# PieSil/CUDA-spectral-ray-tracer

Measured on AMD Instinct MI355X. Metric: Mray/s, higher is better.
Workload: dtype f32; 1 GPU; random-spheres tri scene (4802 tris, 9603 BVH nodes), 1920x1080, 1024 spp, depth 16; scene_id=100, tiles=8x8 px per wave, rank = tile % n_gpus, gather=none (1 GPU), launch_mode=one process, one GPU

## Files before the change

cuda-spectral-ray-tracer_amd/binding.py:

```python
import ctypes as C
import os

_HERE = os.path.dirname(os.path.abspath(__file__))
LIB_PATH = os.environ.get("SRT_LIB_PATH") or os.path.join(_HERE, "libsrt_hip.so")

N_CIE = 95
TILE_PLANES = 9
TILE_LANES = 64

SCENE_CORNELL, SCENE_PRISM, SCENE_TRIS, SCENE_RANDOM_SPHERES, SCENE_MESH100K = 0, 1, 2, 100, 101
BVH_REFERENCE, BVH_SAH = 0, 1
MAT_LAMBERTIAN, MAT_METALLIC, MAT_DIELECTRIC, MAT_EMISSIVE, MAT_NO_MAT = 0, 1, 2, 4, 6


class TriIn(C.Structure):
    _fields_ = [("v0", C.c_float * 3), ("v1", C.c_float * 3), ("v2", C.c_float * 3),
                ("mat_index", C.c_uint32), ("aa_plane", C.c_uint32)]


class Material(C.Structure):
    _fields_ = [("col", C.c_float * 3), ("reflection_fuzz", C.c_float), ("material_type", C.c_uint32),
                ("spectral_distribution", C.c_float * N_CIE), ("emission_power", C.c_float),
                ("sellmeier_B", C.c_float * 3), ("sellmeier_C", C.c_float * 3)]


class CameraData(C.Structure):
    _fields_ = [("width", C.c_uint32), ("height", C.c_uint32),
                ("pixel_delta_u", C.c_float * 3), ("pixel_delta_v", C.c_float * 3), ("pixel00_loc", C.c_float * 3),
                ("defocus_angle", C.c_float),
                ("camera_center", C.c_float * 3), ("defocus_disk_u", C.c_float * 3), ("defocus_disk_v", C.c_float * 3)]


class Stats(C.Structure):
    _fields_ = [("rays", C.c_uint64), ("paths", C.c_uint64), ("node_visits", C.c_uint64), ("tri_tests", C.c_uint64),
                ("box_tests", C.c_uint64), ("util", C.c_uint64 * 9), ("reserved", C.c_uint64 * 2), ("shade", C.c_uint64 * 4),
                ("waves", C.c_uint64 * 4), ("hits", C.c_uint64)]


class Calibration(C.Structure):
    _fields_ = [("wave_cycles_mean", C.c_double), ("wave_cycles_max", C.c_double), ("wall_ms", C.c_double),
                ("instr_per_wave", C.c_uint64), ("n_waves", C.c_uint32), ("n_cu", C.c_uint32), ("waves_per_simd", C.c_uint32),
                ("reserved", C.c_uint32), ("wave_cycles_min", C.c_double)]


class Adaptive(C.Structure):
    _fields_ = [("rel_tol", C.c_float), ("abs_tol", C.c_float), ("min_spp", C.c_uint32), ("reserved", C.c_uint32)]


class Denoise(C.Structure):
    _fields_ = [("levels", C.c_uint32), ("sigma_color", C.c_float), ("sigma_normal", C.c_float), ("sigma_albedo", C.c_float),
                ("sigma_depth", C.c_float), ("reserved", C.c_uint32 * 3)]


class DenoiseVG(C.Structure):
    _fields_ = [("levels", C.c_uint32), ("sigma_variance", C.c_float), ("sigma_normal", C.c_float), ("sigma_albedo", C.c_float),
                ("sigma_depth", C.c_float), ("variance_floor", C.c_float), ("reserved", C.c_uint32 * 2)]


class TreeTuning(C.Structure):
    _fields_ = [("pixels_per_lane", C.c_double), ("throughput_bound", C.c_uint32), ("reinsertion", C.c_uint32),
                ("probe_width", C.c_uint32), ("probe_height", C.c_uint32), ("probe_spp", C.c_uint32), ("nodes_swapped", C.c_uint32),
                ("order_status", C.c_int32)]


class TileScheduleInfo(C.Structure):
    _fields_ = [("tiles_local", C.c_uint32), ("n_rows", C.c_uint32), ("cost_max", C.c_uint32), ("n_waves_plan", C.c_uint32),
                ("split_load_pct", C.c_uint32), ("order_max_pct", C.c_uint32), ("streams", C.c_uint32), ("reserved", C.c_uint32)]


assert C.sizeof(Denoise) == 32 and C.sizeof(DenoiseVG) == 32
assert C.sizeof(Adaptive) == 16 and C.sizeof(TreeTuning) == 40 and C.sizeof(TileScheduleInfo) == 32
assert C.sizeof(Material) == 428 and C.sizeof(CameraData) == 84 and C.sizeof(TriIn) == 44

_vp, _i, _u32, _u64, _f, _sz = C.c_void_p, C.c_int, C.c_uint32, C.c_uint64, C.c_float, C.c_size_t
_fp = C.POINTER(C.c_float)
PROTOTYPES = {
    "srt_version": (C.c_char_p, []),
    "srt_camera_init": (_i, [_i, _i, _f, _fp, _fp, _fp, _f, _f, C.POINTER(CameraData)]),
    "srt_scene_create": (_vp, []),
    "srt_scene_builtin": (_vp, [_i, _u64]),
    "srt_scene_destroy": (None, [_vp]),
    "srt_scene_default_camera": (_i, [_vp, _i, _i, C.POINTER(CameraData)]),
    "srt_scene_set_triangles": (_i, [_vp, C.POINTER(TriIn), _sz]),
    "srt_scene_set_materials": (_i, [_vp, C.POINTER(Material), _sz]),
    "srt_scene_set_background": (_i, [_vp, _fp]),
    "srt_scene_tri_count": (_sz, [_vp]),
    "srt_scene_material_count": (_sz, [_vp]),
    "srt_scene_get_triangles": (_i, [_vp, C.POINTER(TriIn)]),
    "srt_scene_get_materials": (_i, [_vp, C.POINTER(Material)]),
    "srt_scene_get_background": (_i, [_vp, _fp]),
    "srt_scene_get_tri_records": (_i, [_vp, _fp]),
    "srt_material_bake": (_i, [C.POINTER(Material)]),
    "srt_set_reference_quirks": (_i, [_i]),
    "srt_bake_sigmoid_spectrum": (_i, [_fp, _f, _i, _fp]),
    "srt_fit_sigmoid_coeffs": (_i, [_fp, _fp]),
    "srt_color_tables": (_i, [_fp, _fp]),
    "srt_background_spectrum": (_i, [_fp, _fp]),
    "srt_rotation_matrix": (_i, [_f, _i, _fp]),
    "srt_scene_build_bvh": (_i, [_vp, _i, _u64]),
    "srt_scene_order_children": (_i, [_vp, _fp]),
    "srt_scene_optimise_bvh": (_i, [_vp, C.c_int]),
    "srt_scene_is_paired": (_i, [_vp]),
    "srt_scene_node_count": (_sz, [_vp]),
    "srt_scene_bvh_depth": (_i, [_vp]),
    "srt_scene_get_bvh": (_i, [_vp, C.POINTER(C.c_int32), C.POINTER(C.c_int32), C.POINTER(C.c_int32), _fp]),
    "srt_create": (_i, [_i, C.POINTER(_vp)]),
    "srt_destroy": (None, [_vp]),
    "srt_last_error": (C.c_char_p, [_vp]),
    "srt_upload_scene": (_i, [_vp, _vp]),
    "srt_set_camera": (_i, [_vp, C.POINTER(CameraData)]),
    "srt_launch_plan": (_i, [_vp, C.POINTER(_i), C.POINTER(_i), C.POINTER(_i), C.POINTER(_i)]),
    "srt_launch_paired": (_i, [_vp, C.POINTER(_i)]),
    "srt_set_test_knobs": (_i, [_vp, _i, _i, _u32]),
    "srt_get_test_knobs": (_i, [_vp, C.POINTER(_i), C.POINTER(_i), C.POINTER(_u32), C.POINTER(_i)]),
    "srt_launch_lds_bytes": (_i, [_vp, C.POINTER(_sz)]),
    "srt_init_device_params": (_i, [_vp, _u32, _u32, _u32, _u32, _u32, _u32, _u32, _u32, _u64]),
    "srt_set_partition": (_i, [_vp, _u32, _u32]),
    "srt_render_chunk": (_i, [_vp, _u32, _u32, _u32, _u32, _vp]),
    "srt_synchronize": (_i, [_vp]),
    "srt_accum_reset": (_i, [_vp]),
    "srt_render_chunk_accum": (_i, [_vp, _u32, _u32, _u32, _u32, _u32, _vp]),
    "srt_accum_samples": (_i, [_vp, C.POINTER(_u32)]),
    "srt_accum_reset_adaptive": (_i, [_vp, C.POINTER(Adaptive)]),
    "srt_accum_active": (_i, [_vp, C.POINTER(_u64)]),
    "srt_read_accum_stats": (_i, [_vp, C.POINTER(_u32), _fp, _fp, _u32, _u32]),
    "srt_accum_reset_spectral": (_i, [_vp]),
    "srt_read_spectral": (_i, [_vp, _u32, _u32, _fp, _u32, _u32]),
    "srt_develop_spectral": (_i, [_vp, _fp, _u32, _f, _fp, _u32, _u32]),
    "srt_develop_spectral_srgb": (_i, [_vp, _fp, _f, _fp, _fp, _fp, _u32, _u32]),
    "srt_develop_kat": (_i, [_vp, _fp, _u32, _fp, _u32, _f, _fp]),
    "srt_develop_last_ms": (_i, [_vp, _fp, _fp]),
    "srt_accum_reset_features": (_i, [_vp]),
    "srt_read_features": (_i, [_vp, _fp, _u32, _u32]),
    "srt_accum_reset_adaptive_features": (_i, [_vp, C.POINTER(Adaptive)]),
    "srt_accum_reset_spectral_features": (_i, [_vp]),
    "srt_denoise_developed": (_i, [_vp, C.POINTER(Denoise), _fp, _u32, _f, _fp, _fp, _u32, _u32]),
    "srt_denoise_developed_kat": (_i, [_vp, C.POINTER(Denoise), _fp, _fp, _fp, _u32, _u32, _u32, _u32, _fp, _fp]),
    "srt_denoise_features": (_i, [_vp, C.POINTER(Denoise), _fp, _fp, _fp, _u32, _u32]),
    "srt_denoise_kat": (_i, [_vp, C.POINTER(Denoise), _fp, _fp, _u32, _u32, _u32, _fp]),
    "srt_denoise_last_ms": (_i, [_vp, _fp, _fp, _fp, C.POINTER(_u32)]),
    "srt_denoise_features_vg": (_i, [_vp, C.POINTER(DenoiseVG), _fp, _fp, _fp, _fp, _u32, _u32]),
    "srt_denoise_vg_kat": (_i, [_vp, C.POINTER(DenoiseVG), _fp, _fp, _u32, _u32, _u32, _fp, _fp]),
    "srt_denoise_estimate_last_ms": (_i, [_vp, _fp]),
    "srt_denoise_features_mv": (_i, [_vp, C.POINTER(DenoiseVG), _fp, _fp, _fp, _fp, _u32, _u32]),
    "srt_denoise_mv_kat": (_i, [_vp, C.POINTER(DenoiseVG), _fp, _fp, C.POINTER(_u32), _fp, _u32, _u32, _fp, _fp]),
    "srt_accum_reset_streams": (_i, [_vp, _u32]),
    "srt_accum_streams": (_i, [_vp, C.POINTER(_u32)]),
    "srt_set_gather_planes": (_i, [_vp, _u32]),
    "srt_tile_buffer": (_i, [_vp, C.POINTER(_vp), C.POINTER(_sz), C.POINTER(_u32), C.POINTER(_u32)]),
    "srt_copy_tile_buffer": (_i, [_vp, _vp, _vp]),
    "srt_scatter_tiles": (_i, [_vp, _vp, _vp]),
    "srt_dev_fb": (_i, [_vp, C.POINTER(_vp), C.POINTER(_vp), C.POINTER(_vp), C.POINTER(_sz)]),
    "srt_read_fb": (_i, [_vp, _fp, _fp, _fp]),
    "srt_read_fb_rowmajor": (_i, [_vp, _fp, _fp, _fp, _u32, _u32]),
    "srt_read_fb_aux": (_i, [_vp, _i, _fp, _fp, _fp]),
    "srt_get_tile_costs": (_i, [_vp, C.POINTER(C.c_uint32), _sz]),
    "srt_order_children_by_profile": (_i, [_vp, _vp, C.c_uint32, C.c_uint32, C.c_uint32, C.c_uint32, C.c_uint32, C.POINTER(C.c_uint32)]),
    "srt_pixels_per_lane": (_i, [_vp, _u32, _u32, _u32, C.POINTER(C.c_double)]),
    "srt_tune_tree_for_throughput": (_i, [_vp, _vp, _u32, _u32, _u32, _u32, _i, C.POINTER(TreeTuning)]),
    "srt_get_stats": (_i, [_vp, C.POINTER(Stats)]),
    "srt_set_count_traversal": (_i, [_vp, _i]),
    "srt_get_wave_debug": (_i, [_vp, C.POINTER(C.c_uint32), _sz]),
    "srt_last_kernel_ms": (_i, [_vp, C.POINTER(_f)]),
    "srt_trace_rays": (_i, [_vp, _fp, _sz, _fp]),
    "srt_device_op_sweep": (_i, [_vp, _i, _fp, _fp, _sz, _fp]),
    "srt_order_tiles_kat": (_i, [_vp, C.POINTER(_u32), _u32, _u32, _u32, _u32, C.POINTER(_u32), _sz, C.POINTER(_u32), C.POINTER(_u32)]),
    "srt_read_tile_schedule": (_i, [_vp, _i, C.POINTER(_u32), _sz, C.POINTER(TileScheduleInfo)]),
    "srt_calibrate": (_i, [_vp, _i, _u32, _u32, C.POINTER(Calibration)]),
    "srt_ctx_device": (_i, [_vp]),
    "srt_ctx_cu_count": (_i, [_vp]),
    "srt_comm_init_all": (_i, [C.POINTER(_i), _i, C.POINTER(_vp)]),
    "srt_comm_unique_id": (_i, [C.POINTER(C.c_ubyte)]),
    "srt_comm_init_rank": (_i, [_vp, C.POINTER(C.c_ubyte), _u32, _u32, C.POINTER(_vp)]),
    "srt_comm_available": (_i, []),
    "srt_comm_set_gather_planes": (_i, [_vp, _u32]),
    "srt_comm_last_gather_ms": (_i, [_vp, C.POINTER(_f)]),
    "srt_comm_destroy": (None, [_vp]),
    "srt_comm_last_error": (C.c_char_p, [_vp]),
    "srt_comm_world": (_u32, [_vp]),
    "srt_comm_local_count": (_u32, [_vp]),
    "srt_comm_ctx": (_vp, [_vp, _u32]),
    "srt_comm_root_ctx": (_vp, [_vp]),
    "srt_comm_upload_scene": (_i, [_vp, _vp]),
    "srt_comm_set_camera": (_i, [_vp, C.POINTER(CameraData)]),
    "srt_comm_init_device_params": (_i, [_vp, _u32, _u32, _u32, _u32, _u32, _u32, _u32, _u32, _u64]),
    "srt_render_frame_multi": (_i, [_vp, _u32, _u32, _u32, _u32]),
    "srt_comm_accum_reset": (_i, [_vp]),
    "srt_render_frame_multi_accum": (_i, [_vp, _u32, _u32, _u32, _u32, _u32]),
    "srt_comm_accum_reset_adaptive": (_i, [_vp, C.POINTER(Adaptive)]),
    "srt_comm_accum_active": (_i, [_vp, C.POINTER(_u64)]),
    "srt_comm_accum_reset_spectral": (_i, [_vp]),
    "srt_comm_accum_reset_features": (_i, [_vp]),
    "srt_comm_accum_reset_adaptive_features": (_i, [_vp, C.POINTER(Adaptive)]),
    "srt_comm_accum_reset_spectral_features": (_i, [_vp]),
    "srt_comm_accum_reset_streams": (_i, [_vp, _u32]),
    "srt_comm_synchronize": (_i, [_vp]),
    "srt_comm_stats": (_i, [_vp, C.POINTER(_u64), C.POINTER(_u64), C.POINTER(_f)]),
}


class SrtError(RuntimeError):
    def __init__(self, code, msg):
        super().__init__("srt error %d: %s" % (code, msg))
        self.code = code


_lib = None


def lib():
    global _lib
    if _lib is None:
        if not os.path.exists(LIB_PATH):
            raise ImportError("%s not found: run `python -c 'import __graft_entry__ as g; g.build()'` "
                              "(there is no CPU fallback for the render path)" % LIB_PATH)
        L = C.CDLL(LIB_PATH)
        for name, (res, args) in PROTOTYPES.items():
            fn = getattr(L, name)
            fn.restype = res
            fn.argtypes = args
        _lib = L
    return _lib


COMM_ID_BYTES = 128


def check_comm(code, comm=None):
    if code is not None and code < 0:
        msg = lib().srt_comm_last_error(comm)
        raise SrtError(code, msg.decode() if msg else "")
    return code


def check(code, ctx=None):
    if code is not None and code < 0:
        msg = lib().srt_last_error(ctx)
        raise SrtError(code, msg.decode() if msg else "")
    return code


def fptr(arr):
    return arr.ctypes.data_as(_fp)
```

cuda-spectral-ray-tracer_amd/csrc/srt_capi.cpp:

```cpp
#include <dlfcn.h>
#include <hip/hip_runtime.h>
#include <stdint.h>
#include <stdlib.h>
#include <string.h>

#include <algorithm>
#include <cmath>
#include <cstddef>
#include <string>
#include <vector>

#include "srt_host.h"
#include "srt_internal.h"

using namespace srt;

#ifndef SRT_FRINGE_STRIDE_L2
#define SRT_FRINGE_STRIDE_L2 96
#endif
static constexpr uint32_t kFringeStrideL2 = SRT_FRINGE_STRIDE_L2;
static constexpr uint32_t kScoreShadeL2 = 320u, kScoreFringeL2 = 800u;

struct DeviceBuffer {
    void *ptr = nullptr;
    size_t bytes = 0;
    DeviceBuffer() = default;
    DeviceBuffer(DeviceBuffer &&o) noexcept { swap(o); }
    DeviceBuffer &operator=(DeviceBuffer &&o) noexcept { swap(o); return *this; }
    ~DeviceBuffer() { release(); }
    void swap(DeviceBuffer &o) { std::swap(ptr, o.ptr); std::swap(bytes, o.bytes); }
    void release() { if (ptr) (void)hipFree(ptr); ptr = nullptr; bytes = 0; }
    hipError_t reserve(size_t n) {
        if (n <= bytes) return hipSuccess;
        release();
        const hipError_t e = hipMalloc(&ptr, n);
        if (e == hipSuccess) bytes = n; else ptr = nullptr;
        return e;
    }
    template <typename T> T *as() const { return static_cast<T *>(ptr); }
    explicit operator bool() const { return ptr != nullptr; }
};

struct srt_ctx {
    int device = 0;
    std::string err;
    DeviceBuffer d_nodes, d_nodes_sw, d_fringe, d_tris, d_mat_sd, d_mat_par, d_shade, d_cmf;
    DeviceBuffer d_mat_col;
    int root_ref = 0, stack_depth = 1, n_inner = 0, n_records = 0;
    bool paired = false;
    uint32_t fringe_stride = 96;
    uint32_t n_tris = 0;
    uint32_t n_materials = 0;
    bool scene_ready = false, camera_ready = false, params_ready = false;
    srt_camera_data cam;
    uint32_t tx = 0, ty = 0, bx = 0, by = 0, chunk_w = 0, chunk_h = 0, spp = 0, bounce = 0;
    uint64_t seed = SRT_DEFAULT_SEED;
    uint32_t n_lanes = 0;
    uint32_t rank = 0, world = 1;
    uint32_t gather_planes = 3;
    uint32_t fb_groups_valid = 3;
    uint32_t last_w = 0, last_h = 0, last_offx = 0, last_offy = 0;
    uint32_t tiles_x = 0, tiles_y = 0, n_tiles = 0, tiles_local = 0, tiles_padded = 0;
    DeviceBuffer d_rng;
    DeviceBuffer d_fb;
    DeviceBuffer d_tiles;
    DeviceBuffer d_counters;
    int n_cu = 256;
    uint32_t waves_per_cu = 0;
    uint32_t score_shade = 0, score_fringe = 0;
    uint32_t debug_lane_limit = 0;
    PlanKnobs knobs;
    bool knobs_from_env = false;
    uint32_t split_load_pct = 200;
    uint32_t probe_spp = 2;
    int order_max_pct = -1;
    DeviceBuffer d_tile_cost, d_tile_order;
    srt_tile_schedule_info sched_note = {};
    bool sched_probe_queue = false, sched_compacted_queue = false;
    bool count_traversal = false;
    hipEvent_t ev0 = nullptr, ev1 = nullptr;
    bool timed = false;
    DeviceBuffer d_rowmajor;
    uint32_t rowmajor_w = 0, rowmajor_h = 0;
    OrderProfile order_profile = {};
    DeviceBuffer d_wave_debug;
    uint32_t stats_spp = 0;
    bool stats_adaptive = false;
    struct Accumulation {
        enum class State { Invalid, Empty, Bound } state = State::Invalid;
        enum class Kind { Plain, Adaptive, Spectral, Streams, Features, AdaptiveFeatures, SpectralFeatures } kind = Kind::Plain;
        uint32_t total = 0;
        uint32_t n_streams = 1;
        uint32_t w = 0, h = 0, offx = 0, offy = 0;
        void invalidate() { state = State::Invalid; }
        void begin(Kind k, uint32_t streams_per_pixel = 1) { kind = k; n_streams = streams_per_pixel; state = State::Empty; }
        bool valid() const { return state != State::Invalid; }
        bool bound() const { return state == State::Bound; }
        bool adaptive() const { return kind == Kind::Adaptive || kind == Kind::AdaptiveFeatures; }
        bool spectral() const { return kind == Kind::Spectral || kind == Kind::SpectralFeatures; }
        bool streamed() const { return kind == Kind::Streams; }
        bool featured() const { return kind == Kind::Features || kind == Kind::AdaptiveFeatures || kind == Kind::SpectralFeatures; }
    } accum;
    DeviceBuffer d_accum;
    DeviceBuffer d_adapt;
    DeviceBuffer d_adapt_queue;
    DeviceBuffer d_film;
    DeviceBuffer d_film_staging;
    DeviceBuffer d_features;
    DeviceBuffer d_features_staging;
    DeviceBuffer d_denoise;
    DeviceBuffer d_denoise_in;
    DeviceBuffer d_denoise_dev;
    hipEvent_t denoise_ev[12] = {};
    uint32_t denoise_timed_levels = 0;
    uint32_t denoise_level_ev = 1;
    bool denoise_timed = false;
    DeviceBuffer d_develop;
    DeviceBuffer d_develop_in;
    hipEvent_t develop_ev[3] = {};
    bool develop_timed = false, develop_epilogue = false;
    DeviceBuffer d_streams;
    uint32_t streams_seeded = 0;
};

namespace {

struct Roctx {
    int (*push)(const char *) = nullptr;
    int (*pop)() = nullptr;
    Roctx() {
        for (const char *n : {"libroctx64.so.4", "libroctx64.so", "/opt/rocm/lib/libroctx64.so.4"}) {
            if (void *h = dlopen(n, RTLD_NOW | RTLD_LOCAL)) {
                push = (int (*)(const char *))dlsym(h, "roctxRangePushA");
                pop = (int (*)())dlsym(h, "roctxRangePop");
                if (push && pop) return;
                push = nullptr; pop = nullptr;
            }
        }
    }
};
struct RoctxRange {
    static Roctx &api() { static Roctx r; return r; }
    explicit RoctxRange(const char *name) { if (api().push) api().push(name); }
    ~RoctxRange() { if (api().pop) api().pop(); }
};

int fail(srt_ctx *ctx, int code, const std::string &msg) {
    if (ctx) ctx->err = msg;
    set_global_error(msg);
    return code;
}
int hip_fail(srt_ctx *ctx, hipError_t e, const char *what) {
    return fail(ctx, SRT_ERR_HIP, std::string(what) + ": " + hipGetErrorString(e));
}
#define HIP_TRY_AS(ctx, what, expr) do { if (hipError_t _e = (expr)) return hip_fail(ctx, _e, what); } while (0)
#define HIP_TRY(ctx, expr) HIP_TRY_AS(ctx, #expr, expr)

int upload(srt_ctx *ctx, DeviceBuffer &dst, const std::vector<float> &src) {
    HIP_TRY(ctx, dst.reserve(src.size() * sizeof(float)));
    HIP_TRY(ctx, hipMemcpy(dst.ptr, src.data(), src.size() * sizeof(float), hipMemcpyHostToDevice));
    return SRT_OK;
}


struct TileSchedule {
    uint32_t *rows = nullptr, *sorted = nullptr, *info = nullptr, *cost = nullptr;
    static size_t order_bytes(size_t tiles) { return (tiles * 65 + 4) * sizeof(uint32_t); }
    static size_t cost_bytes(size_t tiles) { return 2 * tiles * sizeof(uint32_t); }
    explicit TileSchedule(const srt_ctx *c) : cost(c->d_tile_cost.as<uint32_t>()) {
        if (!c->d_tile_order) return;
        const size_t tiles = (c->d_tile_order.bytes / sizeof(uint32_t) - 4) / 65;
        rows = c->d_tile_order.as<uint32_t>(); sorted = rows + tiles * 64; info = sorted + tiles;
    }
};

struct AdaptQueue {
    uint32_t *info, *rows, *flags;
    unsigned long long *counts;
    static size_t bytes(size_t n_rows) { return (8 + 2 * n_rows) * sizeof(uint32_t); }
    explicit AdaptQueue(const DeviceBuffer &d_adapt_queue)
        : info(d_adapt_queue.as<uint32_t>()), rows(info + 8), flags(rows + (d_adapt_queue.bytes / sizeof(uint32_t) - 8) / 2),
          counts(reinterpret_cast<unsigned long long *>(info + 4)) {}
};
int read_adapt_counts(srt_ctx *c, uint64_t *rendered, uint64_t *active) {
    unsigned long long counts = 0;
    HIP_TRY(c, hipMemcpy(&counts, AdaptQueue(c->d_adapt_queue).counts, sizeof(counts), hipMemcpyDeviceToHost));
    if (rendered) *rendered = counts & 0xffffffffull;
    if (active) *active = counts >> 32;
    return SRT_OK;
}

struct AccumLayout {
    static constexpr size_t kAccumHeaderBytes = 256;
    AccumHeader *header;
    float *sums, *y;
    static size_t sums_bytes(size_t lanes) { return 3 * lanes * sizeof(float); }
    static size_t bytes(size_t lanes) { return kAccumHeaderBytes + sums_bytes(lanes); }
    explicit AccumLayout(const srt_ctx *c)
        : header(c->d_accum.as<AccumHeader>()), sums(reinterpret_cast<float *>(c->d_accum.as<char>() + kAccumHeaderBytes)), y(sums + c->n_lanes) {}
};
void set_accum_header(RenderParams &p, AccumHeader *h) { p.wave_debug = reinterpret_cast<uint32_t *>(h); }

struct AdaptPlanes {
    float *sum2;
    uint32_t *state;
    static size_t bytes(size_t lanes) { return 2 * lanes * sizeof(float); }
    explicit AdaptPlanes(const srt_ctx *c) : sum2(c->d_adapt.as<float>()), state(c->d_adapt.as<uint32_t>() + c->n_lanes) {}
};

struct StreamPlanes {
    uint32_t *rng;
    float *sums;
    static size_t sums_bytes(size_t lanes, size_t k) { return 3 * k * lanes * sizeof(float); }
    static size_t bytes(size_t lanes, size_t k) { return kStreamSumPlane * k * lanes * sizeof(uint32_t) + sums_bytes(lanes, k); }
    StreamPlanes(const DeviceBuffer &d_streams, size_t lanes, size_t k) : rng(d_streams.as<uint32_t>()), sums(d_streams.as<float>() + kStreamSumPlane * k * lanes) {}
};

uint32_t clipped_w(const srt_ctx *c) { return std::min<uint32_t>(c->last_w, c->tx * c->bx); }
uint32_t clipped_h(const srt_ctx *c) { return std::min<uint32_t>(c->last_h, c->ty * c->by); }
struct ChunkRect { uint32_t w, h; size_t first; };
ChunkRect chunk_rect(const srt_ctx *c, uint32_t image_width, uint32_t image_height) {
    if (c->last_offx >= image_width || c->last_offy >= image_height) return {0, 0, 0};
    return {std::min<uint32_t>(clipped_w(c), image_width - c->last_offx), std::min<uint32_t>(clipped_h(c), image_height - c->last_offy),
            (size_t)c->last_offy * image_width + c->last_offx};
}

size_t wave_debug_bytes(size_t n_waves) { return sizeof(OrderProfile) + n_waves * 4 * sizeof(uint32_t); }
uint32_t wave_debug_waves(const srt_ctx *c) { return c->d_wave_debug ? (uint32_t)((c->d_wave_debug.bytes - sizeof(OrderProfile)) / (4 * sizeof(uint32_t))) : 0u; }

float *fb_plane(const srt_ctx *c, int k) { return c->d_fb.as<float>() + (size_t)k * c->n_lanes; }

LaunchPlan plan_of(const srt_ctx *c) { LaunchPlan lp; render_launch_plan(c->stack_depth, c->n_records, c->n_inner, c->knobs, lp); return lp; }

void fill_params(const srt_ctx *c, RenderParams &p) {
    memset(&p, 0, sizeof(p));
    p.nodes = c->d_nodes.as<const float4>(); p.nodes_sw = c->d_nodes_sw.as<const float>(); p.fringe = c->d_fringe.as<const float4>(); p.tris = c->d_tris.as<const float4>();
    p.mat_sd = c->d_mat_sd.as<const float2>(); p.mat_par = c->d_mat_par.as<const float4>();
    p.shade = c->d_shade.as<const float4>(); p.cmf = c->d_cmf.as<const float4>();
    p.root_ref = c->root_ref; p.stack_depth = c->stack_depth; p.n_materials = c->n_materials;
    p.n_inner = c->n_inner; p.n_cached = 0;
    p.n_tris = c->n_tris; p.n_records = c->n_records; p.fringe_stride = c->fringe_stride;
    p.paired = c->paired ? 1u : 0u;
    for (int k = 0; k < 3; k++) {
        p.du[k] = c->cam.pixel_delta_u[k]; p.dv[k] = c->cam.pixel_delta_v[k]; p.p00[k] = c->cam.pixel00_loc[k];
        p.center[k] = c->cam.camera_center[k]; p.disk_u[k] = c->cam.defocus_disk_u[k]; p.disk_v[k] = c->cam.defocus_disk_v[k];
    }
    p.defocus_angle = c->cam.defocus_angle;
    p.tx = c->tx; p.ty = c->ty; p.bx = c->bx; p.by = c->by;
    p.spp = c->spp; p.bounce_limit = c->bounce;
    p.rank = c->rank; p.world = c->world;
    p.rng = c->d_rng.as<uint32_t>(); p.n_lanes = c->n_lanes;
    p.tile_out = c->d_tiles.as<float>(); p.counters = c->d_counters.as<unsigned long long>();
    p.tile_group_stride = c->tiles_padded * (uint32_t)(kGroupPlanes * kTileLanes);
    p.write_parity = c->gather_planes == (uint32_t)kTilePlanes ? 1u : 0u;
}


struct Pass {
    uint32_t spp_add;
    hipStream_t st;
    RenderMode mode;
    bool later;
    LaunchPlan plan;
    bool ordered;
    uint32_t adapt_bound;
    uint32_t streams;
};

bool adaptive_mode(RenderMode m) { return m == Adaptive || m == AdaptiveFeatures; }
uint32_t split_rows_bound(const srt_ctx *c) { return (uint32_t)std::min<uint64_t>((uint64_t)c->tiles_local * 64, 0x7fffffffull); }
constexpr uint64_t kQueueSlots = 1ull << 32;
bool queue_may_split(const srt_ctx *c, uint32_t streams) { return c->split_load_pct && (streams == 1 || (uint64_t)split_rows_bound(c) * streams * 64 < kQueueSlots); }

void tile_geometry(srt_ctx *c) {
    const uint32_t cover_w = c->tx * c->bx, cover_h = c->ty * c->by;
    c->tiles_x = (cover_w + 7) / 8; c->tiles_y = (cover_h + 7) / 8;
    c->n_tiles = c->tiles_x * c->tiles_y;
    c->tiles_padded = (c->n_tiles + c->world - 1) / c->world;
    c->tiles_local = c->n_tiles > c->rank ? (c->n_tiles - c->rank + c->world - 1) / c->world : 0;
}

int prepare_tiles(srt_ctx *c, const Pass &ps) {
    tile_geometry(c);
    const size_t tile_floats = (size_t)std::max<uint32_t>(c->tiles_padded, 1) * kTileLanes;
    HIP_TRY(c, c->d_tiles.reserve(tile_floats * kTilePlanes * sizeof(float)));
    if (!(adaptive_mode(ps.mode) && ps.later)) HIP_TRY(c, hipMemsetAsync(c->d_tiles.ptr, 0, tile_floats * c->gather_planes * sizeof(float), ps.st));
    HIP_TRY(c, hipMemsetAsync(c->d_counters.ptr, 0, (kCounters + 1) * sizeof(unsigned long long), ps.st));
    return SRT_OK;
}

void chunk_params(const srt_ctx *c, const Pass &ps, uint32_t width, uint32_t height, uint32_t offx, uint32_t offy, RenderParams &p) {
    fill_params(c, p);
    if (ps.spp_add) p.spp = ps.spp_add / ps.streams;
    p.width = width; p.height = height; p.offx = offx; p.offy = offy;
    p.tiles_x = c->tiles_x; p.tiles_y = c->tiles_y; p.n_tiles = c->n_tiles;
    p.tiles_local = c->tiles_local;
    p.pixel_counter = reinterpret_cast<uint32_t *>(c->d_counters.as<unsigned long long>() + kCounters);
    p.waves_per_cu_override = c->waves_per_cu;
    const bool all_cached = ps.plan.all_cached;
    p.score_shade = c->score_shade ? c->score_shade : (all_cached ? 70u : kScoreShadeL2);
    const bool paired = render_paired_variant(c->paired, render_narrow_refs(c->n_records, c->knobs), all_cached);
    p.score_fringe = c->score_fringe ? c->score_fringe : (all_cached ? (paired ? 400u : 280u) : kScoreFringeL2);
    p.tile_order = nullptr; p.tile_cost = nullptr; p.queue_rows = nullptr; p.queue_rows_bound = c->tiles_local;
    p.debug_lane_limit = c->debug_lane_limit;
}

int run_cost_probe(srt_ctx *c, const Pass &ps, const RenderParams &p) {
    HIP_TRY(c, c->d_tile_cost.reserve(TileSchedule::cost_bytes(c->tiles_local)));
    HIP_TRY(c, c->d_tile_order.reserve(TileSchedule::order_bytes(c->tiles_local)));
    const TileSchedule sched(c);
    HIP_TRY(c, hipMemsetAsync(sched.cost, 0, TileSchedule::cost_bytes(c->tiles_local), ps.st));
    RenderParams pp = p;
    pp.spp = c->probe_spp; pp.tile_cost = sched.cost;
    RoctxRange range_probe("srt cost probe + pixel queue");
    HIP_TRY(c, launch_render(pp, c->knobs, (uint32_t)c->n_cu, Probe, ps.st));
    const uint32_t n_waves_plan = std::max<uint32_t>((uint32_t)c->n_cu * (uint32_t)ps.plan.waves_per_cu / ps.streams, 1u);
    const uint32_t order_pct = c->order_max_pct >= 0 ? (uint32_t)c->order_max_pct : ((!ps.plan.all_cached && (uint64_t)c->tiles_local < 6ull * n_waves_plan) ? 100u : 0u);
    const uint32_t split_pct = queue_may_split(c, ps.streams) ? c->split_load_pct : 0u;
    HIP_TRY(c, launch_order_tiles(sched.cost, sched.sorted, sched.rows, c->tiles_local, n_waves_plan, split_pct, sched.info, order_pct, ps.st));
    c->sched_note = {};
    c->sched_note.tiles_local = c->tiles_local; c->sched_note.n_waves_plan = n_waves_plan; c->sched_note.split_load_pct = split_pct;
    c->sched_note.order_max_pct = order_pct; c->sched_note.streams = ps.streams;
    HIP_TRY(c, hipMemsetAsync(c->d_counters.as<unsigned long long>() + kCounters, 0, sizeof(unsigned long long), ps.st));
    return SRT_OK;
}

enum class QueueSource { Identity, FreshProbe, ReusedProbe, Compacted };

QueueSource queue_source(const srt_ctx *c, const Pass &ps) {
    if (adaptive_mode(ps.mode) && ps.later && c->tiles_local <= kQueueTileMask) return QueueSource::Compacted;
    if (!ps.ordered) return QueueSource::Identity;
    return ps.later ? QueueSource::ReusedProbe : QueueSource::FreshProbe;
}

int choose_queue(srt_ctx *c, Pass &ps, RenderParams &p) {
    const bool schedulable = c->probe_spp > 0 && c->tiles_local > 1 && c->tiles_local <= kQueueTileMask;
    ps.ordered = schedulable && (ps.spp_add || c->spp > 4 * c->probe_spp);
    ps.adapt_bound = ps.ordered && c->split_load_pct ? split_rows_bound(c) : c->tiles_local;
    if (adaptive_mode(ps.mode)) HIP_TRY(c, c->d_adapt_queue.reserve(AdaptQueue::bytes(std::max<uint32_t>(ps.adapt_bound, 1u))));
    const QueueSource src = queue_source(c, ps);
    c->sched_probe_queue = false; c->sched_compacted_queue = false;
    if (src == QueueSource::Compacted) {
        const AdaptQueue q(c->d_adapt_queue);
        p.tile_order = q.rows;
        p.queue_rows = q.info;
        p.prio_cost = ps.ordered ? c->d_tile_cost.as<uint32_t>() : nullptr;
        p.queue_rows_bound = ps.adapt_bound;
    } else if (src != QueueSource::Identity) {
        if (src == QueueSource::FreshProbe)
            if (const int rc = run_cost_probe(c, ps, p)) return rc;
        const TileSchedule sched(c);
        p.tile_order = sched.rows;
        p.queue_rows = sched.info;
        p.prio_cost = sched.cost;
        if (queue_may_split(c, ps.streams)) p.queue_rows_bound = split_rows_bound(c);
    }
    c->sched_probe_queue = ps.ordered && src != QueueSource::Identity;
    p.queue_rows_bound *= ps.streams;
    return SRT_OK;
}

int bind_wave_debug(srt_ctx *c, const Pass &ps, RenderParams &p) {
    if (!c->count_traversal) return SRT_OK;
    const uint32_t most_waves = render_launch_grid(ps.plan, (uint32_t)c->n_cu, p.waves_per_cu_override, UINT32_MAX).waves;
    HIP_TRY(c, c->d_wave_debug.reserve(wave_debug_bytes(most_waves)));
    HIP_TRY(c, hipMemsetAsync(c->d_wave_debug.ptr, 0, c->d_wave_debug.bytes, ps.st));
    p.wave_debug = c->d_wave_debug.as<uint32_t>();
    if (c->order_profile.magic == kOrderProfileMagic)
        HIP_TRY(c, hipMemcpyAsync(c->d_wave_debug.ptr, &c->order_profile, sizeof(OrderProfile), hipMemcpyHostToDevice, ps.st));
    return SRT_OK;
}

int launch_pass(srt_ctx *c, const Pass &ps, RenderParams &p) {
    if (c->count_traversal && render_launch_grid(ps.plan, (uint32_t)c->n_cu, p.waves_per_cu_override, p.queue_rows_bound).waves > wave_debug_waves(c))
        return fail(c, SRT_ERR_HIP, "srt_render_chunk: the launch started more waves than the debug buffer holds (launch plan and launcher disagree)");
    HIP_TRY(c, hipEventRecord(c->ev0, ps.st));
    if (ps.spp_add) set_accum_header(p, AccumLayout(c).header);
    HIP_TRY(c, launch_render(p, c->knobs, (uint32_t)c->n_cu, ps.mode, ps.st));
    HIP_TRY(c, hipEventRecord(c->ev1, ps.st));
    return SRT_OK;
}

int compact_adaptive_queue(srt_ctx *c, const Pass &ps, const RenderParams &p) {
    const TileSchedule sched(c);
    const AdaptQueue dst(c->d_adapt_queue);
    AdaptQueueParams q = {};
    q.src_rows = ps.ordered ? sched.rows : nullptr; q.src_info = ps.ordered ? sched.info : nullptr; q.n_identity = c->tiles_local;
    q.dst_info = dst.info; q.dst_rows = dst.rows; q.flags = dst.flags; q.counts = dst.counts;
    q.state = AdaptPlanes(c).state;
    q.spp_total = c->accum.total + ps.spp_add;
    q.width = p.width; q.height = p.height; q.tx = c->tx; q.ty = c->ty; q.bx = c->bx; q.by = c->by;
    q.tiles_x = c->tiles_x; q.n_tiles = c->n_tiles; q.rank = c->rank; q.world = c->world;
    q.lane_limit = c->debug_lane_limit ? c->debug_lane_limit : 64u;
    HIP_TRY(c, hipMemsetAsync(q.counts, 0, sizeof(unsigned long long), ps.st));
    HIP_TRY(c, launch_adapt_queue(q, ps.adapt_bound, ps.st));
    c->sched_compacted_queue = true;
    return SRT_OK;
}

int combine_streams(srt_ctx *c, const Pass &ps, const RenderParams &p) {
    StreamCombineParams q = {};
    q.stream_sums = StreamPlanes(c->d_streams, c->n_lanes, ps.streams).sums; q.sums = AccumLayout(c).sums; q.tile_out = p.tile_out;
    q.streams = ps.streams; q.spp_total = c->accum.total + ps.spp_add; q.n_lanes = c->n_lanes;
    q.tile_group_stride = p.tile_group_stride; q.write_parity = p.write_parity; q.tiles_local = c->tiles_local;
    q.width = p.width; q.height = p.height; q.tx = c->tx; q.ty = c->ty; q.bx = c->bx; q.by = c->by;
    q.tiles_x = c->tiles_x; q.n_tiles = c->n_tiles; q.rank = c->rank; q.world = c->world;
    q.lane_limit = c->debug_lane_limit ? c->debug_lane_limit : 64u;
    HIP_TRY(c, launch_stream_combine(q, ps.st));
    return SRT_OK;
}

int render_chunk_impl(srt_ctx *c, uint32_t width, uint32_t height, uint32_t offx, uint32_t offy, uint32_t spp_add, hipStream_t st) {
    Pass ps = {};
    ps.spp_add = spp_add; ps.st = st;
    ps.mode = !spp_add ? (c->count_traversal ? Counting : Plain) : c->accum.adaptive() ? (c->accum.featured() ? AdaptiveFeatures : Adaptive) : c->accum.spectral() ? (c->accum.featured() ? SpectralFeatures : Spectral) : c->accum.streamed() ? Streams : c->accum.featured() ? Features : Accum;
    ps.later = spp_add && c->accum.bound(); ps.plan = plan_of(c);
    ps.streams = ps.mode == Streams ? c->accum.n_streams : 1u;
    c->last_w = width; c->last_h = height; c->last_offx = offx; c->last_offy = offy;
    RenderParams p;
    if (const int rc = prepare_tiles(c, ps)) return rc;
    chunk_params(c, ps, width, height, offx, offy, p);
    if (const int rc = choose_queue(c, ps, p)) return rc;
    if (const int rc = bind_wave_debug(c, ps, p)) return rc;
    RoctxRange range_render("srt render_kernel");
    if (const int rc = launch_pass(c, ps, p)) return rc;
    if (adaptive_mode(ps.mode))
        if (const int rc = compact_adaptive_queue(c, ps, p)) return rc;
    if (ps.mode == Streams)
        if (const int rc = combine_streams(c, ps, p)) return rc;
    c->timed = true;
    c->stats_spp = spp_add;
    c->stats_adaptive = adaptive_mode(ps.mode);
    return SRT_OK;
}

int read_planes(srt_ctx *c, int first_plane, float *p0, float *p1, float *p2) {
    if (!c || !c->d_fb) return fail(c, SRT_ERR_INVALID, "read: device parameters not initialised");
    if (const int rc = srt_synchronize(c)) return rc;
    float *dst[3] = {p0, p1, p2};
    for (int k = 0; k < 3; k++)
        if (dst[k]) HIP_TRY(c, hipMemcpy(dst[k], fb_plane(c, first_plane + k), (size_t)c->n_lanes * sizeof(float), hipMemcpyDeviceToHost));
    return SRT_OK;
}

int read_rowmajor(srt_ctx *c, const float *const src[3], float *const host[3], uint32_t image_width, uint32_t image_height) {
    HIP_TRY(c, hipSetDevice(c->device));
    const size_t n = (size_t)image_width * image_height;
    if (c->rowmajor_w != image_width || c->rowmajor_h != image_height || !c->d_rowmajor) {
        HIP_TRY(c, c->d_rowmajor.reserve(3 * n * sizeof(float)));
        HIP_TRY(c, hipMemset(c->d_rowmajor.ptr, 0, 3 * n * sizeof(float)));
        c->rowmajor_w = image_width; c->rowmajor_h = image_height;
    }
    float *dst[3] = {c->d_rowmajor.as<float>(), c->d_rowmajor.as<float>() + n, c->d_rowmajor.as<float>() + 2 * n};
    HIP_TRY(c, launch_unswizzle(src, dst, c->tx, c->ty, c->bx, c->by, c->last_w, c->last_h, c->last_offx, c->last_offy, image_width, image_height, nullptr));
    const ChunkRect rect = chunk_rect(c, image_width, image_height);
    const size_t pitch = (size_t)image_width * sizeof(float);
    for (int k = 0; k < 3 && rect.w && rect.h; k++)
        if (host[k]) HIP_TRY(c, hipMemcpy2D(host[k] + rect.first, pitch, dst[k] + rect.first, pitch, (size_t)rect.w * sizeof(float), rect.h, hipMemcpyDeviceToHost));
    HIP_TRY(c, hipDeviceSynchronize());
    return SRT_OK;
}

}

extern "C" {

int srt_create(int device, srt_ctx **out) {
    if (!out) return fail(nullptr, SRT_ERR_INVALID, "srt_create: null out");
    *out = nullptr;
    int n = 0;
    hipError_t e = hipGetDeviceCount(&n);
    if (e != hipSuccess || n <= 0)
        return fail(nullptr, SRT_ERR_NO_DEVICE, std::string("srt_create: no HIP device (") + (e != hipSuccess ? hipGetErrorString(e) : "count 0") +
                                                    "); this library has no CPU fallback");
    if (device < 0 || device >= n) return fail(nullptr, SRT_ERR_NO_DEVICE, "srt_create: device index out of range");
    e = hipSetDevice(device);
    if (e != hipSuccess) return hip_fail(nullptr, e, "hipSetDevice");
    srt_ctx *c = new srt_ctx();
    c->device = device;
    if (const char *ev = getenv("SRT_WAVES_PER_CU")) c->waves_per_cu = (uint32_t)std::max(0, atoi(ev));
    if (const char *ev = getenv("SRT_PROBE_SPP")) c->probe_spp = (uint32_t)std::max(0, atoi(ev));
    if (const char *ev = getenv("SRT_SCORE_SHADE")) c->score_shade = (uint32_t)std::max(1, atoi(ev));
    if (const char *ev = getenv("SRT_SCORE_FRINGE")) c->score_fringe = (uint32_t)std::max(1, atoi(ev));
    if (const char *tk = getenv("SRT_TEST_KNOBS")) if (atoi(tk) == 1) {
        if (const char *ev = getenv("SRT_DEBUG_LANE_LIMIT")) { c->debug_lane_limit = (uint32_t)std::max(0, atoi(ev)); c->knobs_from_env = true; }
        if (const char *ev = getenv("SRT_WIDE_REFS")) { c->knobs.wide_refs = atoi(ev) != 0; c->knobs_from_env = true; }
        if (const char *ev = getenv("SRT_LDS_CACHE_MAX")) { c->knobs.lds_cache_max = std::max(0, atoi(ev)); c->knobs_from_env = true; }
    }
    if (const char *ev = getenv("SRT_SPLIT_LOAD")) c->split_load_pct = (uint32_t)std::max(0, atoi(ev));
    if (const char *ev = getenv("SRT_ORDER_MAX_PCT")) c->order_max_pct = std::min(400, std::max(-1, atoi(ev)));
    {
        hipDeviceProp_t prop;
        if (hipGetDeviceProperties(&prop, device) == hipSuccess && prop.multiProcessorCount > 0) c->n_cu = prop.multiProcessorCount;
    }
    std::vector<float> rows(96 * 4);
    cmf_rows(rows.data());
    int rc = upload(c, c->d_cmf, rows);
    if (rc != SRT_OK) { delete c; return rc; }
    if ((e = c->d_counters.reserve((kCounters + 1) * sizeof(unsigned long long))) != hipSuccess ||
        (e = hipMemset(c->d_counters.ptr, 0, (kCounters + 1) * sizeof(unsigned long long))) != hipSuccess ||
        (e = hipEventCreate(&c->ev0)) != hipSuccess || (e = hipEventCreate(&c->ev1)) != hipSuccess) {
        int r = hip_fail(nullptr, e, "srt_create");
        srt_destroy(c);
        return r;
    }
    *out = c;
    return SRT_OK;
}

void srt_destroy(srt_ctx *c) {
    if (!c) return;
    (void)hipSetDevice(c->device);
    (void)hipDeviceSynchronize();
    if (c->ev0) (void)hipEventDestroy(c->ev0);
    if (c->ev1) (void)hipEventDestroy(c->ev1);
    for (hipEvent_t e : c->denoise_ev) if (e) (void)hipEventDestroy(e);
    for (hipEvent_t e : c->develop_ev) if (e) (void)hipEventDestroy(e);
    delete c;
}

int srt_ctx_device(const srt_ctx *ctx) { return ctx ? ctx->device : -1; }
int srt_ctx_cu_count(const srt_ctx *ctx) { return ctx ? ctx->n_cu : -1; }

const char *srt_last_error(const srt_ctx *ctx) { return ctx ? ctx->err.c_str() : global_error(); }

int srt_upload_scene(srt_ctx *c, const srt_scene *s) {
    if (!c || !s) return fail(c, SRT_ERR_INVALID, "srt_upload_scene: null argument");
    c->accum.invalidate();
    c->sched_probe_queue = false; c->sched_compacted_queue = false;
    HIP_TRY(c, hipSetDevice(c->device));
    FlatScene f;
    int rc = flatten_scene(*s, f);
    if (rc != SRT_OK) return fail(c, rc, global_error());
    if (render_lds_bytes(f.stack_depth, 1, 0, f.n_records, c->knobs) > 64 * 1024) return fail(c, SRT_ERR_BVH, "srt_upload_scene: BVH too deep for the LDS traversal stack");
    if ((rc = upload(c, c->d_nodes, f.nodes)) != SRT_OK) return rc;
    {
        LaunchPlan plan;
        render_launch_plan(f.stack_depth, f.n_records, f.n_inner, c->knobs, plan);
        uint32_t stride = plan.all_cached ? 96u : kFringeStrideL2;
        if (const char *ev = getenv("SRT_FRINGE_STRIDE")) stride = (atoi(ev) == 128 && !plan.all_cached) ? 128u : 96u;
        if ((uint64_t)(f.n_records - f.n_inner + 1) * stride >= (1ull << 31)) stride = 96u;
        std::vector<float> padded;
        if (stride != 96u) {
            const size_t n_fr = f.fringe.size() / 24;
            padded.assign(n_fr * 32, 0.f);
            for (size_t k = 0; k < n_fr; k++) memcpy(&padded[32 * k], &f.fringe[24 * k], 24 * sizeof(float));
        }
        if ((rc = upload(c, c->d_fringe, stride == 96u ? f.fringe : padded)) != SRT_OK) return rc;
        c->fringe_stride = stride;
        c->d_nodes_sw.release();
        if (!plan.all_cached && (rc = upload(c, c->d_nodes_sw, f.nodes_sw)) != SRT_OK) return rc;
    }
    if ((rc = upload(c, c->d_tris, f.tris)) != SRT_OK) return rc;
    if ((rc = upload(c, c->d_mat_sd, f.mat_sd)) != SRT_OK) return rc;
    if ((rc = upload(c, c->d_mat_par, f.mat_par)) != SRT_OK) return rc;
    if ((rc = upload(c, c->d_shade, f.shade)) != SRT_OK) return rc;
    {
        std::vector<float> col(4 * s->mats.size(), 0.f);
        for (size_t m = 0; m < s->mats.size(); m++)
            for (int k = 0; k < 3; k++) col[4 * m + k] = s->mats[m].col[k];
        if ((rc = upload(c, c->d_mat_col, col)) != SRT_OK) return rc;
    }
    c->root_ref = f.root_ref; c->stack_depth = f.stack_depth; c->n_materials = (uint32_t)s->mats.size();
    c->n_inner = f.n_inner; c->n_records = f.n_records; c->n_tris = (uint32_t)s->raw.size();
    c->paired = tree_is_paired(*s);
    c->scene_ready = true;
    return SRT_OK;
}

int srt_set_camera(srt_ctx *c, const srt_camera_data *cam) {
    if (!c || !cam) return fail(c, SRT_ERR_INVALID, "srt_set_camera: null argument");
    c->accum.invalidate();
    c->cam = *cam;
    c->camera_ready = true;
    return SRT_OK;
}

int srt_launch_plan(const srt_ctx *c, int *waves_per_cu, int *n_cached, int *all_cached, int *narrow_refs) {
    if (!c || !c->scene_ready) return fail(nullptr, SRT_ERR_INVALID, "srt_launch_plan: no scene uploaded");
    const LaunchPlan plan = plan_of(c);
    if (waves_per_cu) *waves_per_cu = plan.waves_per_cu;
    if (n_cached) *n_cached = plan.n_cached;
    if (all_cached) *all_cached = plan.all_cached ? 1 : 0;
    if (narrow_refs) *narrow_refs = render_narrow_refs(c->n_records, c->knobs) ? 1 : 0;
    return SRT_OK;
}

int srt_launch_paired(const srt_ctx *c, int *paired) {
    if (!c || !c->scene_ready || !paired) return fail(nullptr, SRT_ERR_INVALID, "srt_launch_paired: no scene uploaded / null argument");
    const LaunchPlan plan = plan_of(c);
    *paired = render_paired_variant(c->paired, render_narrow_refs(c->n_records, c->knobs), plan.all_cached) ? 1 : 0;
    return SRT_OK;
}

int srt_launch_lds_bytes(const srt_ctx *c, size_t *bytes) {
    if (!c || !c->scene_ready || !bytes) return fail(nullptr, SRT_ERR_INVALID, "srt_launch_lds_bytes: no scene uploaded / null argument");
    const LaunchPlan plan = plan_of(c);
    *bytes = render_lds_bytes(c->stack_depth, plan.waves_per_block, plan.n_cached, c->n_records, c->knobs);
    return SRT_OK;
}

int srt_set_test_knobs(srt_ctx *c, int wide_refs, int lds_cache_max, uint32_t lane_limit) {
    if (!c || lds_cache_max < -1 || lane_limit > 64) return fail(c, SRT_ERR_INVALID, "srt_set_test_knobs: bad argument");
    c->knobs.wide_refs = wide_refs != 0; c->knobs.lds_cache_max = lds_cache_max; c->debug_lane_limit = lane_limit;
    c->scene_ready = false;
    return SRT_OK;
}
int srt_get_test_knobs(const srt_ctx *c, int *wide_refs, int *lds_cache_max, uint32_t *lane_limit, int *from_env) {
    if (!c) return fail(nullptr, SRT_ERR_INVALID, "srt_get_test_knobs: null ctx");
    if (wide_refs) *wide_refs = c->knobs.wide_refs ? 1 : 0;
    if (lds_cache_max) *lds_cache_max = c->knobs.lds_cache_max;
    if (lane_limit) *lane_limit = c->debug_lane_limit;
    if (from_env) *from_env = c->knobs_from_env ? 1 : 0;
    return SRT_OK;
}

int srt_internal_init_device_params(srt_ctx *c, uint32_t tx, uint32_t ty, uint32_t bx, uint32_t by, uint32_t chunk_w, uint32_t chunk_h,
                                    uint32_t spp, uint32_t bounce_limit, uint64_t seed, int wait) {
    if (!c) return fail(c, SRT_ERR_INVALID, "srt_init_device_params: null ctx");
    if (tx == 0 || ty == 0 || bx == 0 || by == 0 || chunk_w == 0 || chunk_h == 0)
        return fail(c, SRT_ERR_INVALID, "srt_init_device_params: zero dimension");
    c->accum.invalidate();
    c->sched_probe_queue = false; c->sched_compacted_queue = false;
    const uint64_t lanes = (uint64_t)tx * ty * bx * by;
    if (lanes > 0x7fffffffull) return fail(c, SRT_ERR_INVALID, "srt_init_device_params: grid too large");
    HIP_TRY(c, hipSetDevice(c->device));
    c->tx = tx; c->ty = ty; c->bx = bx; c->by = by; c->chunk_w = chunk_w; c->chunk_h = chunk_h;
    c->spp = (uint16_t)spp; c->bounce = (uint16_t)bounce_limit;
    c->seed = seed; c->n_lanes = (uint32_t)lanes;
    c->streams_seeded = 0;
    HIP_TRY(c, c->d_rng.reserve(6 * lanes * sizeof(uint32_t)));
    HIP_TRY(c, c->d_fb.reserve(kTilePlanes * lanes * sizeof(float)));
    HIP_TRY(c, hipMemset(c->d_fb.ptr, 0, kTilePlanes * lanes * sizeof(float)));
    HIP_TRY(c, launch_init_rng(c->d_rng.as<uint32_t>(), c->n_lanes, seed, nullptr));
    if (wait) HIP_TRY(c, hipDeviceSynchronize());
    c->fb_groups_valid = (uint32_t)kTileGroups;
    c->params_ready = true;
    return SRT_OK;
}

int srt_init_device_params(srt_ctx *c, uint32_t tx, uint32_t ty, uint32_t bx, uint32_t by, uint32_t chunk_w, uint32_t chunk_h,
                           uint32_t spp, uint32_t bounce_limit, uint64_t seed) {
    return srt_internal_init_device_params(c, tx, ty, bx, by, chunk_w, chunk_h, spp, bounce_limit, seed, 1);
}

int srt_set_partition(srt_ctx *c, uint32_t rank, uint32_t world) {
    if (!c || world == 0 || rank >= world) return fail(c, SRT_ERR_INVALID, "srt_set_partition: need rank < world");
    c->accum.invalidate();
    c->sched_probe_queue = false; c->sched_compacted_queue = false;
    c->rank = rank; c->world = world;
    return SRT_OK;
}

// ... 944 lines not shown
        }
        c->count_traversal = true; c->rank = 0; c->world = 1;
        int r = srt_init_device_params(c, tx, ty, bx, by, width, height, spp, bounce_limit, SRT_DEFAULT_SEED);
        if (r == SRT_OK) r = srt_render_chunk(c, width, height, 0, 0, nullptr);
        if (r == SRT_OK) r = srt_synchronize(c);
        c->count_traversal = counting; c->rank = rank; c->world = world;
        c->order_profile = OrderProfile{};
        c->params_ready = false;
        if (r != SRT_OK) return r;
        unsigned long long h[kCounters];
        HIP_TRY_AS(c, "srt_order_children_by_profile: counters", hipMemcpy(h, c->d_counters.ptr, sizeof(h), hipMemcpyDeviceToHost));
        work = h[1] + 2ull * h[2];
        return SRT_OK;
    };
    unsigned long long work_before = 0, work_after = 0;
    if ((rc = probe_frame(true, work_before)) != SRT_OK) return rc;
    std::vector<uint32_t> cnt(2 * n_nodes, 0u);
    HIP_TRY_AS(c, "srt_order_children_by_profile: read back", hipMemcpy(cnt.data(), d_cnt.ptr, cnt.size() * sizeof(uint32_t), hipMemcpyDeviceToHost));
    {
        unsigned long long samples = 0;
        for (uint32_t v : cnt) samples += v;
        if (samples == 0) return fail(c, SRT_ERR_INVALID, "srt_order_children_by_profile: the probe frame recorded no samples (no closest hit with the sibling's box beyond it)");
    }
    const uint32_t *won = cnt.data();
    std::vector<uint32_t> swapped_nodes;
    for (size_t k = 0; k < n_nodes; k++) {
        BvhNode &nd = s->nodes[k];
        if (nd.prim >= 0) continue;
        const uint32_t l = won[2 * k], r = won[2 * k + 1];
        if (l + r >= std::max<uint32_t>(min_samples, 1u) && r > l) { std::swap(nd.left, nd.right); swapped_nodes.push_back((uint32_t)k); }
    }
    if (!swapped_nodes.empty()) {
        rc = srt_upload_scene(c, s);
        if (rc == SRT_OK) rc = probe_frame(false, work_after);
        if (rc == SRT_OK && work_after >= work_before) {
            for (uint32_t k : swapped_nodes) std::swap(s->nodes[k].left, s->nodes[k].right);
            swapped_nodes.clear();
            rc = srt_upload_scene(c, s);
        }
    }
    if (rc == SRT_OK && n_swapped) *n_swapped = (uint32_t)swapped_nodes.size();
    return rc;
}

int srt_pixels_per_lane(const srt_ctx *c, uint32_t width, uint32_t height, uint32_t world, double *out) {
    if (!c || !c->scene_ready || !out) return fail(nullptr, SRT_ERR_INVALID, "srt_pixels_per_lane: no scene uploaded / null argument");
    const double lanes = (double)c->n_cu * plan_of(c).waves_per_cu * 64.0;
    *out = (double)width * height / (double)std::max<uint32_t>(world, 1u) / (lanes > 0 ? lanes : 1.0);
    return SRT_OK;
}

static constexpr double kTunePixelsPerLane = 6.0;
static constexpr size_t kTuneReinsertionMaxTris = 8192;
static constexpr int kTuneReinsertionPasses = 3;
static constexpr uint32_t kTuneProbeDivisor = 4, kTuneProbeMinSide = 32, kTuneProbeSpp = 8;
static constexpr uint32_t kTuneDecidingRays = 16;

int srt_tune_tree_for_throughput(srt_ctx *c, srt_scene *s, uint32_t width, uint32_t height, uint32_t world, uint32_t bounce_limit,
                                 int only_if_throughput_bound, srt_tree_tuning *out) {
    if (out) memset(out, 0, sizeof(*out));
    if (!c || !s || !out || !s->bvh_valid || width == 0 || height == 0)
        return fail(c, SRT_ERR_INVALID, "srt_tune_tree_for_throughput: null argument / BVH not built / empty frame");
    int rc = srt_upload_scene(c, s);
    if (rc == SRT_OK) rc = srt_pixels_per_lane(c, width, height, world, &out->pixels_per_lane);
    if (rc != SRT_OK) return rc;
    out->throughput_bound = out->pixels_per_lane >= kTunePixelsPerLane ? 1u : 0u;
    if (only_if_throughput_bound && !out->throughput_bound) return SRT_OK;
    if (s->raw.size() <= kTuneReinsertionMaxTris) {
        auto resident = [&](const FlatScene &f) { LaunchPlan lp; render_launch_plan(f.stack_depth, f.n_records, f.n_inner, c->knobs, lp); return lp.all_cached; };
        const bool kept = optimise_bvh_unless(*s, kTuneReinsertionPasses, [&](const FlatScene &before, const FlatScene &after) { return !(resident(before) && !resident(after)); });
        out->reinsertion = kept ? 1u : 2u;
    }
    const uint32_t pw = std::max(width / kTuneProbeDivisor, kTuneProbeMinSide), ph = std::max(height / kTuneProbeDivisor, kTuneProbeMinSide);
    srt_camera_data probe_cam{};
    rc = srt_scene_default_camera(s, (int)pw, (int)ph, &probe_cam);
    if (rc == SRT_OK) rc = srt_set_camera(c, &probe_cam);
    if (rc == SRT_OK) {
        out->probe_width = pw; out->probe_height = ph; out->probe_spp = kTuneProbeSpp;
        rc = srt_order_children_by_profile(c, s, pw, ph, kTuneProbeSpp, bounce_limit, kTuneDecidingRays, &out->nodes_swapped);
    } else fail(c, rc, global_error());
    out->order_status = rc;
    return SRT_OK;
}

int srt_set_count_traversal(srt_ctx *c, int on) {
    if (!c) return fail(c, SRT_ERR_INVALID, "srt_set_count_traversal: null ctx");
    c->count_traversal = on != 0;
    return SRT_OK;
}

int srt_last_kernel_ms(srt_ctx *c, float *ms) {
    if (!c || !ms || !c->timed) return fail(c, SRT_ERR_INVALID, "srt_last_kernel_ms: nothing rendered yet");
    HIP_TRY(c, hipSetDevice(c->device));
    HIP_TRY(c, hipEventSynchronize(c->ev1));
    HIP_TRY(c, hipEventElapsedTime(ms, c->ev0, c->ev1));
    return SRT_OK;
}

int srt_trace_rays(srt_ctx *c, const float *rays, size_t n, float *out) {
    if (!c || !c->scene_ready || (!rays && n) || (!out && n)) return fail(c, SRT_ERR_INVALID, "srt_trace_rays: scene not uploaded / bad argument");
    if (n == 0) return SRT_OK;
    HIP_TRY(c, hipSetDevice(c->device));
    DeviceBuffer d_in, d_out;
    HIP_TRY_AS(c, "srt_trace_rays", d_in.reserve(6 * n * sizeof(float)));
    HIP_TRY_AS(c, "srt_trace_rays", d_out.reserve(4 * n * sizeof(float)));
    HIP_TRY_AS(c, "srt_trace_rays", hipMemcpy(d_in.ptr, rays, 6 * n * sizeof(float), hipMemcpyHostToDevice));
    RenderParams p;
    fill_params(c, p);
    HIP_TRY_AS(c, "srt_trace_rays", launch_trace(p, d_in.as<float>(), n, d_out.as<float>(), nullptr));
    HIP_TRY_AS(c, "srt_trace_rays", hipDeviceSynchronize());
    HIP_TRY_AS(c, "srt_trace_rays", hipMemcpy(out, d_out.ptr, 4 * n * sizeof(float), hipMemcpyDeviceToHost));
    return SRT_OK;
}

int srt_device_op_sweep(srt_ctx *c, int which, const float *a, const float *b, size_t n, float *out) {
    if (!c || !a || !b || !out) return fail(c, SRT_ERR_INVALID, "srt_device_op_sweep: null argument");
    if (n == 0) return SRT_OK;
    HIP_TRY(c, hipSetDevice(c->device));
    DeviceBuffer buf;
    HIP_TRY_AS(c, "srt_device_op_sweep", buf.reserve(3 * n * sizeof(float)));
    float *d = buf.as<float>();
    HIP_TRY_AS(c, "srt_device_op_sweep", hipMemcpy(d, a, n * sizeof(float), hipMemcpyHostToDevice));
    HIP_TRY_AS(c, "srt_device_op_sweep", hipMemcpy(d + n, b, n * sizeof(float), hipMemcpyHostToDevice));
    HIP_TRY_AS(c, "srt_device_op_sweep", launch_op_sweep(which, d, d + n, n, d + 2 * n, nullptr));
    HIP_TRY_AS(c, "srt_device_op_sweep", hipDeviceSynchronize());
    HIP_TRY_AS(c, "srt_device_op_sweep", hipMemcpy(out, d + 2 * n, n * sizeof(float), hipMemcpyDeviceToHost));
    return SRT_OK;
}

int srt_order_tiles_kat(srt_ctx *c, const uint32_t *cost, uint32_t n, uint32_t n_waves, uint32_t split_load_pct, uint32_t order_max_pct,
                        uint32_t *rows_out, size_t rows_cap, uint32_t *sorted_out, uint32_t *info_out) {
    if (!c || !cost || !rows_out || !sorted_out || !info_out) return fail(c, SRT_ERR_INVALID, "srt_order_tiles_kat: null argument");
    if (n == 0 || n > (1u << 20)) return fail(c, SRT_ERR_INVALID, "srt_order_tiles_kat: n must be in 1 .. 2^20");
    if (rows_cap < (size_t)n * 64 + 64) return fail(c, SRT_ERR_INVALID, "srt_order_tiles_kat: rows_cap must be at least 64 * n + 64 (the largest queue and 64 guard words)");
    HIP_TRY(c, hipSetDevice(c->device));
    DeviceBuffer d_cost, d_rows, d_sorted, d_info;
    HIP_TRY_AS(c, "srt_order_tiles_kat", d_cost.reserve(TileSchedule::cost_bytes(n)));
    HIP_TRY_AS(c, "srt_order_tiles_kat", d_rows.reserve(rows_cap * sizeof(uint32_t)));
    HIP_TRY_AS(c, "srt_order_tiles_kat", d_sorted.reserve(n * sizeof(uint32_t)));
    HIP_TRY_AS(c, "srt_order_tiles_kat", d_info.reserve(4 * sizeof(uint32_t)));
    HIP_TRY_AS(c, "srt_order_tiles_kat", hipMemcpy(d_cost.ptr, cost, TileSchedule::cost_bytes(n), hipMemcpyHostToDevice));
    HIP_TRY_AS(c, "srt_order_tiles_kat", hipMemset(d_rows.ptr, 0xff, rows_cap * sizeof(uint32_t)));
    HIP_TRY_AS(c, "srt_order_tiles_kat", hipMemset(d_sorted.ptr, 0xff, n * sizeof(uint32_t)));
    HIP_TRY_AS(c, "srt_order_tiles_kat", hipMemset(d_info.ptr, 0xff, 4 * sizeof(uint32_t)));
    HIP_TRY_AS(c, "srt_order_tiles_kat", launch_order_tiles(d_cost.as<uint32_t>(), d_sorted.as<uint32_t>(), d_rows.as<uint32_t>(), n, n_waves, split_load_pct,
                                                            d_info.as<uint32_t>(), order_max_pct, nullptr));
    HIP_TRY_AS(c, "srt_order_tiles_kat", hipDeviceSynchronize());
    HIP_TRY_AS(c, "srt_order_tiles_kat", hipMemcpy(rows_out, d_rows.ptr, rows_cap * sizeof(uint32_t), hipMemcpyDeviceToHost));
    HIP_TRY_AS(c, "srt_order_tiles_kat", hipMemcpy(sorted_out, d_sorted.ptr, n * sizeof(uint32_t), hipMemcpyDeviceToHost));
    HIP_TRY_AS(c, "srt_order_tiles_kat", hipMemcpy(info_out, d_info.ptr, 4 * sizeof(uint32_t), hipMemcpyDeviceToHost));
    return SRT_OK;
}

int srt_read_tile_schedule(srt_ctx *c, int which, uint32_t *rows_out, size_t rows_cap, srt_tile_schedule_info *info) {
    if (!c || !info || (!rows_out && rows_cap) || (which != 0 && which != 1)) return fail(c, SRT_ERR_INVALID, "srt_read_tile_schedule: bad argument");
    if (which == 0 ? !c->sched_probe_queue : !c->sched_compacted_queue)
        return fail(c, SRT_ERR_INVALID, which == 0 ? "srt_read_tile_schedule: the last launch ran no cost probe's queue (no probe, or too few samples or tiles for one)"
                                                   : "srt_read_tile_schedule: the last launch was no adaptive pass: no compacted queue");
    if (const int rc = srt_synchronize(c)) return rc;
    const uint32_t *d_rows = which == 0 ? TileSchedule(c).rows : AdaptQueue(c->d_adapt_queue).rows;
    const uint32_t *d_info = which == 0 ? TileSchedule(c).info : AdaptQueue(c->d_adapt_queue).info;
    uint32_t head[2] = {0u, 0u};
    HIP_TRY(c, hipMemcpy(head, d_info, sizeof(head), hipMemcpyDeviceToHost));
    srt_tile_schedule_info out = c->sched_probe_queue ? c->sched_note : srt_tile_schedule_info{};
    if (!c->sched_probe_queue) { out.tiles_local = c->tiles_local; out.streams = 1u; }
    out.n_rows = head[0]; out.cost_max = head[1];
    if (rows_cap < out.n_rows) return fail(c, SRT_ERR_INVALID, "srt_read_tile_schedule: rows_cap is smaller than the queue");
    if (out.n_rows) HIP_TRY(c, hipMemcpy(rows_out, d_rows, (size_t)out.n_rows * sizeof(uint32_t), hipMemcpyDeviceToHost));
    *info = out;
    return SRT_OK;
}

int srt_calibrate(srt_ctx *c, int kind, uint32_t waves_per_simd, uint32_t iters, srt_calibration *out) {
    if (!c || !out || kind < 0 || kind >= calib_kinds() || waves_per_simd < 1 || waves_per_simd > 4 || iters == 0)
        return fail(c, SRT_ERR_INVALID, "srt_calibrate: bad argument");
    HIP_TRY(c, hipSetDevice(c->device));
    const uint32_t threads = waves_per_simd * 256u, n_blocks = (uint32_t)c->n_cu, n_waves = n_blocks * threads / 64u;
    DeviceBuffer d_cyc, d_sink, d_table;
    HIP_TRY_AS(c, "srt_calibrate", d_cyc.reserve(n_waves * sizeof(unsigned long long)));
    HIP_TRY_AS(c, "srt_calibrate", d_sink.reserve(1024 * sizeof(float)));
    const uint32_t n_table = 1u << 18;
    if (kind >= 11) {
        HIP_TRY_AS(c, "srt_calibrate", d_table.reserve((size_t)n_table * 64));
        HIP_TRY_AS(c, "srt_calibrate", hipMemset(d_table.ptr, 0, (size_t)n_table * 64));
    }
    struct Event { hipEvent_t ev = nullptr; ~Event() { if (ev) (void)hipEventDestroy(ev); } } e0, e1;
    HIP_TRY_AS(c, "srt_calibrate", hipEventCreate(&e0.ev));
    HIP_TRY_AS(c, "srt_calibrate", hipEventCreate(&e1.ev));
    HIP_TRY_AS(c, "srt_calibrate", launch_calib(kind, n_blocks, threads, iters / 8u + 1u, d_sink.as<float>(), d_cyc.as<unsigned long long>(), d_table.as<float4>(), n_table, nullptr));
    HIP_TRY_AS(c, "srt_calibrate", hipEventRecord(e0.ev, nullptr));
    HIP_TRY_AS(c, "srt_calibrate", launch_calib(kind, n_blocks, threads, iters, d_sink.as<float>(), d_cyc.as<unsigned long long>(), d_table.as<float4>(), n_table, nullptr));
    HIP_TRY_AS(c, "srt_calibrate", hipEventRecord(e1.ev, nullptr));
    HIP_TRY_AS(c, "srt_calibrate", hipEventSynchronize(e1.ev));
    float ms = 0.f;
    HIP_TRY_AS(c, "srt_calibrate", hipEventElapsedTime(&ms, e0.ev, e1.ev));
    std::vector<unsigned long long> h(n_waves);
    HIP_TRY_AS(c, "srt_calibrate", hipMemcpy(h.data(), d_cyc.ptr, n_waves * sizeof(unsigned long long), hipMemcpyDeviceToHost));
    double sum = 0, mx = 0, mn = 1e300;
    for (unsigned long long v : h) { sum += (double)v; mx = std::max(mx, (double)v); mn = std::min(mn, (double)v); }
    memset(out, 0, sizeof(*out));
    out->wave_cycles_mean = sum / n_waves; out->wave_cycles_max = mx; out->wave_cycles_min = mn; out->wall_ms = ms;
    out->instr_per_wave = (uint64_t)iters * 32u;
    out->n_waves = n_waves; out->n_cu = n_blocks; out->waves_per_simd = waves_per_simd;
    return SRT_OK;
}

}
```

cuda-spectral-ray-tracer_amd/csrc/srt_internal.h:

```cpp
#pragma once
#include <hip/hip_runtime.h>
#include <stdint.h>
#include <stddef.h>

struct srt_ctx;
extern "C" int srt_internal_init_device_params(srt_ctx *c, uint32_t tx, uint32_t ty, uint32_t bx, uint32_t by, uint32_t chunk_w, uint32_t chunk_h,
                                               uint32_t spp, uint32_t bounce_limit, uint64_t seed, int wait);

extern "C" uint32_t srt_internal_gather_planes(const srt_ctx *c);

namespace srt {

constexpr int kTilePlanes = 9;
constexpr int kTileGroups = 3;
constexpr int kGroupPlanes = 3;
constexpr int kTileLanes = 64;
constexpr int kCounters = 32;

constexpr uint32_t kQueueTileBits = 22, kQueueTileMask = (1u << kQueueTileBits) - 1u;
constexpr uint32_t kQueuePartShift = kQueueTileBits, kQueuePartMask = 63u;
constexpr uint32_t kQueueLevelShift = 28, kQueueLevelMask = 7u;

struct RenderParams {
    const float4 *nodes;
    const float *nodes_sw;
    const float4 *fringe;
    const float4 *tris;
    const float2 *mat_sd;
    const float4 *shade;
    const float4 *mat_par;
    const float4 *cmf;
    int root_ref;
    int stack_depth;
    int n_inner;
    int n_cached;
    int n_records;
    uint32_t fringe_stride;
    uint32_t n_materials;
    uint32_t n_tris;
    uint32_t paired;
    float du[3], dv[3], p00[3];
    float defocus_angle;
    float center[3], disk_u[3], disk_v[3];
    uint32_t width, height, offx, offy;
    uint32_t tx, ty, bx, by;
    uint32_t spp, bounce_limit;
    uint32_t tiles_x, tiles_y, n_tiles;
    uint32_t rank, world;
    uint32_t tiles_local;
    uint32_t *pixel_counter;
    const uint32_t *tile_order;
    uint32_t *tile_cost;
    const uint32_t *queue_rows;
    const uint32_t *prio_cost;
    uint32_t queue_rows_bound;
    uint32_t waves_per_cu_override;
    uint32_t score_shade, score_fringe;
    uint32_t debug_lane_limit;
    uint32_t *rng;
    uint32_t n_lanes;
    float *tile_out;
    uint32_t tile_group_stride;
    uint32_t write_parity;
    unsigned long long *counters;
    uint32_t *wave_debug;
};

struct OrderProfile {
    unsigned long long magic;
    const int32_t *leaf;
    const int32_t *up;
    const float *sibbox;
    uint32_t *cnt;
    unsigned long long n_nodes;
};
constexpr unsigned long long kOrderProfileMagic = 0x5352544f52444552ull;

struct AccumHeader {
    float *sums;
    uint32_t spp_total;
    uint32_t pad;
    float *sum2;
    uint32_t *state;
    float rel_tol, abs_tol;
    uint32_t min_spp, pad2;
    float *film;
    uint32_t *stream_planes;
    uint32_t streams, pad3;
    float *features;
    const float *mat_col;
};
constexpr uint32_t kFeatureStride = 8;
constexpr uint32_t kStreamSumPlane = 6;
constexpr uint32_t kMaxStreams = 16;
constexpr uint32_t kFilmSamples = 95;
constexpr uint32_t kFilmStride = 96;
constexpr uint32_t kAdaptConverged = 0x80000000u;


struct ScatterParams {
    const float *gathered;
    uint32_t groups;
    float *fb[9];
    uint32_t width, height;
    uint32_t tx, ty, bx, by;
    uint32_t tiles_x, n_tiles, world, tiles_padded;
};

hipError_t launch_init_rng(uint32_t *rng, uint32_t n_lanes, uint64_t seed, hipStream_t st);
struct PlanKnobs { bool wide_refs = false; int lds_cache_max = -1; };
enum RenderMode { Plain = 0, Counting = 1, Probe = 2, Accum = 3, Adaptive = 4, Spectral = 5, Streams = 6, Features = 7, AdaptiveFeatures = 8, SpectralFeatures = 9 };
hipError_t launch_render(const RenderParams &p, const PlanKnobs &knobs, uint32_t n_cu, RenderMode mode, hipStream_t st);
hipError_t launch_accum_header(AccumHeader *dst, float *sums, uint32_t spp_total, hipStream_t st);
struct AdaptQueueParams {
    const uint32_t *src_rows, *src_info;
    uint32_t n_identity;
    uint32_t *dst_rows, *dst_info, *flags;
    unsigned long long *counts;
    const uint32_t *state;
    uint32_t spp_total;
    uint32_t width, height, tx, ty, bx, by, tiles_x, n_tiles, rank, world, lane_limit;
};
hipError_t launch_adapt_queue(const AdaptQueueParams &p, uint32_t n_rows_bound, hipStream_t st);
hipError_t launch_film_unswizzle(const float *film, float *dst, uint32_t first, uint32_t count, uint32_t w, uint32_t h, uint32_t tx,
                                 uint32_t ty, uint32_t bx, hipStream_t st);
hipError_t launch_features_unswizzle(const float *rows, float *dst, uint32_t w, uint32_t h, uint32_t tx, uint32_t ty, uint32_t bx, hipStream_t st);
struct StreamCombineParams {
    const float *stream_sums;
    float *sums;
    float *tile_out;
    uint32_t streams, spp_total, n_lanes;
    uint32_t tile_group_stride, write_parity;
    uint32_t tiles_local;
    uint32_t width, height, tx, ty, bx, by, tiles_x, n_tiles, rank, world, lane_limit;
};
hipError_t launch_stream_combine(const StreamCombineParams &p, hipStream_t st);
struct DenoisePrepassParams {
    const float *sums;
    size_t sum_pixel_stride, sum_comp_stride;
    const float4 *rows;
    uint32_t tx, ty, bx;
    uint32_t w, h, samples;
    float4 *guides, *colour;
    const uint32_t *counts;
};
hipError_t launch_denoise_prepass(const DenoisePrepassParams &p, hipStream_t st);
struct DenoiseLevelParams {
    const float4 *guides, *src;
    float4 *dst;
    uint32_t w, h, step;
    uint32_t tiles_x;
    float kn, ka, kz, kc;
};
hipError_t launch_denoise_level(const DenoiseLevelParams &p, hipStream_t st);
hipError_t launch_denoise_epilogue(const float *colour, float *out_xyz, float *out_lin, float *out_q, size_t n, hipStream_t st);
struct DenoiseVarianceParams {
    const float4 *guides;
    float *colour, *out_var;
    uint32_t w, h;
    uint32_t tiles_x;
    float kn, ka, kz;
};
hipError_t launch_denoise_variance(const DenoiseVarianceParams &p, hipStream_t st);
struct DenoiseMeasuredParams {
    const float *sum_y, *sum_y2;
    const uint32_t *counts;
    size_t sum_pixel_stride;
    uint32_t tx, ty, bx;
    uint32_t w, h;
    float *colour, *out_var;
};
hipError_t launch_denoise_measured(const DenoiseMeasuredParams &p, hipStream_t st);
struct DenoiseLevelVgParams {
    const float4 *guides, *src;
    float4 *dst;
    uint32_t w, h, step;
    uint32_t tiles_x;
    float kn, ka, kz, ks, floor;
};
hipError_t launch_denoise_level_vg(const DenoiseLevelVgParams &p, hipStream_t st);
hipError_t launch_denoise_var_out(const float *colour, float *out_var, size_t n, hipStream_t st);
uint32_t denoise_payload_groups(uint32_t channels);
struct DenoisePayloadPrepassParams {
    const float *developed;
    float4 *payload;
    size_t pixels;
    uint32_t channels, groups, samples;
};
hipError_t launch_denoise_payload_prepass(const DenoisePayloadPrepassParams &p, hipStream_t st);
struct DenoiseLevelDevParams {
    const float4 *guides, *src;
    float4 *dst;
    const float4 *psrc;
    float4 *pdst;
    uint32_t w, h, step;
    uint32_t tiles_x;
    uint32_t groups;
    float kn, ka, kz, kc;
};
hipError_t launch_denoise_level_dev(const DenoiseLevelDevParams &p, hipStream_t st);
hipError_t launch_denoise_dev_out(const float4 *payload, float *out_dev, uint32_t channels, uint32_t groups, size_t n, hipStream_t st);
constexpr uint32_t kMaxDevelopChannels = 16;
struct DevelopParams {
    const float *film, *response;
    float *out;
    float scale;
    uint32_t channels;
    uint32_t n_lanes, tx, ty, bx;
    uint32_t w, h;
};
uint32_t develop_padded_channels(uint32_t channels);
hipError_t launch_develop(const DevelopParams &p, hipStream_t st);
hipError_t launch_develop_srgb(const float *xyz, float *out_lin, float *out_q, uint32_t samples, size_t n, hipStream_t st);
hipError_t launch_order_tiles(const uint32_t *cost, uint32_t *sorted, uint32_t *rows, uint32_t n, uint32_t n_waves,
                              uint32_t split_load_pct, uint32_t *queue_info, uint32_t order_max_pct, hipStream_t st);
hipError_t launch_scatter(const ScatterParams &p, hipStream_t st);
hipError_t launch_unswizzle(const float *const src[3], float *const dst[3], uint32_t tx, uint32_t ty, uint32_t bx, uint32_t by,
                            uint32_t n_cols, uint32_t n_rows, uint32_t offx, uint32_t offy, uint32_t image_width,
                            uint32_t image_height, hipStream_t st);
// ... 16 lines not shown
```

cuda-spectral-ray-tracer_amd/csrc/srt_kernel_common.h:

```cpp
#pragma once
#include "srt_device.h"
#include "srt_internal.h"

namespace srt {

constexpr int kLdsUniF4 = 16;
constexpr int kLdsCmfF4 = 96;
constexpr int kLdsTablesF4 = kLdsUniF4 + kLdsCmfF4;

struct LdsUniforms {
    float du[3], dv[3], p00[3], center[3], disk_u[3], disk_v[3], defocus_angle;
    uint32_t width, height, offx, offy, tx, ty, bx, by, tiles_x, n_tiles, rank, world, spp, n_lanes;
    uint32_t n_rows;
    uint32_t lane_limit;
    uint32_t rng[2], tile_out[2], tile_order[2], tile_cost[2], pixel_counter[2];
    uint32_t tile_group_stride;
    uint32_t first_row_taken;
    uint32_t n_assigned_slots;
    uint32_t prio_cost[2], prio_full;
    uint32_t accum_sums[2], spp_total;
    uint32_t accum_sum2[2], accum_state[2], min_spp;
    float rel_tol, abs_tol;
    uint32_t accum_film[2];
    uint32_t streams;
};
static_assert(sizeof(LdsUniforms) <= kLdsUniF4 * 16, "uniform block too large");
typedef __attribute__((address_space(3))) LdsUniforms lds_uniforms;
__device__ __forceinline__ void split_ptr(const void *p, __attribute__((address_space(3))) uint32_t *dst) {
    const unsigned long long v = (unsigned long long)p;
    dst[0] = (uint32_t)v; dst[1] = (uint32_t)(v >> 32);
}
template <typename T>
__device__ __forceinline__ T *join_ptr(uint32_t lo, uint32_t hi) { return reinterpret_cast<T *>(((unsigned long long)hi << 32) | lo); }

constexpr size_t kLdsBudget = 160 * 1024;

#ifndef SRT_PRIO_MODE
#define SRT_PRIO_MODE 1
#endif
#ifndef SRT_ASSIGN_FIRST_ROW
#define SRT_ASSIGN_FIRST_ROW 1
#endif
#ifndef SRT_PRIO_L2
#define SRT_PRIO_L2 0
#endif
#ifndef SRT_PRIO_T1
#define SRT_PRIO_T1 256
#define SRT_PRIO_T2 64
#define SRT_PRIO_T3 16
#endif

__device__ __forceinline__ uint32_t wave_sum(uint32_t v) {
#pragma unroll
    for (int off = 32; off > 0; off >>= 1) v += __shfl_xor(v, off, 64);
    return v;
}

__device__ __forceinline__ uint32_t block_linear_idx(uint32_t i, uint32_t j, uint32_t tx, uint32_t ty, uint32_t bx) {
    uint32_t gbx = i / tx, gby = j / ty;
    uint32_t lx = i - gbx * tx, ly = j - gby * ty;
    return ly * tx + lx + tx * ty * (gby * bx + gbx);
}

struct QueueRow { uint32_t tile_local, part, s; };
__host__ __device__ __forceinline__ uint32_t queue_row_pack(uint32_t tile_local, uint32_t part, uint32_t s) {
    return tile_local | (part << kQueuePartShift) | (s << kQueueLevelShift);
}
__host__ __device__ __forceinline__ QueueRow queue_row_unpack(uint32_t row) {
    return {row & kQueueTileMask, (row >> kQueuePartShift) & kQueuePartMask, (row >> kQueueLevelShift) & kQueueLevelMask};
}
__device__ __forceinline__ bool queue_slot_in_share(uint32_t lt, uint32_t part, uint32_t s) { return (lt >> (6u - s)) == part; }

struct PixelIJ { uint32_t i, j; };
__device__ __forceinline__ uint32_t queue_global_tile(uint32_t tile_local, uint32_t rank, uint32_t world) { return rank + world * tile_local; }
__device__ __forceinline__ PixelIJ tile_slot_pixel(uint32_t tile, uint32_t lt, uint32_t tiles_x) {
    const uint32_t tile_x = tile % tiles_x, tile_y = tile / tiles_x;
    return {tile_x * 8u + (lt & 7u), tile_y * 8u + (lt >> 3)};
}
__device__ __forceinline__ bool queue_slot_in_chunk(uint32_t tile, uint32_t lt, PixelIJ px, uint32_t n_tiles, uint32_t lane_limit, uint32_t width,
                                                    uint32_t height, uint32_t tx, uint32_t ty, uint32_t bx, uint32_t by) {
    return (tile < n_tiles) && (lt < lane_limit) && (px.i < width) && (px.j < height) && (px.i / tx < bx) && (px.j / ty < by);
}

}
```

cuda-spectral-ray-tracer_amd/csrc/srt_kernels.hip:

```cpp
#include <algorithm>
#include <stdlib.h>

#include "srt_color_consts.h"
#include "srt_kernel_common.h"

namespace srt {

#ifndef SRT_INNER_BURST
#define SRT_INNER_BURST 8
#endif
#ifndef SRT_BURST_DROP
#define SRT_BURST_DROP 3
#endif
#ifndef SRT_ASM_BURST
#define SRT_ASM_BURST 2
#endif
#ifndef SRT_INNER_BURST_L2
#define SRT_INNER_BURST_L2 4
#endif
#ifndef SRT_ASM_BURST_L2
#define SRT_ASM_BURST_L2 1
#endif
#ifndef SRT_BURST_DROP_L2
#define SRT_BURST_DROP_L2 2
#endif
constexpr int kInnerBurstL2 = SRT_INNER_BURST_L2;
constexpr uint32_t kBurstDropL2 = SRT_BURST_DROP_L2;
constexpr int kInnerBurst = SRT_INNER_BURST;
constexpr uint32_t kBurstDrop = SRT_BURST_DROP;
static inline size_t round16(size_t v) { return (v + 15) & ~(size_t)15; }
bool render_narrow_refs(int n_records, const PlanKnobs &k) { return !k.wide_refs && n_records <= 32767; }
static inline size_t cache_bytes(int n_cached, bool narrow) { return round16((size_t)n_cached * (narrow ? 52 : 56)); }
static inline size_t stack_slots(int stack_depth) { return (size_t)(stack_depth < 1 ? 1 : stack_depth) + kStackSentinels; }
static inline size_t stack_bytes(int stack_depth, bool narrow) { return stack_slots(stack_depth) * 64 * (narrow ? 2 : 4); }
size_t render_lds_bytes(int stack_depth, int waves_per_block, int n_cached, int n_records, const PlanKnobs &k) {
    const bool narrow = render_narrow_refs(n_records, k);
    return (size_t)kLdsTablesF4 * 16 + cache_bytes(n_cached, narrow) + (size_t)waves_per_block * stack_bytes(stack_depth, narrow);
}
void render_launch_shape(int stack_depth, int n_records, int n_inner, const PlanKnobs &k, int &waves_per_block, int &n_cached) {
    const bool narrow = render_narrow_refs(n_records, k);
    const size_t stack = stack_bytes(stack_depth, narrow);
    waves_per_block = 16;
    while (waves_per_block > 1 && (size_t)kLdsTablesF4 * 16 + waves_per_block * stack + 16 * 1024 > kLdsBudget) waves_per_block /= 2;
    const size_t blocks_per_cu = 16 / waves_per_block;
    const size_t per_block = kLdsBudget / blocks_per_cu;
    const size_t fixed = (size_t)kLdsTablesF4 * 16 + waves_per_block * stack + 64;
    size_t room = per_block > fixed ? (per_block - fixed) / (narrow ? 52 : 56) : 0;
    if (room > (size_t)n_inner) room = (size_t)n_inner;
    if (k.lds_cache_max >= 0) room = std::min(room, (size_t)k.lds_cache_max);
    n_cached = (int)room;
}
void render_launch_plan(int stack_depth, int n_records, int n_inner, const PlanKnobs &k, LaunchPlan &lp) {
    render_launch_shape(stack_depth, n_records, n_inner, k, lp.waves_per_block, lp.n_cached);
    lp.all_cached = lp.n_cached == n_inner;
    lp.waves_per_eu = 4;
    lp.blocks_per_cu = 16 / lp.waves_per_block;
    lp.waves_per_cu = lp.waves_per_block * lp.blocks_per_cu;
}
RenderGrid render_launch_grid(const LaunchPlan &lp, uint32_t n_cu, uint32_t waves_per_cu_override, uint32_t queue_rows_bound) {
    RenderGrid g;
    g.waves_per_block = lp.waves_per_block;
    uint32_t waves_per_cu = (uint32_t)lp.waves_per_cu;
    if (waves_per_cu_override > 0 && waves_per_cu_override < 16 && g.waves_per_block == 16) {
        g.waves_per_block = (int)waves_per_cu_override;
        waves_per_cu = waves_per_cu_override;
    }
    uint32_t n_waves = n_cu * waves_per_cu;
    if (n_waves > queue_rows_bound) n_waves = queue_rows_bound;
    g.n_blocks = (n_waves + (uint32_t)g.waves_per_block - 1) / (uint32_t)g.waves_per_block;
    g.waves = g.n_blocks * (uint32_t)g.waves_per_block;
    return g;
}

#ifndef SRT_PAIRED_VARIANT
#define SRT_PAIRED_VARIANT 1
#endif
bool render_paired_variant(bool tree_is_paired, bool narrow, bool all_cached) { return SRT_PAIRED_VARIANT != 0 && tree_is_paired && narrow == all_cached; }

#ifndef SRT_ASSIGN_PERM
#define SRT_ASSIGN_PERM 0
#endif
__device__ __forceinline__ uint32_t assigned_band(uint32_t w) {
    if (SRT_ASSIGN_PERM == 1) return (w & 3u) * 4u + (w >> 2);
    if (SRT_ASSIGN_PERM == 2) return (w & 4u) ? ((w & ~3u) | (3u - (w & 3u))) : w;
    return w;
}

__global__ void init_rng_kernel(uint32_t *rng, uint32_t n_lanes, uint64_t seed) {
    uint32_t idx = blockIdx.x * blockDim.x + threadIdx.x;
    if (idx >= n_lanes) return;
    Rng s;
    rng_seed(s, seed + idx);
    rng[0 * (size_t)n_lanes + idx] = s.d;
    rng[1 * (size_t)n_lanes + idx] = s.v0;
    rng[2 * (size_t)n_lanes + idx] = s.v1;
    rng[3 * (size_t)n_lanes + idx] = s.v2;
    rng[4 * (size_t)n_lanes + idx] = s.v3;
    rng[5 * (size_t)n_lanes + idx] = s.v4;
}

__device__ __forceinline__ bool adaptive_converged(float s1, float s2, uint32_t n_samples, uint32_t min_spp, float rel_tol, float abs_tol) {
    const float n = (float)n_samples;
    const float mean = s1 / n;
    const float mm = mean * mean;
    float v = s2 / n - mm;
    v = v > 0.0f ? v : 0.0f;
    const float var_mean = v / (n - 1.0f);
    const float tol = rel_tol * mean + abs_tol;
    const float tt = tol * tol;
    const bool finite = __builtin_isfinite(s1) && __builtin_isfinite(s2) && __builtin_isfinite(mm) && __builtin_isfinite(tt);
    return n_samples >= min_spp && finite && var_mean <= tt;
}

template <int MODE, bool NARROW, bool ALL_CACHED, bool PAIRED>
__global__ __launch_bounds__(1024) void render_kernel(const RenderParams P) {
    constexpr bool COUNT = (MODE == 1);
    constexpr bool PROBE = (MODE == 2);
    constexpr bool ITERS = COUNT || PROBE;
    constexpr bool ACCUM = (MODE == 3 || MODE == 4 || MODE == 5 || MODE == 7 || MODE == 8 || MODE == 9);
    constexpr bool ADAPT = (MODE == 4 || MODE == 8);
    constexpr bool FILM = (MODE == 5 || MODE == 9);
    constexpr bool STREAMS = (MODE == 6);
    constexpr bool FEATURES = (MODE == 7 || MODE == 8 || MODE == 9);
    constexpr bool S2_MEM = ADAPT && !NARROW && !ALL_CACHED && !PAIRED;
    extern __shared__ float4 lds4[];
    lds_uniforms *U = (lds_uniforms *)lds4;
    float4 *s_cmf = lds4 + kLdsUniF4;
    constexpr bool narrow = NARROW;
    const uint32_t nc = (uint32_t)P.n_cached;
    float4 *s_q0 = lds4 + kLdsTablesF4, *s_q1 = s_q0 + nc, *s_q2 = s_q1 + nc;
    uint32_t *s_r0 = reinterpret_cast<uint32_t *>(s_q2 + nc), *s_r1 = s_r0 + nc;
    const size_t cache_b = (((size_t)nc * (narrow ? 52u : 56u)) + 15u) & ~(size_t)15u;
    char *s_stack_base = reinterpret_cast<char *>(lds4 + kLdsTablesF4) + cache_b;
    const uint32_t lane = threadIdx.x & 63u;
    const uint32_t wave = threadIdx.x >> 6;

    if (threadIdx.x == 0) {
        for (int a = 0; a < 3; a++) {
            U->du[a] = P.du[a]; U->dv[a] = P.dv[a]; U->p00[a] = P.p00[a]; U->center[a] = P.center[a];
            U->disk_u[a] = P.disk_u[a]; U->disk_v[a] = P.disk_v[a];
        }
        U->defocus_angle = P.defocus_angle;
        U->n_rows = P.queue_rows ? P.queue_rows[0] : P.tiles_local;
        U->lane_limit = P.debug_lane_limit ? P.debug_lane_limit : 64u;
        U->width = P.width; U->height = P.height; U->offx = P.offx; U->offy = P.offy;
        U->tx = P.tx; U->ty = P.ty; U->bx = P.bx; U->by = P.by;
        U->tiles_x = P.tiles_x; U->n_tiles = P.n_tiles; U->rank = P.rank; U->world = P.world; U->spp = P.spp; U->n_lanes = P.n_lanes;
        split_ptr(P.rng, U->rng); split_ptr(P.tile_out, U->tile_out); split_ptr(P.tile_order, U->tile_order);
        split_ptr(P.tile_cost, U->tile_cost); split_ptr(P.pixel_counter, U->pixel_counter);
        U->tile_group_stride = P.tile_group_stride;
        U->n_assigned_slots = gridDim.x * (blockDim.x >> 6) * 64u;
        U->first_row_taken = 0u;
        split_ptr(P.prio_cost, U->prio_cost);
        U->prio_full = __float_as_uint(P.queue_rows && P.prio_cost ? (float)P.queue_rows[1] * (float)P.spp : 0.f);
        if constexpr (ACCUM) {
            const AccumHeader *ah = reinterpret_cast<const AccumHeader *>(P.wave_debug);
            split_ptr(ah->sums, U->accum_sums);
            U->spp_total = ah->spp_total;
        }
        if constexpr (ADAPT) {
            const AccumHeader *ah = reinterpret_cast<const AccumHeader *>(P.wave_debug);
            split_ptr(ah->sum2, U->accum_sum2); split_ptr(ah->state, U->accum_state);
            U->min_spp = ah->min_spp; U->rel_tol = ah->rel_tol; U->abs_tol = ah->abs_tol;
        }
        if constexpr (FILM) split_ptr(reinterpret_cast<const AccumHeader *>(P.wave_debug)->film, U->accum_film);
        if constexpr (FEATURES) {
            const AccumHeader *ah = reinterpret_cast<const AccumHeader *>(P.wave_debug);
            if constexpr (FILM) split_ptr(ah->features, U->accum_sum2);
            else split_ptr(ah->features, U->accum_film);
            if constexpr (ADAPT || FILM) split_ptr(ah->mat_col, U->tile_cost);
            else split_ptr(ah->mat_col, U->accum_sum2);
        }
        if constexpr (STREAMS) {
            const AccumHeader *ah = reinterpret_cast<const AccumHeader *>(P.wave_debug);
            split_ptr(ah->stream_planes, U->accum_sums);
            U->streams = ah->streams;
            U->n_rows *= ah->streams;
        }
    }
    for (uint32_t k = threadIdx.x; k < kLdsCmfF4; k += blockDim.x) s_cmf[k] = P.cmf[k];
    for (uint32_t k = threadIdx.x; k < nc; k += blockDim.x) {
        s_q0[k] = P.nodes[4 * k + 0]; s_q1[k] = P.nodes[4 * k + 1]; s_q2[k] = P.nodes[4 * k + 2];
        const float4 q3 = P.nodes[4 * k + 3];
        const uint32_t lr = __float_as_uint(q3.x), rr = __float_as_uint(q3.y);
        if (narrow) s_r0[k] = (lr & 0xffffu) | (rr << 16);
        else { s_r0[k] = lr; s_r1[k] = rr; }
    }
    __syncthreads();

    NodeSrc ns;
    ns.global_nodes = make_rsrc(P.nodes, (uint32_t)P.n_inner * 64u);
    ns.fringe_stride = ALL_CACHED ? 96u : P.fringe_stride;
    ns.global_fringe = make_rsrc(P.fringe, (uint32_t)(P.n_records - P.n_inner) * ns.fringe_stride);
    ns.global_nodes_sw = make_rsrc(P.nodes_sw, P.nodes_sw ? (uint32_t)P.n_inner * 80u : 0u);
    ns.n_inner = P.n_inner;
    ns.lds_q0 = (lds_cf4 *)s_q0; ns.lds_q1 = (lds_cf4 *)s_q1; ns.lds_q2 = (lds_cf4 *)s_q2;
    ns.lds_r0 = (lds_cu32 *)s_r0; ns.lds_r1 = (lds_cu32 *)s_r1;
    ns.n_cached = P.n_cached;
    const buf_rsrc shade_rsrc = make_rsrc(P.shade, P.n_tris * 48u);
    const buf_rsrc sd_rsrc = make_rsrc(P.mat_sd, (P.n_materials + 1u) * 768u);
    const uint32_t spp = P.spp;
    uint32_t w_shade = P.score_shade, w_fringe = P.score_fringe;
    asm volatile("" : "+s"(w_shade), "+s"(w_fringe));
    StackRef my_stack;
    {
        const size_t slots = (size_t)(P.stack_depth < 1 ? 1 : P.stack_depth) + kStackSentinels;
        my_stack.s16 = (lds_i16 *)(s_stack_base + (size_t)wave * slots * 128u) + lane;
        my_stack.s32 = (lds_i32 *)(s_stack_base + (size_t)wave * slots * 256u) + lane;
        stack_init<NARROW>(my_stack);
    }

    bool dead = false, have_path = false, have_pixel = false;
    uint32_t idx = 0;
    uint32_t out_slot = 0;
    uint32_t pixel_ij = 0;
    Rng rs; rs.d = rs.v0 = rs.v1 = rs.v2 = rs.v3 = rs.v4 = 0u;
    V3 acc = mk(0.f, 0.f, 0.f);
    float acc2 = 0.f;
    uint32_t sample = 0, bounce = 0, valid = 0;
    V3 ro = mk(0.f, 0.f, 0.f), rd = mk(0.f, 0.f, 1.f), inv = mk(0.f, 0.f, 1.f);
    float hero = kLambdaMin;
    float pw[kWavelengths];
#pragma unroll
    for (int k = 0; k < kWavelengths; k++) pw[k] = 0.f;
    Trav tv; tv.node = kTravIdle; tv.sp = 0u; tv.top = -1; tv.c = kFltMax; tv.hit = -1; tv.nf[0] = tv.nf[1] = tv.nf[2] = 0u;
    uint32_t n_rays = 0;
    TravStats ts;
    bool parked = false, exclusive = false;
    OrderProfile prof;
    prof.magic = 0;
    if (COUNT && P.wave_debug) prof = *reinterpret_cast<const OrderProfile *>(P.wave_debug);
    unsigned long long t_shade = 0, t_inner = 0, t_fringe = 0, t_mark = 0;
    if (COUNT) t_mark = __builtin_amdgcn_s_memtime();
    const unsigned long long t_born = t_mark;
    unsigned long long t_dry = 0;
    uint32_t cur_tile_local = 0, pixel_iters0 = 0;
    uint32_t pixel_rays0 = 0, max_pix_iters = 0, max_pix_rays = 0;
    uint32_t w_shade_passes = 0, l_shade = 0, l_cam = 0, w_reject_iters = 0;
    uint32_t n_hits = 0;

    for (;;) {
        if (__ballot(have_pixel) == 0ull) parked = false;
        if (__ballot(!dead && !parked && tv.node < 0) != 0ull) {
            bool end_path = false, begin_trav = false;
            if (COUNT) { w_shade_passes++; l_shade += (uint32_t)__popcll(__ballot(!dead && tv.node == kTravDone)); }
            float xyz_x = 0.0f, xyz_y = 0.0f, xyz_z = 0.0f;

            if (!dead && tv.node == kTravDone) {
                tv.node = kTravIdle;
                float wl[kWavelengths];
                hero_expand(hero, wl);
                uint32_t sd_table = P.n_materials;
                bool was_hit = false, hit_scattered = false;
                if (tv.hit < 0) {
                    end_path = true;
                } else {
                    if (COUNT && P.wave_debug && prof.magic == kOrderProfileMagic) {
                        int k = prof.leaf[tv.hit];
                        for (int guard = 0; guard < 96; guard++) {
                            const int up = prof.up[k];
                            if (up < 0) break;
                            const float *b = prof.sibbox + 6 * (size_t)k;
                            const float x0 = (b[0] - ro.x) * inv.x, x1 = (b[1] - ro.x) * inv.x;
                            const float y0 = (b[2] - ro.y) * inv.y, y1 = (b[3] - ro.y) * inv.y;
                            const float z0 = (b[4] - ro.z) * inv.z, z1 = (b[5] - ro.z) * inv.z;
                            const float e = fmaxf(fmaxf(fmaxf(0.0f, fminf(x0, x1)), fminf(y0, y1)), fminf(z0, z1));
                            const float m = fminf(fminf(fmaxf(x0, x1), fmaxf(y0, y1)), fmaxf(z0, z1));
                            if (e <= m && e > tv.c) atomicAdd(&prof.cnt[up], 1u);
                            k = up >> 1;
                        }
                    }
                    const uint32_t srec = __umul24((uint32_t)tv.hit, 48u);
                    const f4v s0 = buf_load16(shade_rsrc, srec), s1 = buf_load16(shade_rsrc, srec + 16u), s2 = buf_load16(shade_rsrc, srec + 32u);
                    const V3 n_geo = mk(s0.x, s0.y, s0.z);
                    const V3 hp = ro + tv.c * rd;
                    const bool front_face = dot(rd, n_geo) < 0;
                    const V3 n = front_face ? n_geo : -n_geo;
                    const uint32_t mat = __float_as_uint(s0.w);
                    const uint32_t mtype = __float_as_uint(s1.x);
                    const float fuzz = s1.y;

                    V3 scatter_direction = mk(0.f, 0.f, 0.f);
                    float eps_sign = 1.0f;
                    bool did_scatter = true;
                    const V3 unit_in = unit_vector(rd);
                    if (mtype == 4u) {
                        did_scatter = false;
                    } else if (mtype == 2u) {
                        float ir = sellmeier_index(s1.z, s1.w, s2.x, s2.y, s2.z, s2.w, wl[0]);
                        float refraction_ratio = front_face ? (1.0f / ir) : ir;
                        float cos_theta = fminf(dot(-unit_in, n), 1.0f);
                        float sin_theta = sqrtf(1.0f - cos_theta * cos_theta);
                        bool cannot_refract = refraction_ratio * sin_theta > 1.0f;
                        if (!cannot_refract)
                            cannot_refract = reflectance(cos_theta, refraction_ratio) > rng_uniform(rs);
                        if (cannot_refract) {
                            scatter_direction = reflect(unit_in, n);
                        } else {
                            scatter_direction = refract(unit_in, n, refraction_ratio);
                            eps_sign = -1.0f;
                            valid = 1;
                        }
                    } else {
                        const V3 ruv = random_unit_vector(rs);
                        if (mtype == 1u) {
                            V3 reflected = reflect(unit_in, n);
                            scatter_direction = reflected + fuzz * ruv;
                            did_scatter = dot(scatter_direction, n) > 0;
                            if (!did_scatter) valid = 0;
                        } else {
                            scatter_direction = n + ruv;
                            if (near_zero(scatter_direction)) scatter_direction = n;
                        }
                    }
                    if constexpr (FEATURES) {
                        if (bounce == 0u) {
                            const uint32_t rows_lo = (uint32_t)__builtin_amdgcn_readfirstlane((int)(FILM ? U->accum_sum2[0] : U->accum_film[0])), rows_hi = (uint32_t)__builtin_amdgcn_readfirstlane((int)(FILM ? U->accum_sum2[1] : U->accum_film[1]));
                            const uint32_t col_lo = (uint32_t)__builtin_amdgcn_readfirstlane((int)((ADAPT || FILM) ? U->tile_cost[0] : U->accum_sum2[0])), col_hi = (uint32_t)__builtin_amdgcn_readfirstlane((int)((ADAPT || FILM) ? U->tile_cost[1] : U->accum_sum2[1]));
                            float4 *row = join_ptr<float4>(rows_lo, rows_hi) + (size_t)idx * (kFeatureStride / 4u);
                            const buf_rsrc col_rsrc = make_rsrc(join_ptr<const float>(col_lo, col_hi), P.n_materials * 16u);
                            const uint32_t col_off = (mat < P.n_materials ? mat : P.n_materials) * 16u;
                            {
                                float4 f = row[0];
                                const float red = __uint_as_float(__builtin_amdgcn_raw_buffer_load_b32(col_rsrc, (int)col_off, 0, 0));
                                f.x = f.x + n.x; f.y = f.y + n.y; f.z = f.z + n.z; f.w = f.w + red;
                                row[0] = f;
                            }
                            asm volatile("" ::: "memory");
                            {
                                float4 f = row[1];
                                const float2 gb = buf_load8(col_rsrc, col_off + 4u);
                                const float dist = tv.c * sqrtf((rd.x * rd.x + rd.y * rd.y) + rd.z * rd.z);
                                f.x = f.x + gb.x; f.y = f.y + gb.y; f.z = f.z + dist; f.w = f.w + 1.0f;
                                row[1] = f;
                            }
                        }
                    }
                    sd_table = mat;
                    ro = hp + (eps_sign * kEpsilon) * n;
                    rd = scatter_direction;
                    hit_scattered = did_scatter;
                    was_hit = true;
                    if (COUNT) n_hits++;
                }
                const bool ends_here = !was_hit || !hit_scattered;
                const float delta_lambda = (kLambdaMax - kLambdaMin) / (float)kWavelengths;
                const uint32_t sd_base = __umul24(sd_table, 768u);
                int off[kWavelengths];
                float wgt[kWavelengths];
                float2 sp[kWavelengths];
#pragma unroll
                for (int k = 0; k < kWavelengths; k++) {
                    interp_coords(wl[k], off[k], wgt[k]);
                    sp[k] = buf_load8(sd_rsrc, sd_base + (uint32_t)off[k] * 8u);
                }
#pragma unroll
                for (int k = 0; k < kWavelengths; k++) pw[k] *= interp_pair(sp[k], wgt[k]);
                if (ends_here) {
#pragma unroll
                    for (int k = 0; k < kWavelengths; k++) {
                        const float4 r0 = s_cmf[off[k]], r1 = s_cmf[off[k] + 1];
                        const float w = wgt[k], power = (uint32_t)k < valid ? pw[k] : 0.0f;
                        xyz_x += ((1.0f - w) * r0.x + w * r1.x) * power * delta_lambda;
                        xyz_y += ((1.0f - w) * r0.y + w * r1.y) * power * delta_lambda;
                        xyz_z += ((1.0f - w) * r0.z + w * r1.z) * power * delta_lambda;
                    }
                    if constexpr (FILM) {
                        float *row = join_ptr<float>(U->accum_film[0], U->accum_film[1]) + (size_t)idx * kFilmStride;
                        float2 fp[kWavelengths];
#pragma unroll
                        for (int k = 0; k < kWavelengths; k++) __builtin_memcpy(&fp[k], row + off[k], sizeof(float2));
#pragma unroll
                        for (int k = 0; k < kWavelengths; k++) {
                            const float w = wgt[k], power = (uint32_t)k < valid ? pw[k] : 0.0f;
                            fp[k].x = fp[k].x + (1.0f - w) * power;
                            fp[k].y = fp[k].y + w * power;
                            __builtin_memcpy(row + off[k], &fp[k], sizeof(float2));
                        }
                    }
                }
                if (was_hit) {
                    if (!hit_scattered) {
                        end_path = true;
                    } else {
                        bounce++;
                        if (bounce < P.bounce_limit) begin_trav = true;
                        else { valid = 0; end_path = true; }
                    }
                }
            }

            if (end_path) {
                acc = acc + mk(xyz_x, xyz_y, xyz_z);
                if constexpr (S2_MEM) {
                    float *s2 = join_ptr<float>(U->accum_sum2[0], U->accum_sum2[1]) + idx;
                    *s2 = *s2 + xyz_y * xyz_y;
                } else if constexpr (ADAPT) {
                    acc2 = acc2 + xyz_y * xyz_y;
                }
                have_path = false;
            }

            const bool switched_any = SRT_PRIO_MODE != 0 && (ALL_CACHED || SRT_PRIO_L2) && __ballot(!dead && !parked && tv.node < 0 && !have_path && !begin_trav && (!have_pixel || sample == spp)) != 0ull;
            if (!dead && !parked && tv.node < 0 && !have_path && !begin_trav && (!have_pixel || sample == spp)) {
                if (have_pixel && PROBE) {
                    uint32_t *tcost = join_ptr<uint32_t>(U->tile_cost[0], U->tile_cost[1]);
                    atomicAdd(tcost + cur_tile_local, ts.n_iters - pixel_iters0 + 1u);
                    atomicMax(tcost + P.tiles_local + cur_tile_local, ts.n_iters - pixel_iters0 + 1u);
                    have_pixel = false;
                }
                if (have_pixel && COUNT) { max_pix_iters = max(max_pix_iters, ts.n_iters - pixel_iters0); max_pix_rays = max(max_pix_rays, n_rays - pixel_rays0); }
                if constexpr (STREAMS) {
                    if (have_pixel) {
                        const size_t nl0 = U->n_lanes, nlk = nl0 * U->streams;
                        const bool stream0 = idx < nl0;
                        uint32_t *planes = join_ptr<uint32_t>(U->accum_sums[0], U->accum_sums[1]);
                        uint32_t *rng = stream0 ? join_ptr<uint32_t>(U->rng[0], U->rng[1]) : planes;
                        const size_t nl = stream0 ? nl0 : nlk;
                        rng[0 * nl + idx] = rs.d; rng[1 * nl + idx] = rs.v0; rng[2 * nl + idx] = rs.v1;
                        rng[3 * nl + idx] = rs.v2; rng[4 * nl + idx] = rs.v3; rng[5 * nl + idx] = rs.v4;
                        float *sums = reinterpret_cast<float *>(planes + kStreamSumPlane * nlk);
                        sums[0 * nlk + idx] = acc.x; sums[1 * nlk + idx] = acc.y; sums[2 * nlk + idx] = acc.z;
                        have_pixel = false;
                    }
                }
                if (have_pixel && !PROBE && !STREAMS) {
                    {
                        uint32_t *rng = join_ptr<uint32_t>(U->rng[0], U->rng[1]);
                        const size_t nl = U->n_lanes;
                        rng[0 * nl + idx] = rs.d; rng[1 * nl + idx] = rs.v0; rng[2 * nl + idx] = rs.v1;
                        rng[3 * nl + idx] = rs.v2; rng[4 * nl + idx] = rs.v3; rng[5 * nl + idx] = rs.v4;
                    }
                    if constexpr (ACCUM) {
                        float *sums = join_ptr<float>(U->accum_sums[0], U->accum_sums[1]);
                        const size_t nl = U->n_lanes;
                        sums[0 * nl + idx] = acc.x; sums[1 * nl + idx] = acc.y; sums[2 * nl + idx] = acc.z;
                    }
                    if constexpr (ADAPT) {
                        float *s2 = join_ptr<float>(U->accum_sum2[0], U->accum_sum2[1]) + idx;
                        if constexpr (S2_MEM) acc2 = *s2;
                        else *s2 = acc2;
                        const uint32_t total = U->spp_total;
                        const bool stop = adaptive_converged(acc.y, acc2, total, U->min_spp, U->rel_tol, U->abs_tol);
                        join_ptr<uint32_t>(U->accum_state[0], U->accum_state[1])[idx] = total | (stop ? kAdaptConverged : 0u);
                    }
                    const float inv_spp = 1.0f / (float)(ACCUM ? U->spp_total : spp);
                    const V3 c = inv_spp * acc;
                    const float r_lin = (SRT_XYZ2RGB_00 * c.x) + (SRT_XYZ2RGB_01 * c.y) + (SRT_XYZ2RGB_02 * c.z);
                    const float g_lin = (SRT_XYZ2RGB_10 * c.x) + (SRT_XYZ2RGB_11 * c.y) + (SRT_XYZ2RGB_12 * c.z);
                    const float b_lin = (SRT_XYZ2RGB_20 * c.x) + (SRT_XYZ2RGB_21 * c.y) + (SRT_XYZ2RGB_22 * c.z);
                    const float r = correct_channel(r_lin), g = correct_channel(g_lin), b = correct_channel(b_lin);
                    float *o = join_ptr<float>(U->tile_out[0], U->tile_out[1]) + out_slot;
                    const size_t gs = U->tile_group_stride;
                    o[0 * kTileLanes] = (float)(int)(r * 255.99f);
                    o[1 * kTileLanes] = (float)(int)(g * 255.99f);
                    o[2 * kTileLanes] = (float)(int)(b * 255.99f);
                    if (P.write_parity) {
                        o[gs + 0 * kTileLanes] = r; o[gs + 1 * kTileLanes] = g; o[gs + 2 * kTileLanes] = b;
                        o[2 * gs + 0 * kTileLanes] = acc.x; o[2 * gs + 1 * kTileLanes] = acc.y; o[2 * gs + 2 * kTileLanes] = acc.z;
                    }
                    have_pixel = false;
                }
                bool searching = true;
                if (exclusive) { parked = true; exclusive = false; searching = false; }
                while (searching) {
                    const unsigned long long m = __ballot(1);
                    const int leader = __ffsll((long long)m) - 1;
                    uint32_t base = 0;
                    const bool row_open = SRT_ASSIGN_FIRST_ROW != 0 && ((U->first_row_taken >> wave) & 1u) == 0u;
                    if (COUNT && row_open && m != ~0ull && lane == (uint32_t)leader) atomicAdd(&P.counters[23], 1ull);
                    const bool assigned = row_open && m == ~0ull;
                    if (assigned) {
                        if (lane == 0) atomicOr((unsigned int *)&U->first_row_taken, 1u << wave);
                        base = (assigned_band(wave) * gridDim.x + blockIdx.x) * 64u;
                    }
                    else {
                        if ((int)lane == leader) base = atomicAdd(join_ptr<uint32_t>(U->pixel_counter[0], U->pixel_counter[1]), (uint32_t)__popcll(m));
                        base = (uint32_t)__shfl((int)base, leader, 64) + (SRT_ASSIGN_FIRST_ROW != 0 ? U->n_assigned_slots : 0u);
                    }
                    const uint32_t pix = base + (uint32_t)__popcll(m & ((1ull << lane) - 1ull));
                    if (pix >= U->n_rows * 64u) { dead = true; searching = false; if (COUNT && t_dry == 0) t_dry = __builtin_amdgcn_s_memtime(); }
                    else {
                        const uint32_t *tile_order = join_ptr<const uint32_t>(U->tile_order[0], U->tile_order[1]);
                        QueueRow qr;
                        uint32_t tile_local, stream = 0u;
                        if constexpr (STREAMS) {
                            const uint32_t src_row = (pix >> 6) / U->streams;
                            stream = (pix >> 6) - src_row * U->streams;
                            qr = queue_row_unpack(tile_order ? tile_order[src_row] : 0u);
                            tile_local = tile_order ? qr.tile_local : src_row;
                        } else {
                            qr = queue_row_unpack(tile_order ? tile_order[pix >> 6] : 0u);
                            tile_local = tile_order ? qr.tile_local : (pix >> 6);
                        }
                        const uint32_t row_s = qr.s;
                        const uint32_t lt = pix & 63u;
                        const bool whole_wave = m == ~0ull;
                        if (!queue_slot_in_share(lt, qr.part, row_s)) {
                            if (whole_wave) { parked = true; searching = false; }
                            continue;
                        }
                        exclusive = whole_wave && row_s != 0u;
                        const uint32_t tile = queue_global_tile(tile_local, U->rank, U->world);
                        const PixelIJ px = tile_slot_pixel(tile, lt, U->tiles_x);
                        const uint32_t i = px.i, j = px.j;
                        const uint32_t gtx = U->tx, gty = U->ty, gbx = U->bx;
                        if ((tile < U->n_tiles) && (lt < U->lane_limit) && (i < U->width) && (j < U->height) && (i / gtx < gbx) && (j / gty < U->by)) {
                            if constexpr (ADAPT) {
                                const uint32_t *state = join_ptr<const uint32_t>(U->accum_state[0], U->accum_state[1]);
                                if (state[block_linear_idx(i, j, gtx, gty, gbx)] & kAdaptConverged) continue;
                            }
                            idx = block_linear_idx(i, j, gtx, gty, gbx);
                            out_slot = tile_local * (uint32_t)(kGroupPlanes * kTileLanes) + lt;
                            pixel_ij = i | (j << 16);
                            if constexpr (STREAMS) {
                                const size_t nl0 = U->n_lanes, nlk = nl0 * U->streams;
                                idx += stream * U->n_lanes;
                                const bool stream0 = stream == 0u;
                                const uint32_t *planes = join_ptr<const uint32_t>(U->accum_sums[0], U->accum_sums[1]);
                                const uint32_t *rng = stream0 ? join_ptr<const uint32_t>(U->rng[0], U->rng[1]) : planes;
                                const size_t nl = stream0 ? nl0 : nlk;
                                rs.d = rng[0 * nl + idx]; rs.v0 = rng[1 * nl + idx]; rs.v1 = rng[2 * nl + idx];
                                rs.v2 = rng[3 * nl + idx]; rs.v3 = rng[4 * nl + idx]; rs.v4 = rng[5 * nl + idx];
                                const float *sums = reinterpret_cast<const float *>(planes + kStreamSumPlane * nlk);
                                acc = mk(sums[0 * nlk + idx], sums[1 * nlk + idx], sums[2 * nlk + idx]);
                            } else {
                                const uint32_t *rng = join_ptr<const uint32_t>(U->rng[0], U->rng[1]);
                                const size_t nl = U->n_lanes;
                                rs.d = rng[0 * nl + idx]; rs.v0 = rng[1 * nl + idx]; rs.v1 = rng[2 * nl + idx];
                                rs.v2 = rng[3 * nl + idx]; rs.v3 = rng[4 * nl + idx]; rs.v4 = rng[5 * nl + idx];
                            }
                            if constexpr (STREAMS) {
                            } else if constexpr (ACCUM) {
                                const float *sums = join_ptr<const float>(U->accum_sums[0], U->accum_sums[1]);
                                const size_t nl = U->n_lanes;
                                acc = mk(sums[0 * nl + idx], sums[1 * nl + idx], sums[2 * nl + idx]);
                                if constexpr (ADAPT && !S2_MEM) acc2 = join_ptr<const float>(U->accum_sum2[0], U->accum_sum2[1])[idx];
                            } else {
                                acc = mk(0.f, 0.f, 0.f);
                            }
                            sample = 0;
                            if (PROBE) { cur_tile_local = tile_local; pixel_iters0 = ts.n_iters; }
                            if (COUNT) { pixel_iters0 = ts.n_iters; pixel_rays0 = n_rays; }
                            have_pixel = true;
                            searching = false;
                        }
                    }
                }
                __builtin_amdgcn_s_waitcnt(0x0070);
            }

#if SRT_PRIO_MODE
            if (!PROBE && (ALL_CACHED || SRT_PRIO_L2) && switched_any) {
                float rem = 0.f;
                const uint32_t *tc = join_ptr<const uint32_t>(U->prio_cost[0], U->prio_cost[1]);
                if (tc && have_pixel && !dead) rem = (float)tc[out_slot / (uint32_t)(kGroupPlanes * kTileLanes)] * (float)(spp - sample);
#pragma unroll
                for (int off = 32; off > 0; off >>= 1) rem = fmaxf(rem, __shfl_xor(rem, off, 64));
                const float full = __uint_as_float(U->prio_full);
                const uint32_t pr = (uint32_t)__builtin_amdgcn_readfirstlane((int)((rem > (SRT_PRIO_T1 / 1024.0f) * full ? 1u : 0u) + (rem > (SRT_PRIO_T2 / 1024.0f) * full ? 1u : 0u) + (rem > (SRT_PRIO_T3 / 1024.0f) * full ? 1u : 0u)));
                if (pr == 0u) __builtin_amdgcn_s_setprio(0);
                else if (pr == 1u) __builtin_amdgcn_s_setprio(1);
                else if (pr == 2u) __builtin_amdgcn_s_setprio(2);
                else __builtin_amdgcn_s_setprio(3);
            }
#endif

            if (COUNT) l_cam += (uint32_t)__popcll(__ballot(!dead && tv.node < 0 && !have_path && !begin_trav && have_pixel && sample < spp));
            if (!dead && tv.node < 0 && !have_path && !begin_trav && have_pixel && sample < spp) {
                float px = -0.5f + rng_uniform(rs);
                float py = -0.5f + rng_uniform(rs);
                const V3 du = mk(U->du[0], U->du[1], U->du[2]), dv = mk(U->dv[0], U->dv[1], U->dv[2]);
                const V3 cam_center = mk(U->center[0], U->center[1], U->center[2]);
                const V3 pixel_center = (mk(U->p00[0], U->p00[1], U->p00[2]) + (float)(U->offx + (pixel_ij & 0xffffu)) * du) + (float)(U->offy + (pixel_ij >> 16)) * dv;
                V3 pixel_sample = pixel_center + (px * du + py * dv);
                V3 origin = cam_center;
                if (!(U->defocus_angle <= 0.0f)) {
                    float dx, dy;
#if SRT_ASM_RNG
                    rng_disk_loop_asm(rs, dx, dy);
#else
                    for (;;) {
                        dx = rng_pm1(rs);
                        dy = rng_pm1(rs);
                        if ((dx * dx + dy * dy) + 0.0f * 0.0f < 1.0f) break;
                    }
#endif
                    origin = (cam_center + dx * mk(U->disk_u[0], U->disk_u[1], U->disk_u[2])) +
                             dy * mk(U->disk_v[0], U->disk_v[1], U->disk_v[2]);
                }
                ro = origin;
                rd = pixel_sample - origin;
                hero = hero_draw(rs);
#pragma unroll
                for (int k = 0; k < kWavelengths; k++) pw[k] = 1.0f;
                valid = kWavelengths;
                sample++;
                bounce = 0;
                have_path = true;
                if (P.bounce_limit > 0) begin_trav = true;
                else { valid = 0;
                       have_path = false;  }
            }

            if (begin_trav) {
                n_rays++;
                inv = mk(1.0f / rd.x, 1.0f / rd.y, 1.0f / rd.z);
                ray_near_addresses(ns, inv, tv.nf);
                (void)trav_begin<ITERS>(tv, stack_base<NARROW>(my_stack), P.tris, P.root_ref, ro, rd, ts);
            }
        }

        if (COUNT) { const unsigned long long now = __builtin_amdgcn_s_memtime(); t_shade += now - t_mark; t_mark = now; }
        if (__ballot(!dead) == 0ull) break;
        const unsigned long long alive_mask = __ballot(!dead && !parked);
        if (alive_mask == 0ull) continue;
        const uint32_t n_alive = (uint32_t)__popcll(alive_mask);
        const uint32_t n_inner_u = (uint32_t)P.n_inner;
        if (!COUNT && n_alive == 1u) {
            while (__ballot(tv.node >= 0) != 0ull) {
                if (tv.node >= 0) {
                    if ((uint32_t)tv.node < n_inner_u) trav_step_inner<ITERS, NARROW, ALL_CACHED>(tv, ns, ro, inv, my_stack, ts);
                    else trav_step_fringe<ITERS, NARROW, PAIRED>(tv, ns, ro, rd, inv, my_stack, ts);
                }
            }
            continue;
        }
        if (!ITERS && NARROW && ALL_CACHED && kInnerBurst == 8 && kBurstDrop == 3u && SRT_ASM_BURST == 2) {
            while (inner_phase_asm(tv, ns, ro, inv, n_inner_u, n_alive, w_shade, w_fringe) != 0u) {
                if (tv.node >= (int)n_inner_u) trav_step_fringe<ITERS, NARROW, PAIRED>(tv, ns, ro, rd, inv, my_stack, ts);
            }
        } else
        for (;;) {
            const unsigned long long trav_mask = __ballot(tv.node >= 0);
            if (trav_mask == 0ull) break;
            const unsigned long long fringe_mask = __ballot(tv.node >= (int)n_inner_u);
            const uint32_t n_trav = (uint32_t)__popcll(trav_mask), n_fringe = (uint32_t)__popcll(fringe_mask);
            const uint32_t s_sh = (n_alive - n_trav) * P.score_shade;
            const uint32_t s_fr = n_fringe * P.score_fringe;
            const uint32_t s_in = (n_trav - n_fringe) << 8;
            if (s_sh > max(s_fr, s_in)) break;
            const bool do_fringe = s_fr > s_in;
            if (COUNT) { ts.w_iters++; ts.w_alive += n_alive; if (do_fringe) { ts.w_fringe++; ts.l_fringe += n_fringe; } else ts.l_inner += n_trav - n_fringe; }
            if (do_fringe) {
                if (tv.node >= (int)n_inner_u) trav_step_fringe<ITERS, NARROW, PAIRED>(tv, ns, ro, rd, inv, my_stack, ts);
                if (COUNT) { const unsigned long long now = __builtin_amdgcn_s_memtime(); t_fringe += now - t_mark; t_mark = now; }
            } else {
                bool at_inner = (uint32_t)tv.node < n_inner_u;
                constexpr int burst_len = ALL_CACHED ? kInnerBurst : kInnerBurstL2;
                constexpr uint32_t burst_drop = ALL_CACHED ? kBurstDrop : kBurstDropL2;
                const uint32_t stay = (n_trav - n_fringe + burst_drop - 1u) / burst_drop;
                if (!ITERS && NARROW && ALL_CACHED && kInnerBurst == 8 && SRT_ASM_BURST == 1) {
                    inner_burst8_asm(tv, ns, ro, inv, n_inner_u, stay);
                } else if (!ITERS && !NARROW && !ALL_CACHED && kInnerBurstL2 == 4 && SRT_ASM_BURST_L2 && P.nodes_sw != nullptr) {
                    inner_burst4_mixed_asm(tv, ns, ro, inv, n_inner_u, stay);
                } else
#pragma unroll
                for (int burst = 0; burst < burst_len; burst++) {
                    if (at_inner) trav_step_inner<ITERS, NARROW, ALL_CACHED>(tv, ns, ro, inv, my_stack, ts);
                    at_inner = (uint32_t)tv.node < n_inner_u;
                    const unsigned long long m = __ballot(at_inner);
                    if (COUNT && burst > 0) { ts.w_iters++; ts.w_alive += n_alive; }
                    if (COUNT && burst < burst_len - 1) ts.l_inner += (uint32_t)__popcll(m);
                    if ((uint32_t)__popcll(m) < stay) break;
                }
                if (COUNT) { const unsigned long long now = __builtin_amdgcn_s_memtime(); t_inner += now - t_mark; t_mark = now; }
            }
        }
    }

    {
        uint32_t r = wave_sum(n_rays);
        if (!PROBE && lane == 0 && r) atomicAdd(&P.counters[0], (unsigned long long)r);
        if (COUNT) {
            uint32_t a = wave_sum(ts.n_iters), b = wave_sum(ts.n_tri), c = wave_sum(ts.n_box);
            if (lane == 0) {
                atomicAdd(&P.counters[1], (unsigned long long)a);
                atomicAdd(&P.counters[2], (unsigned long long)b);
                atomicAdd(&P.counters[3], (unsigned long long)c);
                atomicAdd(&P.counters[4], (unsigned long long)ts.w_iters);
                atomicAdd(&P.counters[5], (unsigned long long)ts.w_alive);
            }
            const uint32_t nn = wave_sum(ts.n_nan), nh = wave_sum(n_hits);
            if (lane == 0) {
                atomicAdd(&P.counters[24], (unsigned long long)nh);
                atomicAdd(&P.counters[6], (unsigned long long)nn);
                atomicAdd(&P.counters[7], (unsigned long long)ts.w_fringe);
                atomicAdd(&P.counters[8], (unsigned long long)ts.l_fringe);
                atomicAdd(&P.counters[9], (unsigned long long)ts.l_inner);
                atomicAdd(&P.counters[10], t_shade);
            }
            const unsigned long long t_end = __builtin_amdgcn_s_memtime();
            uint32_t dry_first = t_dry ? (uint32_t)((t_dry - t_born) >> 8) : 0xffffffffu;
#pragma unroll
            for (int off = 32; off > 0; off >>= 1) dry_first = min(dry_first, (uint32_t)__shfl_xor((int)dry_first, off, 64));
            uint32_t wave_max_pix_rays = max_pix_rays;
#pragma unroll
            for (int off = 32; off > 0; off >>= 1) wave_max_pix_rays = max(wave_max_pix_rays, (uint32_t)__shfl_xor((int)wave_max_pix_rays, off, 64));
            atomicMax(&P.counters[13], (unsigned long long)max_pix_iters);
            atomicMax(&P.counters[14], (unsigned long long)max_pix_rays);
            if (lane == 0) {
                atomicAdd(&P.counters[11], t_inner);
                atomicAdd(&P.counters[12], t_fringe);
                atomicAdd(&P.counters[15], (unsigned long long)w_shade_passes);
                atomicAdd(&P.counters[16], (unsigned long long)l_shade);
                atomicAdd(&P.counters[17], (unsigned long long)l_cam);
                atomicAdd(&P.counters[18], (unsigned long long)w_reject_iters);
                if (P.wave_debug) {
                    uint32_t *w = P.wave_debug + sizeof(OrderProfile) / 4u + 4u * (blockIdx.x * (blockDim.x >> 6) + wave);
                    w[0] = (uint32_t)((t_end - t_born) >> 8); w[1] = dry_first; w[2] = r; w[3] = wave_max_pix_rays;
                }
                atomicAdd(&P.counters[19], 1ull);
                atomicAdd(&P.counters[20], t_end - t_born);
                atomicMax(&P.counters[21], t_end - t_born);
                atomicAdd(&P.counters[22], dry_first != 0xffffffffu ? (t_end - t_born) - ((unsigned long long)dry_first << 8) : 0ull);
            }
        }
    }
}

__global__ __launch_bounds__(1024) void order_tiles_kernel(const uint32_t *__restrict__ cost, uint32_t *__restrict__ sorted,
                                                          uint32_t *__restrict__ rows, uint32_t n, uint32_t n_waves,
                                                          uint32_t split_load_pct, uint32_t *__restrict__ queue_info, uint32_t order_max_pct) {
    constexpr uint32_t kBinsN = 4096;
    __shared__ uint32_t s_bin[kBinsN];
    __shared__ uint32_t s_max;
    __shared__ unsigned long long s_sum;
    __shared__ uint32_t s_scan[1024];
    __shared__ float s_load;
    const uint32_t t = threadIdx.x;
    if (t == 0) { s_max = 1u; s_sum = 0ull; }
    for (uint32_t b = t; b < kBinsN; b += 1024) s_bin[b] = 0u;
    __syncthreads();
    auto key_of = [&](uint32_t k) -> uint32_t {
        const uint32_t c = cost[k];
        if (order_max_pct == 0u) return c;
        const unsigned long long mx64 = (unsigned long long)cost[n + k] * 64ull;
        const unsigned long long key = mx64 > c ? c + (mx64 - c) * order_max_pct / 100ull : c;
        return key > 0xffffffffull ? 0xffffffffu : (uint32_t)key;
    };
    __shared__ uint32_t s_kmax;
    if (t == 0) s_kmax = 1u;
    uint32_t m = 0, km = 0;
    unsigned long long sum = 0;
    for (uint32_t k = t; k < n; k += 1024) { m = max(m, cost[k]); km = max(km, key_of(k)); sum += cost[k]; }
    atomicMax(&s_max, m);
    atomicAdd(&s_sum, sum);
    __syncthreads();
    atomicMax(&s_kmax, km);
    __syncthreads();
    const float scale = (float)(kBinsN - 1) / (float)s_kmax;
    auto bin_of = [&](uint32_t c) { uint32_t b = (uint32_t)((float)c * scale); b = b > kBinsN - 1 ? kBinsN - 1 : b; return (kBinsN - 1) - b; };
    for (uint32_t k = t; k < n; k += 1024) atomicAdd(&s_bin[bin_of(key_of(k))], 1u);
    __syncthreads();
    if (t == 0) {
        uint32_t acc = 0;
        for (uint32_t b = 0; b < kBinsN; b++) { const uint32_t c = s_bin[b]; s_bin[b] = acc; acc += c; }
    }
    __syncthreads();
    for (uint32_t k = t; k < n; k += 1024) sorted[atomicAdd(&s_bin[bin_of(key_of(k))], 1u)] = k;
    __syncthreads();

    const float g[7] = {1.0f, 0.934f, 0.925f, 0.797f, 0.747f, 0.656f, 0.485f};
    auto level_for = [&](uint32_t c, float target) {
        uint32_t s = 0;
        while (s < 6u && (float)c * g[s] > target) s++;
        return s;
    };
    auto lat_of = [&](uint32_t k) -> uint32_t { return cost[k]; };
    const bool may_split = split_load_pct != 0u && n <= (1u << 20);
    float target = 3.0e38f;
    if (may_split) {
        const float load_factor = (float)split_load_pct * 0.01f;
        const float lat_max = (float)s_max;
        float lo_t = lat_max * g[6], hi_t = fmaxf(lat_max, load_factor * (float)s_sum / (float)(n_waves ? n_waves : 1u));
        for (int it = 0; it < 14; it++) {
            const float mid = 0.5f * (lo_t + hi_t);
            float load = 0.f;
            for (uint32_t k = t; k < n; k += 1024) { const uint32_t c = lat_of(k); const uint32_t s = level_for(c, mid); load += (float)(1u << s) * (float)c * g[s]; }
            if (t == 0) s_load = 0.f;
            __syncthreads();
            atomicAdd(&s_load, load);
            __syncthreads();
            const bool feasible = load_factor * s_load <= (float)n_waves * mid;
            __syncthreads();
            if (feasible) hi_t = mid; else lo_t = mid;
        }
        target = hi_t;
    }
    auto level_of = [&](uint32_t k) { return may_split ? level_for(lat_of(k), target) : 0u; };
    const uint32_t per = (n + 1023u) / 1024u;
    const uint32_t lo = min(n, t * per), hi = min(n, lo + per);
    uint32_t mine = 0;
    for (uint32_t k = lo; k < hi; k++) mine += 1u << level_of(sorted[k]);
    s_scan[t] = mine;
    __syncthreads();
    if (t == 0) {
        uint32_t acc = 0;
        for (uint32_t b = 0; b < 1024u; b++) { const uint32_t c = s_scan[b]; s_scan[b] = acc; acc += c; }
        queue_info[0] = acc;
        queue_info[1] = s_max;
    }
    __syncthreads();
    uint32_t at = s_scan[t];
    for (uint32_t k = lo; k < hi; k++) {
        const uint32_t tile = sorted[k], s = level_of(tile);
        for (uint32_t part = 0; part < (1u << s); part++) rows[at++] = queue_row_pack(tile, part, s);
    }
}

__global__ __launch_bounds__(64) void scatter_tiles_kernel(const ScatterParams P) {
    const uint32_t tile = blockIdx.x;
    const uint32_t lane = threadIdx.x;
    const PixelIJ px = tile_slot_pixel(tile, lane, P.tiles_x);
    if (!queue_slot_in_chunk(tile, lane, px, P.n_tiles, kTileLanes, P.width, P.height, P.tx, P.ty, P.bx, P.by)) return;
    const uint32_t idx = block_linear_idx(px.i, px.j, P.tx, P.ty, P.bx);
    const uint32_t rank = tile % P.world, local = tile / P.world;
    for (uint32_t g = 0; g < P.groups; g++) {
        const float *src = P.gathered + (((size_t)rank * P.groups + g) * P.tiles_padded + local) * (kGroupPlanes * kTileLanes) + lane;
#pragma unroll
        for (int p = 0; p < kGroupPlanes; p++) P.fb[g * kGroupPlanes + p][idx] = src[p * kTileLanes];
    }
}

__global__ void unswizzle_kernel(const float *r, const float *g, const float *b, float *dr, float *dg, float *db, uint32_t tx,
                                 uint32_t ty, uint32_t bx, uint32_t by, uint32_t n_cols, uint32_t n_rows, uint32_t offx,
                                 uint32_t offy, uint32_t image_width, uint32_t image_height) {
    const uint32_t idx = blockIdx.x * blockDim.x + threadIdx.x;
    const uint32_t block_size = tx * ty;
    if (idx >= block_size * bx * by) return;
    const uint32_t blk = idx / block_size, thread_idx = idx % block_size;
    const uint32_t block_x = blk % bx, block_y = blk / bx;
    uint32_t fb_x = tx * block_x + thread_idx % tx;
    uint32_t fb_y = ty * block_y + thread_idx / tx;
    if (fb_x < n_cols && fb_y < n_rows) {
        fb_x += offx; fb_y += offy;
        if (fb_x < image_width && fb_y < image_height) {
            const size_t o = (size_t)fb_y * image_width + fb_x;
// ... 167 lines not shown

hipError_t launch_trace(const RenderParams &p, const float *rays, size_t n, float *out, hipStream_t st) {
    if (n == 0) return hipSuccess;
    const size_t lds = stack_slots(p.stack_depth) * 64 * 4;
    hipLaunchKernelGGL(trace_rays_kernel, dim3((uint32_t)((n + 63) / 64)), dim3(64), lds, st, p, rays, (uint32_t)n, out);
    return hipGetLastError();
}

hipError_t launch_op_sweep(int which, const float *a, const float *b, size_t n, float *out, hipStream_t st) {
    if (n == 0) return hipSuccess;
    hipLaunchKernelGGL(op_sweep_kernel, dim3((uint32_t)((n + 255) / 256)), dim3(256), 0, st, which, a, b, (uint32_t)n, out);
    return hipGetLastError();
}

template <int>
__global__ void accum_header_kernel(AccumHeader *dst, float *sums, uint32_t spp_total) {
    if (threadIdx.x == 0) { dst->sums = sums; dst->spp_total = spp_total; dst->pad = 0u; }
}

hipError_t launch_accum_header(AccumHeader *dst, float *sums, uint32_t spp_total, hipStream_t st) {
    hipLaunchKernelGGL(accum_header_kernel<0>, dim3(1), dim3(64), 0, st, dst, sums, spp_total);
    return hipGetLastError();
}

template <int>
__global__ __launch_bounds__(256) void adapt_flag_kernel(const AdaptQueueParams P) {
    const uint32_t lane = threadIdx.x & 63u;
    const uint32_t wave = (blockIdx.x * blockDim.x + threadIdx.x) >> 6, n_waves = (gridDim.x * blockDim.x) >> 6;
    const uint32_t n_rows = P.src_info ? P.src_info[0] : P.n_identity;
    uint32_t rendered = 0, active = 0;
    for (uint32_t r = wave; r < n_rows; r += n_waves) {
        const QueueRow qr = P.src_rows ? queue_row_unpack(P.src_rows[r]) : QueueRow{r, 0u, 0u};
        const uint32_t tile = queue_global_tile(qr.tile_local, P.rank, P.world);
        const PixelIJ px = tile_slot_pixel(tile, lane, P.tiles_x);
        bool rend = false, act = false;
        if (queue_slot_in_share(lane, qr.part, qr.s) && queue_slot_in_chunk(tile, lane, px, P.n_tiles, P.lane_limit, P.width, P.height, P.tx, P.ty, P.bx, P.by)) {
            const uint32_t st = P.state[block_linear_idx(px.i, px.j, P.tx, P.ty, P.bx)];
            rend = (st & ~kAdaptConverged) == P.spp_total;
            act = rend && (st & kAdaptConverged) == 0u;
        }
        const unsigned long long ma = __ballot(act);
        rendered += (uint32_t)__popcll(__ballot(rend));
        active += (uint32_t)__popcll(ma);
        if (lane == 0) P.flags[r] = ma != 0ull ? 1u : 0u;
    }
    if (lane == 0 && rendered) atomicAdd(P.counts, (unsigned long long)rendered | ((unsigned long long)active << 32));
}

template <int>
__global__ __launch_bounds__(1024) void adapt_scan_kernel(const AdaptQueueParams P) {
    __shared__ uint32_t s_scan[1024];
    const uint32_t t = threadIdx.x;
    const uint32_t n = P.src_info ? P.src_info[0] : P.n_identity;
    const uint32_t per = (n + 1023u) / 1024u;
    const uint32_t lo = min(n, t * per), hi = min(n, lo + per);
    uint32_t mine = 0;
    for (uint32_t k = lo; k < hi; k++) mine += P.flags[k];
    s_scan[t] = mine;
    __syncthreads();
    if (t == 0) {
        uint32_t acc = 0;
        for (uint32_t b = 0; b < 1024u; b++) { const uint32_t c = s_scan[b]; s_scan[b] = acc; acc += c; }
        P.dst_info[0] = acc;
        P.dst_info[1] = P.src_info ? P.src_info[1] : 0u;
    }
    __syncthreads();
    uint32_t at = s_scan[t];
    for (uint32_t k = lo; k < hi; k++)
        if (P.flags[k]) P.dst_rows[at++] = P.src_rows ? P.src_rows[k] : k;
}

hipError_t launch_adapt_queue(const AdaptQueueParams &p, uint32_t n_rows_bound, hipStream_t st) {
    const uint32_t waves = n_rows_bound < 1u ? 1u : (n_rows_bound > 4096u ? 4096u : n_rows_bound);
    hipLaunchKernelGGL(adapt_flag_kernel<0>, dim3((waves + 3u) / 4u), dim3(256), 0, st, p);
    hipLaunchKernelGGL(adapt_scan_kernel<0>, dim3(1), dim3(1024), 0, st, p);
    return hipGetLastError();
}

template <int>
__global__ __launch_bounds__(256) void film_unswizzle_kernel(const float *film, float *dst, uint32_t first, uint32_t count, uint32_t w,
                                                             uint32_t h, uint32_t tx, uint32_t ty, uint32_t bx) {
    const size_t t = (size_t)blockIdx.x * blockDim.x + threadIdx.x;
    if (t >= (size_t)w * h * count) return;
    const size_t pix = t / count;
    const uint32_t s = (uint32_t)(t - pix * count);
    const uint32_t y = (uint32_t)(pix / w), x = (uint32_t)(pix - (size_t)y * w);
    dst[t] = film[(size_t)block_linear_idx(x, y, tx, ty, bx) * kFilmStride + first + s];
}

hipError_t launch_film_unswizzle(const float *film, float *dst, uint32_t first, uint32_t count, uint32_t w, uint32_t h, uint32_t tx,
                                 uint32_t ty, uint32_t bx, hipStream_t st) {
    const size_t n = (size_t)w * h * count;
    if (n == 0) return hipSuccess;
    hipLaunchKernelGGL(film_unswizzle_kernel<0>, dim3((uint32_t)((n + 255) / 256)), dim3(256), 0, st, film, dst, first, count, w, h, tx, ty, bx);
    return hipGetLastError();
}

template <int>
__global__ __launch_bounds__(256) void stream_combine_kernel(const StreamCombineParams P) {
    const uint32_t lane = threadIdx.x & 63u;
    const uint32_t tile_local = (blockIdx.x * blockDim.x + threadIdx.x) >> 6;
    if (tile_local >= P.tiles_local) return;
    const uint32_t tile = queue_global_tile(tile_local, P.rank, P.world);
    const PixelIJ px = tile_slot_pixel(tile, lane, P.tiles_x);
    if (!queue_slot_in_chunk(tile, lane, px, P.n_tiles, P.lane_limit, P.width, P.height, P.tx, P.ty, P.bx, P.by)) return;
    const uint32_t idx = block_linear_idx(px.i, px.j, P.tx, P.ty, P.bx);
    const size_t nl = P.n_lanes, nlk = nl * P.streams;
    V3 acc = mk(P.stream_sums[0 * nlk + idx], P.stream_sums[1 * nlk + idx], P.stream_sums[2 * nlk + idx]);
    for (uint32_t k = 1; k < P.streams; k++) {
        const size_t at = (size_t)k * nl + idx;
        acc = acc + mk(P.stream_sums[0 * nlk + at], P.stream_sums[1 * nlk + at], P.stream_sums[2 * nlk + at]);
    }
    P.sums[0 * nl + idx] = acc.x; P.sums[1 * nl + idx] = acc.y; P.sums[2 * nl + idx] = acc.z;
    const float inv_spp = 1.0f / (float)P.spp_total;
    const V3 c = inv_spp * acc;
    const float r_lin = (SRT_XYZ2RGB_00 * c.x) + (SRT_XYZ2RGB_01 * c.y) + (SRT_XYZ2RGB_02 * c.z);
    const float g_lin = (SRT_XYZ2RGB_10 * c.x) + (SRT_XYZ2RGB_11 * c.y) + (SRT_XYZ2RGB_12 * c.z);
    const float b_lin = (SRT_XYZ2RGB_20 * c.x) + (SRT_XYZ2RGB_21 * c.y) + (SRT_XYZ2RGB_22 * c.z);
    const float r = correct_channel(r_lin), g = correct_channel(g_lin), b = correct_channel(b_lin);
    float *o = P.tile_out + (size_t)tile_local * (uint32_t)(kGroupPlanes * kTileLanes) + lane;
    const size_t gs = P.tile_group_stride;
    o[0 * kTileLanes] = (float)(int)(r * 255.99f);
    o[1 * kTileLanes] = (float)(int)(g * 255.99f);
    o[2 * kTileLanes] = (float)(int)(b * 255.99f);
    if (P.write_parity) {
        o[gs + 0 * kTileLanes] = r; o[gs + 1 * kTileLanes] = g; o[gs + 2 * kTileLanes] = b;
        o[2 * gs + 0 * kTileLanes] = acc.x; o[2 * gs + 1 * kTileLanes] = acc.y; o[2 * gs + 2 * kTileLanes] = acc.z;
    }
}

hipError_t launch_stream_combine(const StreamCombineParams &p, hipStream_t st) {
    if (p.tiles_local == 0) return hipSuccess;
    hipLaunchKernelGGL(stream_combine_kernel<0>, dim3((p.tiles_local + 3u) / 4u), dim3(256), 0, st, p);
    return hipGetLastError();
}

template <int>
__global__ __launch_bounds__(256) void features_unswizzle_kernel(const float4 *rows, float4 *dst, uint32_t w, uint32_t h, uint32_t tx, uint32_t ty, uint32_t bx) {
    const size_t pix = (size_t)blockIdx.x * blockDim.x + threadIdx.x;
    if (pix >= (size_t)w * h) return;
    const uint32_t y = (uint32_t)(pix / w), x = (uint32_t)(pix - (size_t)y * w);
    const size_t src = (size_t)block_linear_idx(x, y, tx, ty, bx) * (kFeatureStride / 4u);
    dst[2 * pix + 0] = rows[src + 0]; dst[2 * pix + 1] = rows[src + 1];
}

hipError_t launch_features_unswizzle(const float *rows, float *dst, uint32_t w, uint32_t h, uint32_t tx, uint32_t ty, uint32_t bx, hipStream_t st) {
    const size_t n = (size_t)w * h;
    if (n == 0) return hipSuccess;
    hipLaunchKernelGGL(features_unswizzle_kernel<0>, dim3((uint32_t)((n + 255) / 256)), dim3(256), 0, st, reinterpret_cast<const float4 *>(rows),
                       reinterpret_cast<float4 *>(dst), w, h, tx, ty, bx);
    return hipGetLastError();
}

}
```

cuda-spectral-ray-tracer_amd/renderer.py:

```python
import contextlib
import ctypes as C

import numpy as np

from . import binding as B

DEFAULT_TX, DEFAULT_TY = 28, 16
FEATURE_CHANNELS = 8
FILM_SAMPLES = 95


def reference_grid(chunk_w, chunk_h, tx=DEFAULT_TX, ty=DEFAULT_TY):
    return chunk_w // tx + 1, chunk_h // ty + 1


class Renderer:
    def __init__(self, device=0, _borrowed=None):
        if _borrowed is not None:
            self._h, self._owned = C.c_void_p(_borrowed), False
            self.device = B.lib().srt_ctx_device(self._h)
        else:
            h = C.c_void_p()
            B.check(B.lib().srt_create(int(device), C.byref(h)))
            self._h, self._owned = h, True
# ... 209 lines not shown

    def denoise_mv(self, image_width, image_height, **cfg):
        c = denoise_vg_config(**cfg)
        out = [np.zeros((image_height, image_width, 3), np.float32) for _ in range(3)]
        var = np.zeros((image_height, image_width, 2), np.float32)
        self._ck(B.lib().srt_denoise_features_mv(self._h, C.byref(c), B.fptr(out[0]), B.fptr(out[1]), B.fptr(out[2]), B.fptr(var), image_width, image_height))
        return dict(xyz=out[0], lin=out[1], fb=out[2], var=var)

    def denoise_mv_kat(self, xyz_sums, features, samples, sum_y2, **cfg):
        c = denoise_vg_config(**cfg)
        sums = np.ascontiguousarray(xyz_sums, np.float32)
        rows = np.ascontiguousarray(features, np.float32)
        if sums.ndim != 3 or sums.shape[2] != 3 or rows.shape != sums.shape[:2] + (FEATURE_CHANNELS,):
            raise ValueError("denoise_mv_kat: needs xyz_sums (h, w, 3) and features (h, w, %d), got %r and %r" % (FEATURE_CHANNELS, sums.shape, rows.shape))
        n_in = np.asarray(samples)
        s2 = np.ascontiguousarray(sum_y2, np.float32)
        if n_in.shape != sums.shape[:2] or s2.shape != sums.shape[:2]:
            raise ValueError("denoise_mv_kat: samples and sum_y2 must be (h, w) = %r, got %r and %r" % (sums.shape[:2], n_in.shape, s2.shape))
        if n_in.dtype.kind not in "iu" or (n_in < 1).any() or (n_in > 0x7fffffff).any():
            raise ValueError("denoise_mv_kat: samples must be whole numbers in [1, 2^31 - 1] (every pixel holds at least one sample)")
        n = np.ascontiguousarray(n_in, np.uint32)
        out = np.zeros(sums.shape, np.float32)
        var = np.zeros(sums.shape[:2] + (2,), np.float32)
        self._ck(B.lib().srt_denoise_mv_kat(self._h, C.byref(c), B.fptr(sums), B.fptr(rows), n.ctypes.data_as(C.POINTER(C.c_uint32)), B.fptr(s2),
                                            sums.shape[1], sums.shape[0], B.fptr(out), B.fptr(var)))
        return out, var

    def denoise_estimate_last_ms(self):
        ms = C.c_float()
        self._ck(B.lib().srt_denoise_estimate_last_ms(self._h, C.byref(ms)))
        return ms.value

    def accum_reset_streams(self, k):
        self._ck(B.lib().srt_accum_reset_streams(self._h, int(k)))

    @property
    def accum_streams(self):
        n = C.c_uint32()
        self._ck(B.lib().srt_accum_streams(self._h, C.byref(n)))
        return n.value

    def set_gather_planes(self, planes):
        self._ck(B.lib().srt_set_gather_planes(self._h, planes))
        self.gather_planes = planes

    def tile_buffer(self):
        ptr, n, tl, tp = C.c_void_p(), C.c_size_t(), C.c_uint32(), C.c_uint32()
        self._ck(B.lib().srt_tile_buffer(self._h, C.byref(ptr), C.byref(n), C.byref(tl), C.byref(tp)))
        return ptr.value, n.value, tl.value, tp.value

    def copy_tile_buffer(self, dst_ptr, stream=None):
        self._ck(B.lib().srt_copy_tile_buffer(self._h, C.c_void_p(dst_ptr), C.c_void_p(stream or 0)))

    def scatter_tiles(self, gathered_ptr=None, stream=None):
        self._ck(B.lib().srt_scatter_tiles(self._h, C.c_void_p(gathered_ptr or 0), C.c_void_p(stream or 0)))

    def dev_fb(self):
        r, g, b, n = C.c_void_p(), C.c_void_p(), C.c_void_p(), C.c_size_t()
        self._ck(B.lib().srt_dev_fb(self._h, C.byref(r), C.byref(g), C.byref(b), C.byref(n)))
        return r.value, g.value, b.value, n.value

    def read_fb(self):
        n = self.geom["n_lanes"]
        r, g, b = (np.zeros(n, np.float32) for _ in range(3))
        self._ck(B.lib().srt_read_fb(self._h, B.fptr(r), B.fptr(g), B.fptr(b)))
        return r, g, b

    def read_fb_aux(self, which):
        n = self.geom["n_lanes"]
        r, g, b = (np.zeros(n, np.float32) for _ in range(3))
        self._ck(B.lib().srt_read_fb_aux(self._h, which, B.fptr(r), B.fptr(g), B.fptr(b)))
        return r, g, b

    def read_fb_rowmajor(self, image_width, image_height, into=None):
        if into is None:
            into = tuple(np.zeros(image_width * image_height, np.float32) for _ in range(3))
        r, g, b = into
        self._ck(B.lib().srt_read_fb_rowmajor(self._h, B.fptr(r), B.fptr(g), B.fptr(b), image_width, image_height))
        return r, g, b

    def tile_costs(self, with_max_pixel=False):
        _, _, tl, _ = self.tile_buffer()
        out = np.zeros(tl * (2 if with_max_pixel else 1), np.uint32)
        self._ck(B.lib().srt_get_tile_costs(self._h, out.ctypes.data_as(C.POINTER(C.c_uint32)), out.size))
        return (out[:tl], out[tl:]) if with_max_pixel else out

    def order_children_by_profile(self, scene, width, height, spp, bounce_limit, min_samples=4):
        n = C.c_uint32(0)
        self._ck(B.lib().srt_order_children_by_profile(self._h, scene.handle, width, height, spp, bounce_limit, min_samples, C.byref(n)))
        return n.value

    def stats(self):
        st = B.Stats()
        self._ck(B.lib().srt_get_stats(self._h, C.byref(st)))
        d = {k: getattr(st, k) for k in ("rays", "paths", "node_visits", "tri_tests", "box_tests")}
        d["util"] = list(st.util)
        d["shade"] = list(st.shade)
        d["waves"] = list(st.waves)
        d["hits"] = st.hits
        d["max_pixel_node_visits"], d["max_pixel_rays"] = st.reserved[0], st.reserved[1]
        return d

    def wave_debug(self):
        n = int(self.stats()["waves"][0])
        out = np.zeros((n, 4), np.uint32)
        if n:
            self._ck(B.lib().srt_get_wave_debug(self._h, out.ctypes.data_as(C.POINTER(C.c_uint32)), n))
        return out

    def last_kernel_ms(self):
        ms = C.c_float()
        self._ck(B.lib().srt_last_kernel_ms(self._h, C.byref(ms)))
        return ms.value

    def calibrate(self, kind, waves_per_simd=4, iters=20000):
        cal = B.Calibration()
        self._ck(B.lib().srt_calibrate(self._h, kind, waves_per_simd, iters, C.byref(cal)))
        n_simd = cal.n_cu * 4
        total = cal.instr_per_wave * cal.n_waves
        clock_ghz = cal.wave_cycles_max / (cal.wall_ms * 1e-3) / 1e9
        return dict(kind=kind, waves_per_simd=cal.waves_per_simd, n_cu=cal.n_cu, wave_cycles_min=cal.wave_cycles_min,
                    wave_cycles_mean=cal.wave_cycles_mean, wave_cycles_max=cal.wave_cycles_max, wall_ms=cal.wall_ms,
                    instr_per_wave=cal.instr_per_wave,
                    instr_per_cycle_per_simd=cal.instr_per_wave * cal.waves_per_simd / cal.wave_cycles_max,
                    instr_per_cycle_per_simd_mean_wave=cal.instr_per_wave * cal.waves_per_simd / cal.wave_cycles_mean,
                    instr_per_s=total / (cal.wall_ms * 1e-3), clock_ghz=clock_ghz, n_simd=n_simd)

    def trace_rays(self, rays):
        rays = np.ascontiguousarray(rays, np.float32).reshape(-1, 6)
        out = np.zeros((rays.shape[0], 4), np.float32)
        self._ck(B.lib().srt_trace_rays(self._h, B.fptr(rays), rays.shape[0], B.fptr(out)))
        return out

    def op_sweep(self, which, a, b):
        a = np.ascontiguousarray(a, np.float32); b = np.ascontiguousarray(b, np.float32)
        out = np.zeros_like(a)
        self._ck(B.lib().srt_device_op_sweep(self._h, which, B.fptr(a), B.fptr(b), a.size, B.fptr(out)))
        return out

    def order_tiles_kat(self, cost, n_waves, split_load_pct=200, order_max_pct=0, guard=64):
        cost = np.ascontiguousarray(cost, np.uint32)
        n = cost.size // 2
        u32p = C.POINTER(C.c_uint32)
        rows, order, info = np.zeros(64 * n + guard, np.uint32), np.zeros(n, np.uint32), np.zeros(4, np.uint32)
        self._ck(B.lib().srt_order_tiles_kat(self._h, cost.ctypes.data_as(u32p), n, int(n_waves), int(split_load_pct), int(order_max_pct),
                                             rows.ctypes.data_as(u32p), rows.size, order.ctypes.data_as(u32p), info.ctypes.data_as(u32p)))
        return rows, order, info

    def tile_schedule(self, which=0):
        _, _, tl, _ = self.tile_buffer()
        rows, info = np.zeros(64 * tl, np.uint32), B.TileScheduleInfo()
        self._ck(B.lib().srt_read_tile_schedule(self._h, int(which), rows.ctypes.data_as(C.POINTER(C.c_uint32)), rows.size, C.byref(info)))
        return rows[:info.n_rows].copy(), {name: getattr(info, name) for name, _ in B.TileScheduleInfo._fields_ if name != "reserved"}


class Comm:

    def __init__(self, handle, renderers, owns):
        self._h, self.renderers, self._owns = handle, renderers, owns
        self.world = B.lib().srt_comm_world(handle)

    @staticmethod
    def available():
        return B.lib().srt_comm_available() == 0

    @staticmethod
    def unique_id():
        buf = (C.c_ubyte * B.COMM_ID_BYTES)()
        B.check_comm(B.lib().srt_comm_unique_id(buf))
        return bytes(buf)

    @classmethod
    def init_all(cls, devices):
        arr = (C.c_int * len(devices))(*devices)
        h = C.c_void_p()
        B.check_comm(B.lib().srt_comm_init_all(arr, len(devices), C.byref(h)))
        rs = [Renderer(_borrowed=B.lib().srt_comm_ctx(h, k)) for k in range(B.lib().srt_comm_local_count(h))]
        return cls(h, rs, True)

    @classmethod
    def init_rank(cls, renderer, comm_id, rank, world):
        buf = (C.c_ubyte * B.COMM_ID_BYTES).from_buffer_copy(comm_id)
        h = C.c_void_p()
        B.check_comm(B.lib().srt_comm_init_rank(renderer._h, buf, rank, world, C.byref(h)))
        return cls(h, [renderer], False)

    def close(self):
        if getattr(self, "_h", None):
            B.lib().srt_comm_destroy(self._h)
            self._h = None
            for r in self.renderers:
                if not r._owned:
                    r._h = None

    def __del__(self):
        try:
            self.close()
        except Exception:
            pass

    def _ck(self, code):
        return B.check_comm(code, self._h)

    @property
    def root(self):
        p = B.lib().srt_comm_root_ctx(self._h)
        for r in self.renderers:
            if r._h and r._h.value == p:
                return r
        return None

    def upload_scene(self, scene):
        self._ck(B.lib().srt_comm_upload_scene(self._h, scene.handle))

    def set_camera(self, cam):
        self._ck(B.lib().srt_comm_set_camera(self._h, C.byref(cam)))

    def init_device_params(self, chunk_w, chunk_h, spp, bounce_limit, seed=1984, tx=DEFAULT_TX, ty=DEFAULT_TY, bx=None, by=None):
        if bx is None or by is None:
            bx, by = reference_grid(chunk_w, chunk_h, tx, ty)
        self._ck(B.lib().srt_comm_init_device_params(self._h, tx, ty, bx, by, chunk_w, chunk_h, spp, bounce_limit, seed))
        for r in self.renderers:
            r.geom = dict(tx=tx, ty=ty, bx=bx, by=by, chunk_w=chunk_w, chunk_h=chunk_h, n_lanes=tx * ty * bx * by)

    def set_gather_planes(self, planes):
        self._ck(B.lib().srt_comm_set_gather_planes(self._h, planes))
        for r in self.renderers:
            r.gather_planes = planes

    def last_gather_ms(self):
        ms = C.c_float()
        self._ck(B.lib().srt_comm_last_gather_ms(self._h, C.byref(ms)))
        return ms.value

    def render_frame(self, width, height, offx=0, offy=0):
        self._ck(B.lib().srt_render_frame_multi(self._h, width, height, offx, offy))

    def accum_reset(self):
        self._ck(B.lib().srt_comm_accum_reset(self._h))

    def accum_reset_adaptive(self, rel_tol, abs_tol=0.0, min_spp=16):
        self._ck(B.lib().srt_comm_accum_reset_adaptive(self._h, C.byref(adaptive_config(rel_tol, abs_tol, min_spp))))

    @property
    def accum_active(self):
        n = C.c_uint64()
        self._ck(B.lib().srt_comm_accum_active(self._h, C.byref(n)))
        return n.value

    def accum_reset_spectral(self):
        self._ck(B.lib().srt_comm_accum_reset_spectral(self._h))

    def accum_reset_features(self):
        self._ck(B.lib().srt_comm_accum_reset_features(self._h))

    def accum_reset_adaptive_features(self, rel_tol, abs_tol=0.0, min_spp=16):
        self._ck(B.lib().srt_comm_accum_reset_adaptive_features(self._h, C.byref(adaptive_config(rel_tol, abs_tol, min_spp))))

    def accum_reset_spectral_features(self):
        self._ck(B.lib().srt_comm_accum_reset_spectral_features(self._h))

    def accum_reset_streams(self, k):
        self._ck(B.lib().srt_comm_accum_reset_streams(self._h, int(k)))

    def read_spectral(self, image_width, image_height, first=0, count=None):
        count = FILM_SAMPLES - first if count is None else count
        out = None
        for r in self.renderers:
            f = r.read_spectral(image_width, image_height, first, count)
            out = f if out is None else out + f
        return out

    def develop_spectral(self, image_width, image_height, response, scale=1.0, filter=None):
        resp = sensor_response(response, filter)
        out = None
        for r in self.renderers:
            d = r.develop_spectral(image_width, image_height, resp, scale)
            out = d if out is None else out + d
        return out

    def render_frame_accum(self, width, height, spp_add, offx=0, offy=0):
        self._ck(B.lib().srt_render_frame_multi_accum(self._h, width, height, offx, offy, spp_add))

    def synchronize(self):
        self._ck(B.lib().srt_comm_synchronize(self._h))

    def stats(self):
        rays, paths, ms = C.c_uint64(), C.c_uint64(), C.c_float()
        self._ck(B.lib().srt_comm_stats(self._h, C.byref(rays), C.byref(paths), C.byref(ms)))
        return dict(rays=rays.value, paths=paths.value, max_kernel_ms=ms.value)


def pixels_per_lane(renderer, width, height, world=1):
    out = C.c_double()
    renderer._ck(B.lib().srt_pixels_per_lane(renderer._h, width, height, max(world, 1), C.byref(out)))
    return out.value


def tree_tuning(renderer, scene, width, height, bounce_limit, world=1, gate=False):
    t = B.TreeTuning()
    renderer._ck(B.lib().srt_tune_tree_for_throughput(renderer._h, scene.handle, width, height, max(world, 1), bounce_limit, 1 if gate else 0, C.byref(t)))
    return {name: getattr(t, name) for name, _ in B.TreeTuning._fields_}


def tune_tree_for_throughput(renderer, scene, width, height, bounce_limit, world=1, gate=False):
    t = tree_tuning(renderer, scene, width, height, bounce_limit, world, gate)
# ... 420 lines not shown
```

include/srt_c_api.h:

```cpp
#ifndef SRT_C_API_H
#define SRT_C_API_H

#include <stddef.h>
#include <stdint.h>

#ifdef __cplusplus
extern "C" {
#endif

#define SRT_API __attribute__((visibility("default")))

#define SRT_N_CIE_SAMPLES 95
#define SRT_N_RAY_WAVELENGTHS 7
#define SRT_DEFAULT_SEED 1984u
#define SRT_DEFAULT_TX 28u
#define SRT_DEFAULT_TY 16u

typedef enum {
    SRT_OK = 0,
    SRT_ERR_INVALID = -1,
    SRT_ERR_NO_DEVICE = -2,
    SRT_ERR_HIP = -3,
    SRT_ERR_BVH = -4,
    SRT_ERR_UNSUPPORTED = -5,
// ... 45 lines not shown
SRT_API int srt_camera_init(int image_width, int image_height, float vfov, const float lookfrom[3], const float lookat[3],
                            const float vup[3], float defocus_angle, float focus_dist, srt_camera_data *out);

SRT_API srt_scene *srt_scene_create(void);
SRT_API srt_scene *srt_scene_builtin(int scene_id, uint64_t seed);
SRT_API void srt_scene_destroy(srt_scene *s);
SRT_API int srt_scene_default_camera(const srt_scene *s, int image_width, int image_height, srt_camera_data *out);

SRT_API int srt_scene_set_triangles(srt_scene *s, const srt_tri_in *tris, size_t n);
SRT_API int srt_scene_set_materials(srt_scene *s, const srt_material *mats, size_t m);
SRT_API int srt_scene_set_background(srt_scene *s, const float spectrum[SRT_N_CIE_SAMPLES]);
SRT_API size_t srt_scene_tri_count(const srt_scene *s);
SRT_API size_t srt_scene_material_count(const srt_scene *s);
SRT_API int srt_scene_get_triangles(const srt_scene *s, srt_tri_in *out);
SRT_API int srt_scene_get_materials(const srt_scene *s, srt_material *out);
SRT_API int srt_scene_get_background(const srt_scene *s, float out[SRT_N_CIE_SAMPLES]);
SRT_API int srt_scene_get_tri_records(const srt_scene *s, float *out);

SRT_API int srt_material_bake(srt_material *m);
SRT_API int srt_set_reference_quirks(int on);
SRT_API int srt_bake_sigmoid_spectrum(const float coeffs[3], float scale, int times_d65, float out[SRT_N_CIE_SAMPLES]);
SRT_API int srt_fit_sigmoid_coeffs(const float rgb[3], float coeffs[3]);
SRT_API int srt_color_tables(float cmf[SRT_N_CIE_SAMPLES * 4], float xyz_to_srgb[9]);
SRT_API int srt_background_spectrum(const float rgb[3], float out[SRT_N_CIE_SAMPLES]);

SRT_API int srt_rotation_matrix(float theta, int axis, float m[9]);

SRT_API int srt_scene_build_bvh(srt_scene *s, int mode, uint64_t seed);
SRT_API int srt_scene_order_children(srt_scene *s, const float eye[3]);
SRT_API int srt_scene_optimise_bvh(srt_scene *s, int passes);
SRT_API int srt_scene_is_paired(const srt_scene *s);
SRT_API size_t srt_scene_node_count(const srt_scene *s);
SRT_API int srt_scene_bvh_depth(const srt_scene *s);
SRT_API int srt_scene_get_bvh(const srt_scene *s, int32_t *left, int32_t *right, int32_t *prim, float *boxes);

SRT_API int srt_create(int device, srt_ctx **out);
SRT_API void srt_destroy(srt_ctx *ctx);
SRT_API const char *srt_last_error(const srt_ctx *ctx);

SRT_API int srt_upload_scene(srt_ctx *ctx, const srt_scene *s);
SRT_API int srt_set_camera(srt_ctx *ctx, const srt_camera_data *cam);
SRT_API int srt_launch_plan(const srt_ctx *ctx, int *waves_per_cu, int *n_cached, int *all_cached, int *narrow_refs);
SRT_API int srt_launch_paired(const srt_ctx *ctx, int *paired);
SRT_API int srt_set_test_knobs(srt_ctx *ctx, int wide_refs, int lds_cache_max, uint32_t lane_limit);
SRT_API int srt_get_test_knobs(const srt_ctx *ctx, int *wide_refs, int *lds_cache_max, uint32_t *lane_limit, int *from_env);
SRT_API int srt_launch_lds_bytes(const srt_ctx *ctx, size_t *bytes);
SRT_API int srt_init_device_params(srt_ctx *ctx, uint32_t tx, uint32_t ty, uint32_t bx, uint32_t by, uint32_t chunk_w,
                                   uint32_t chunk_h, uint32_t spp, uint32_t bounce_limit, uint64_t seed);
SRT_API int srt_set_partition(srt_ctx *ctx, uint32_t rank, uint32_t world);

SRT_API int srt_render_chunk(srt_ctx *ctx, uint32_t width, uint32_t height, uint32_t offx, uint32_t offy, void *stream);
SRT_API int srt_synchronize(srt_ctx *ctx);

SRT_API int srt_accum_reset(srt_ctx *ctx);
SRT_API int srt_render_chunk_accum(srt_ctx *ctx, uint32_t width, uint32_t height, uint32_t offx, uint32_t offy, uint32_t spp_add, void *stream);
SRT_API int srt_accum_samples(const srt_ctx *ctx, uint32_t *spp_total);

typedef struct { float rel_tol, abs_tol; uint32_t min_spp, reserved; } srt_adaptive;
SRT_API int srt_accum_reset_adaptive(srt_ctx *ctx, const srt_adaptive *cfg);
SRT_API int srt_accum_active(srt_ctx *ctx, uint64_t *active);
SRT_API int srt_read_accum_stats(srt_ctx *ctx, uint32_t *samples, float *sum_y, float *sum_y2, uint32_t image_width, uint32_t image_height);

SRT_API int srt_accum_reset_spectral(srt_ctx *ctx);
SRT_API int srt_read_spectral(srt_ctx *ctx, uint32_t first, uint32_t count, float *out, uint32_t image_width, uint32_t image_height);

#define SRT_MAX_DEVELOP_CHANNELS 16
SRT_API int srt_develop_spectral(srt_ctx *ctx, const float *response, uint32_t channels, float scale, float *out,
                                 uint32_t image_width, uint32_t image_height);
SRT_API int srt_develop_spectral_srgb(srt_ctx *ctx, const float *response3, float scale, float *out_xyz, float *out_lin, float *out_q,
                                      uint32_t image_width, uint32_t image_height);
SRT_API int srt_develop_kat(srt_ctx *ctx, const float *film, uint32_t n_pixels, const float *response, uint32_t channels, float scale,
                            float *out);
SRT_API int srt_develop_last_ms(srt_ctx *ctx, float *contract_ms, float *epilogue_ms);

SRT_API int srt_accum_reset_features(srt_ctx *ctx);
SRT_API int srt_read_features(srt_ctx *ctx, float *out, uint32_t image_width, uint32_t image_height);

SRT_API int srt_accum_reset_adaptive_features(srt_ctx *ctx, const srt_adaptive *cfg);

SRT_API int srt_accum_reset_spectral_features(srt_ctx *ctx);

typedef struct srt_denoise { uint32_t levels; float sigma_color, sigma_normal, sigma_albedo, sigma_depth; uint32_t reserved[3]; } srt_denoise;
SRT_API int srt_denoise_features(srt_ctx *ctx, const srt_denoise *cfg, float *out_xyz, float *out_lin, float *out_q,
                                 uint32_t image_width, uint32_t image_height);
SRT_API int srt_denoise_kat(srt_ctx *ctx, const srt_denoise *cfg, const float *xyz_sums, const float *features,
                            uint32_t samples, uint32_t w, uint32_t h, float *out_xyz);
SRT_API int srt_denoise_last_ms(srt_ctx *ctx, float *prepass_ms, float level_ms[8], float *epilogue_ms, uint32_t *levels);

typedef struct srt_denoise_vg { uint32_t levels; float sigma_variance, sigma_normal, sigma_albedo, sigma_depth, variance_floor; uint32_t reserved[2]; } srt_denoise_vg;
SRT_API int srt_denoise_features_vg(srt_ctx *ctx, const srt_denoise_vg *cfg, float *out_xyz, float *out_lin, float *out_q, float *out_var,
                                    uint32_t image_width, uint32_t image_height);
SRT_API int srt_denoise_vg_kat(srt_ctx *ctx, const srt_denoise_vg *cfg, const float *xyz_sums, const float *features,
                               uint32_t samples, uint32_t w, uint32_t h, float *out_xyz, float *out_var);
SRT_API int srt_denoise_estimate_last_ms(srt_ctx *ctx, float *ms);

SRT_API int srt_denoise_features_mv(srt_ctx *ctx, const srt_denoise_vg *cfg, float *out_xyz, float *out_lin, float *out_q, float *out_var,
                                    uint32_t image_width, uint32_t image_height);
SRT_API int srt_denoise_mv_kat(srt_ctx *ctx, const srt_denoise_vg *cfg, const float *xyz_sums, const float *features,
                               const uint32_t *samples, const float *sum_y2, uint32_t w, uint32_t h, float *out_xyz, float *out_var);

SRT_API int srt_denoise_developed(srt_ctx *ctx, const srt_denoise *cfg, const float *response, uint32_t channels, float scale,
                                  float *out_dev, float *out_xyz, uint32_t image_width, uint32_t image_height);
SRT_API int srt_denoise_developed_kat(srt_ctx *ctx, const srt_denoise *cfg, const float *xyz_sums, const float *features,
                                      const float *developed, uint32_t channels, uint32_t samples, uint32_t w, uint32_t h,
                                      float *out_dev, float *out_xyz);

#define SRT_MAX_STREAMS 16
SRT_API int srt_accum_reset_streams(srt_ctx *ctx, uint32_t streams);
SRT_API int srt_accum_streams(const srt_ctx *ctx, uint32_t *streams);

SRT_API int srt_set_gather_planes(srt_ctx *ctx, uint32_t planes);
SRT_API int srt_tile_buffer(srt_ctx *ctx, void **dev_ptr, size_t *n_floats, uint32_t *tiles_local, uint32_t *tiles_padded);
SRT_API int srt_copy_tile_buffer(srt_ctx *ctx, void *dst_dev, void *stream);
SRT_API int srt_scatter_tiles(srt_ctx *ctx, const void *dev_gathered, void *stream);

SRT_API int srt_dev_fb(srt_ctx *ctx, void **r, void **g, void **b, size_t *n_floats);
SRT_API int srt_read_fb(srt_ctx *ctx, float *r, float *g, float *b);
SRT_API int srt_read_fb_rowmajor(srt_ctx *ctx, float *r, float *g, float *b, uint32_t image_width, uint32_t image_height);
SRT_API int srt_read_fb_aux(srt_ctx *ctx, int which, float *p0, float *p1, float *p2);

SRT_API int srt_get_tile_costs(srt_ctx *ctx, uint32_t *out, size_t n);
SRT_API int srt_order_children_by_profile(srt_ctx *ctx, srt_scene *scene, uint32_t width, uint32_t height, uint32_t spp,
                                          uint32_t bounce_limit, uint32_t min_samples, uint32_t *n_swapped);
SRT_API int srt_pixels_per_lane(const srt_ctx *ctx, uint32_t width, uint32_t height, uint32_t world, double *out);
typedef struct srt_tree_tuning {
    double   pixels_per_lane;
    uint32_t throughput_bound;
    uint32_t reinsertion;
    uint32_t probe_width, probe_height, probe_spp;
    uint32_t nodes_swapped;
    int32_t  order_status;
} srt_tree_tuning;
SRT_API int srt_tune_tree_for_throughput(srt_ctx *ctx, srt_scene *scene, uint32_t width, uint32_t height, uint32_t world,
                                         uint32_t bounce_limit, int only_if_throughput_bound, srt_tree_tuning *out);
SRT_API int srt_get_stats(srt_ctx *ctx, srt_stats *out);
SRT_API int srt_set_count_traversal(srt_ctx *ctx, int on);
SRT_API int srt_get_wave_debug(srt_ctx *ctx, uint32_t *out, size_t n_waves);
SRT_API int srt_last_kernel_ms(srt_ctx *ctx, float *ms);
SRT_API int srt_trace_rays(srt_ctx *ctx, const float *rays, size_t n, float *out);
SRT_API int srt_device_op_sweep(srt_ctx *ctx, int which, const float *a, const float *b, size_t n, float *out);
SRT_API int srt_order_tiles_kat(srt_ctx *ctx, const uint32_t *cost, uint32_t n, uint32_t n_waves, uint32_t split_load_pct,
                                uint32_t order_max_pct, uint32_t *rows_out, size_t rows_cap, uint32_t *sorted_out, uint32_t *info_out);
typedef struct srt_tile_schedule_info {
    uint32_t tiles_local;
    uint32_t n_rows;
    uint32_t cost_max;
    uint32_t n_waves_plan;
    uint32_t split_load_pct;
    uint32_t order_max_pct;
    uint32_t streams;
    uint32_t reserved;
} srt_tile_schedule_info;
SRT_API int srt_read_tile_schedule(srt_ctx *ctx, int which, uint32_t *rows_out, size_t rows_cap, srt_tile_schedule_info *info);

SRT_API int srt_ctx_device(const srt_ctx *ctx);
SRT_API int srt_ctx_cu_count(const srt_ctx *ctx);

#define SRT_COMM_ID_BYTES 128
typedef struct srt_comm srt_comm;
SRT_API int srt_comm_init_all(const int *devices, int n, srt_comm **out);
SRT_API int srt_comm_unique_id(unsigned char id[SRT_COMM_ID_BYTES]);
SRT_API int srt_comm_init_rank(srt_ctx *ctx, const unsigned char id[SRT_COMM_ID_BYTES], uint32_t rank, uint32_t world, srt_comm **out);
SRT_API int srt_comm_available(void);
SRT_API int srt_comm_set_gather_planes(srt_comm *comm, uint32_t planes);
SRT_API void srt_comm_destroy(srt_comm *comm);
SRT_API const char *srt_comm_last_error(const srt_comm *comm);
SRT_API uint32_t srt_comm_world(const srt_comm *comm);
SRT_API uint32_t srt_comm_local_count(const srt_comm *comm);
SRT_API srt_ctx *srt_comm_ctx(srt_comm *comm, uint32_t local_index);
SRT_API srt_ctx *srt_comm_root_ctx(srt_comm *comm);
SRT_API int srt_comm_upload_scene(srt_comm *comm, const srt_scene *s);
SRT_API int srt_comm_set_camera(srt_comm *comm, const srt_camera_data *cam);
SRT_API int srt_comm_init_device_params(srt_comm *comm, uint32_t tx, uint32_t ty, uint32_t bx, uint32_t by, uint32_t chunk_w,
                                        uint32_t chunk_h, uint32_t spp, uint32_t bounce_limit, uint64_t seed);
SRT_API int srt_render_frame_multi(srt_comm *comm, uint32_t width, uint32_t height, uint32_t offx, uint32_t offy);
SRT_API int srt_comm_accum_reset(srt_comm *comm);
SRT_API int srt_render_frame_multi_accum(srt_comm *comm, uint32_t width, uint32_t height, uint32_t offx, uint32_t offy, uint32_t spp_add);
SRT_API int srt_comm_accum_reset_adaptive(srt_comm *comm, const srt_adaptive *cfg);
SRT_API int srt_comm_accum_active(srt_comm *comm, uint64_t *active);
SRT_API int srt_comm_accum_reset_spectral(srt_comm *comm);
SRT_API int srt_comm_accum_reset_features(srt_comm *comm);
SRT_API int srt_comm_accum_reset_adaptive_features(srt_comm *comm, const srt_adaptive *cfg);
SRT_API int srt_comm_accum_reset_spectral_features(srt_comm *comm);
SRT_API int srt_comm_accum_reset_streams(srt_comm *comm, uint32_t streams);
SRT_API int srt_comm_synchronize(srt_comm *comm);
SRT_API int srt_comm_stats(srt_comm *comm, uint64_t *rays, uint64_t *paths, float *max_kernel_ms);
SRT_API int srt_comm_last_gather_ms(srt_comm *comm, float *ms);

typedef struct {
    double wave_cycles_mean, wave_cycles_max;
    double wall_ms;
    uint64_t instr_per_wave;
    uint32_t n_waves, n_cu, waves_per_simd;
    uint32_t reserved;
    double wave_cycles_min;
} srt_calibration;
SRT_API int srt_calibrate(srt_ctx *ctx, int kind, uint32_t waves_per_simd, uint32_t iters, srt_calibration *out);

#ifdef __cplusplus
}
#endif
#endif
```

Before: 16110 Mray/s.

## Split tile queue into per-class lists (glass, plain, sky) with home waves and stealing

During the cost probe, each tile is classified by its hit and glass counts. A new single-block kernel then builds separate glass, plain and sky work lists and assigns each class a share of home waves in proportion to its probe cost. The render kernel pulls tiles from its home class list and steals from the other classes in a fixed order, aiming to keep divergent glass paths apart from cheap sky or plain tiles within a wave and so cut SIMD divergence and tail imbalance. This adds an extra kernel launch, more queue-head atomics and extra counters, and if the probe estimate is poor it can misbalance work.

```diff
diff --git a/cuda-spectral-ray-tracer_amd/binding.py b/cuda-spectral-ray-tracer_amd/binding.py
--- a/cuda-spectral-ray-tracer_amd/binding.py
+++ b/cuda-spectral-ray-tracer_amd/binding.py
@@ -7,6 +7,7 @@
 N_CIE = 95
 TILE_PLANES = 9
 TILE_LANES = 64
+CLASS_HEADER_WORDS = 16
 
 SCENE_CORNELL, SCENE_PRISM, SCENE_TRIS, SCENE_RANDOM_SPHERES, SCENE_MESH100K = 0, 1, 2, 100, 101
 BVH_REFERENCE, BVH_SAH = 0, 1
@@ -166,6 +167,11 @@
     "srt_device_op_sweep": (_i, [_vp, _i, _fp, _fp, _sz, _fp]),
     "srt_order_tiles_kat": (_i, [_vp, C.POINTER(_u32), _u32, _u32, _u32, _u32, C.POINTER(_u32), _sz, C.POINTER(_u32), C.POINTER(_u32)]),
     "srt_read_tile_schedule": (_i, [_vp, _i, C.POINTER(_u32), _sz, C.POINTER(TileScheduleInfo)]),
+    "srt_set_class_queue_test_knobs": (_i, [_vp, _i, _u32, _u32, _i]),
+    "srt_class_lists_kat": (_i, [_vp, C.POINTER(_u32), C.POINTER(_u32), C.POINTER(_u32), _u32, _u32, _u32, _i, _u32, _u32, _i, C.POINTER(_u32)]),
+    "srt_read_class_schedule": (_i, [_vp, C.POINTER(_u32), C.POINTER(_u32), _sz, C.POINTER(_i)]),
+    "srt_read_class_passes": (_i, [_vp, C.POINTER(_u64)]),
+    "srt_read_rng_state": (_i, [_vp, C.POINTER(_u32), _sz]),
     "srt_calibrate": (_i, [_vp, _i, _u32, _u32, C.POINTER(Calibration)]),
     "srt_ctx_device": (_i, [_vp]),
     "srt_ctx_cu_count": (_i, [_vp]),
diff --git a/cuda-spectral-ray-tracer_amd/csrc/srt_capi.cpp b/cuda-spectral-ray-tracer_amd/csrc/srt_capi.cpp
--- a/cuda-spectral-ray-tracer_amd/csrc/srt_capi.cpp
+++ b/cuda-spectral-ray-tracer_amd/csrc/srt_capi.cpp
@@ -75,6 +75,11 @@
     uint32_t probe_spp = 2;
     int order_max_pct = -1;
     DeviceBuffer d_tile_cost, d_tile_order;
+    uint32_t class_queues = 1, class_glass_min = 16, class_glass_pct = 100;
+    int32_t class_home_glass = -1;
+    DeviceBuffer d_class;
+    bool class_bound = false;
+    bool class_sched_valid = false;
     srt_tile_schedule_info sched_note = {};
     bool sched_probe_queue = false, sched_compacted_queue = false;
     bool count_traversal = false;
@@ -174,6 +179,18 @@
     }
 };
 
+struct ClassLayout {
+    uint32_t *sched = nullptr, *counts = nullptr;
+    size_t tiles = 0;
+    static size_t counts_bytes(size_t tiles) { return 2 * tiles * sizeof(uint32_t); }
+    static size_t bytes(size_t tiles) { return (kClassHeaderWords + 3 * tiles) * sizeof(uint32_t) + counts_bytes(tiles); }
+    explicit ClassLayout(const srt_ctx *c) {
+        if (!c->d_class) return;
+        tiles = (c->d_class.bytes / sizeof(uint32_t) - kClassHeaderWords) / 5;
+        sched = c->d_class.as<uint32_t>(); counts = sched + kClassHeaderWords + 3 * tiles;
+    }
+};
+
 struct AdaptQueue {
     uint32_t *info, *rows, *flags;
     unsigned long long *counts;
@@ -285,7 +302,7 @@
     const size_t tile_floats = (size_t)std::max<uint32_t>(c->tiles_padded, 1) * kTileLanes;
     HIP_TRY(c, c->d_tiles.reserve(tile_floats * kTilePlanes * sizeof(float)));
     if (!(adaptive_mode(ps.mode) && ps.later)) HIP_TRY(c, hipMemsetAsync(c->d_tiles.ptr, 0, tile_floats * c->gather_planes * sizeof(float), ps.st));
-    HIP_TRY(c, hipMemsetAsync(c->d_counters.ptr, 0, (kCounters + 1) * sizeof(unsigned long long), ps.st));
+    HIP_TRY(c, hipMemsetAsync(c->d_counters.ptr, 0, (kCounters + kQueueHeadSlots) * sizeof(unsigned long long), ps.st));
     return SRT_OK;
 }
 
@@ -305,23 +322,47 @@
     p.debug_lane_limit = c->debug_lane_limit;
 }
 
+uint32_t class_lists_wanted(const srt_ctx *c, const Pass &ps, uint32_t n_waves_plan) {
+    if (!c->class_queues || ps.streams != 1 || !ps.plan.all_cached || c->fringe_stride != 96u) return 0u;
+    if (!(ps.mode == Plain || ps.mode == Accum || (ps.mode == Counting && c->order_profile.magic != kOrderProfileMagic))) return 0u;
+    if (c->class_queues == 2) return 2u;
+    return (uint64_t)c->tiles_local >= 6ull * n_waves_plan ? 1u : 0u;
+}
+
 int run_cost_probe(srt_ctx *c, const Pass &ps, const RenderParams &p) {
     HIP_TRY(c, c->d_tile_cost.reserve(TileSchedule::cost_bytes(c->tiles_local)));
     HIP_TRY(c, c->d_tile_order.reserve(TileSchedule::order_bytes(c->tiles_local)));
     const TileSchedule sched(c);
     HIP_TRY(c, hipMemsetAsync(sched.cost, 0, TileSchedule::cost_bytes(c->tiles_local), ps.st));
+    const uint32_t n_waves_plan = std::max<uint32_t>((uint32_t)c->n_cu * (uint32_t)ps.plan.waves_per_cu / ps.streams, 1u);
+    const uint32_t want_lists = class_lists_wanted(c, ps, n_waves_plan);
+    c->class_sched_valid = false;
+    ClassLayout cls(c);
+    if (want_lists) {
+        HIP_TRY(c, c->d_class.reserve(ClassLayout::bytes(c->tiles_local)));
+        cls = ClassLayout(c);
+        HIP_TRY(c, hipMemsetAsync(cls.sched, 0, c->d_class.bytes, ps.st));
+    }
     RenderParams pp = p;
-    pp.spp = c->probe_spp; pp.tile_cost = sched.cost;
+    pp.spp = c->probe_spp; pp.tile_cost = sched.cost; pp.prio_cost = want_lists ? cls.counts : nullptr;
     RoctxRange range_probe("srt cost probe + pixel queue");
     HIP_TRY(c, launch_render(pp, c->knobs, (uint32_t)c->n_cu, Probe, ps.st));
-    const uint32_t n_waves_plan = std::max<uint32_t>((uint32_t)c->n_cu * (uint32_t)ps.plan.waves_per_cu / ps.streams, 1u);
     const uint32_t order_pct = c->order_max_pct >= 0 ? (uint32_t)c->order_max_pct : ((!ps.plan.all_cached && (uint64_t)c->tiles_local < 6ull * n_waves_plan) ? 100u : 0u);
     const uint32_t split_pct = queue_may_split(c, ps.streams) ? c->split_load_pct : 0u;
     HIP_TRY(c, launch_order_tiles(sched.cost, sched.sorted, sched.rows, c->tiles_local, n_waves_plan, split_pct, sched.info, order_pct, ps.st));
     c->sched_note = {};
     c->sched_note.tiles_local = c->tiles_local; c->sched_note.n_waves_plan = n_waves_plan; c->sched_note.split_load_pct = split_pct;
     c->sched_note.order_max_pct = order_pct; c->sched_note.streams = ps.streams;
-    HIP_TRY(c, hipMemsetAsync(c->d_counters.as<unsigned long long>() + kCounters, 0, sizeof(unsigned long long), ps.st));
+    if (want_lists) {
+        ClassListsParams q = {};
+        q.cost = sched.cost; q.counts = cls.counts; q.rows = sched.rows; q.queue_info = sched.info; q.n = c->tiles_local;
+        q.n_waves = render_launch_grid(ps.plan, (uint32_t)c->n_cu, p.waves_per_cu_override, queue_may_split(c, ps.streams) ? split_rows_bound(c) : c->tiles_local).waves;
+        q.allow = want_lists;
+        q.glass_min = c->class_glass_min; q.glass_pct = c->class_glass_pct; q.home_glass = c->class_home_glass; q.sched = cls.sched;
+        HIP_TRY(c, launch_class_lists(q, ps.st));
+        c->class_sched_valid = true;
+    }
+    HIP_TRY(c, hipMemsetAsync(c->d_counters.as<unsigned long long>() + kCounters, 0, kQueueHeadSlots * sizeof(unsigned long long), ps.st));
     return SRT_OK;
 }
 
@@ -354,7 +395,10 @@
         p.queue_rows = sched.info;
         p.prio_cost = sched.cost;
         if (queue_may_split(c, ps.streams)) p.queue_rows_bound = split_rows_bound(c);
-    }
+        if (c->class_sched_valid && class_lists_wanted(c, ps, c->sched_note.n_waves_plan))
+            p.tile_cost = ClassLayout(c).sched;
+    }
+    c->class_bound = render_class_schedule(p) != nullptr;
     c->sched_probe_queue = ps.ordered && src != QueueSource::Identity;
     p.queue_rows_bound *= ps.streams;
     return SRT_OK;
@@ -487,6 +531,13 @@
         if (const char *ev = getenv("SRT_WIDE_REFS")) { c->knobs.wide_refs = atoi(ev) != 0; c->knobs_from_env = true; }
         if (const char *ev = getenv("SRT_LDS_CACHE_MAX")) { c->knobs.lds_cache_max = std::max(0, atoi(ev)); c->knobs_from_env = true; }
     }
+    if (const char *ev = getenv("SRT_CLASS_QUEUES")) { const int v = atoi(ev); c->class_queues = v <= 0 ? 0u : 1u; }
+    if (const char *tk = getenv("SRT_TEST_KNOBS")) if (atoi(tk) == 1) {
+        if (const char *ev = getenv("SRT_CLASS_QUEUES")) if (atoi(ev) == 2) c->class_queues = 2u;
+        if (const char *ev = getenv("SRT_CLASS_HOME_GLASS")) c->class_home_glass = std::max(-1, atoi(ev));
+    }
+    if (const char *ev = getenv("SRT_CLASS_GLASS_MIN")) c->class_glass_min = (uint32_t)std::max(1, atoi(ev));
+    if (const char *ev = getenv("SRT_CLASS_GLASS_PCT")) c->class_glass_pct = (uint32_t)std::min(1000, std::max(1, atoi(ev)));
     if (const char *ev = getenv("SRT_SPLIT_LOAD")) c->split_load_pct = (uint32_t)std::max(0, atoi(ev));
     if (const char *ev = getenv("SRT_ORDER_MAX_PCT")) c->order_max_pct = std::min(400, std::max(-1, atoi(ev)));
     {
@@ -497,8 +548,8 @@
     cmf_rows(rows.data());
     int rc = upload(c, c->d_cmf, rows);
     if (rc != SRT_OK) { delete c; return rc; }
-    if ((e = c->d_counters.reserve((kCounters + 1) * sizeof(unsigned long long))) != hipSuccess ||
-        (e = hipMemset(c->d_counters.ptr, 0, (kCounters + 1) * sizeof(unsigned long long))) != hipSuccess ||
+    if ((e = c->d_counters.reserve((kCounters + kQueueHeadSlots) * sizeof(unsigned long long))) != hipSuccess ||
+        (e = hipMemset(c->d_counters.ptr, 0, (kCounters + kQueueHeadSlots) * sizeof(unsigned long long))) != hipSuccess ||
         (e = hipEventCreate(&c->ev0)) != hipSuccess || (e = hipEventCreate(&c->ev1)) != hipSuccess) {
         int r = hip_fail(nullptr, e, "srt_create");
         srt_destroy(c);
@@ -1749,6 +1800,78 @@
     return SRT_OK;
 }
 
+int srt_set_class_queue_test_knobs(srt_ctx *c, int mode, uint32_t glass_min, uint32_t glass_pct, int home_glass) {
+    if (!c || mode < 0 || mode > 2 || glass_min == 0 || glass_pct == 0 || glass_pct > 1000 || home_glass < -1) return fail(c, SRT_ERR_INVALID, "srt_set_class_queue_test_knobs: bad argument");
+    c->accum.invalidate();
+    c->class_queues = (uint32_t)mode; c->class_glass_min = glass_min; c->class_glass_pct = glass_pct; c->class_home_glass = home_glass;
+    return SRT_OK;
+}
+
+int srt_class_lists_kat(srt_ctx *c, const uint32_t *cost, const uint32_t *counts, const uint32_t *rows, uint32_t n_rows, uint32_t n, uint32_t n_waves,
+                        int allow, uint32_t glass_min, uint32_t glass_pct, int home_glass, uint32_t *sched_out) {
+    if (!c || !cost || !counts || !rows || !sched_out) return fail(c, SRT_ERR_INVALID, "srt_class_lists_kat: null argument");
+    if (n == 0 || n > (1u << 20) || n_rows == 0 || n_rows > 64u * n || n_waves == 0 || n_waves > (1u << 20) || glass_min == 0 || glass_pct == 0 || glass_pct > 1000 || home_glass < -1 || allow < 0 || allow > 2)
+        return fail(c, SRT_ERR_INVALID, "srt_class_lists_kat: bad argument");
+    if (n_rows == n)
+        for (uint32_t q = 0; q < n; q++)
+            if ((rows[q] & kQueueTileMask) >= n) return fail(c, SRT_ERR_INVALID, "srt_class_lists_kat: a row names a tile beyond n");
+    HIP_TRY(c, hipSetDevice(c->device));
+    const size_t words = kClassHeaderWords + 3 * (size_t)n;
+    DeviceBuffer d_cost, d_counts, d_rows, d_info, d_sched;
+    HIP_TRY_AS(c, "srt_class_lists_kat", d_cost.reserve(n * sizeof(uint32_t)));
+    HIP_TRY_AS(c, "srt_class_lists_kat", d_counts.reserve(2 * (size_t)n * sizeof(uint32_t)));
+    HIP_TRY_AS(c, "srt_class_lists_kat", d_rows.reserve((size_t)n_rows * sizeof(uint32_t)));
+    HIP_TRY_AS(c, "srt_class_lists_kat", d_info.reserve(4 * sizeof(uint32_t)));
+    HIP_TRY_AS(c, "srt_class_lists_kat", d_sched.reserve((words + 64) * sizeof(uint32_t)));
+    const uint32_t info[4] = {n_rows, 0u, 0u, 0u};
+    HIP_TRY_AS(c, "srt_class_lists_kat", hipMemcpy(d_cost.ptr, cost, n * sizeof(uint32_t), hipMemcpyHostToDevice));
+    HIP_TRY_AS(c, "srt_class_lists_kat", hipMemcpy(d_counts.ptr, counts, 2 * (size_t)n * sizeof(uint32_t), hipMemcpyHostToDevice));
+    HIP_TRY_AS(c, "srt_class_lists_kat", hipMemcpy(d_rows.ptr, rows, (size_t)n_rows * sizeof(uint32_t), hipMemcpyHostToDevice));
+    HIP_TRY_AS(c, "srt_class_lists_kat", hipMemcpy(d_info.ptr, info, sizeof(info), hipMemcpyHostToDevice));
+    HIP_TRY_AS(c, "srt_class_lists_kat", hipMemset(d_sched.ptr, 0xff, (words + 64) * sizeof(uint32_t)));
+    ClassListsParams q = {};
+    q.cost = d_cost.as<uint32_t>(); q.counts = d_counts.as<uint32_t>(); q.rows = d_rows.as<uint32_t>(); q.queue_info = d_info.as<uint32_t>();
+    q.n = n; q.n_waves = n_waves; q.allow = (uint32_t)allow; q.glass_min = glass_min; q.glass_pct = glass_pct; q.home_glass = home_glass; q.sched = d_sched.as<uint32_t>();
+    HIP_TRY_AS(c, "srt_class_lists_kat", launch_class_lists(q, nullptr));
+    HIP_TRY_AS(c, "srt_class_lists_kat", hipDeviceSynchronize());
+    HIP_TRY_AS(c, "srt_class_lists_kat", hipMemcpy(sched_out, d_sched.ptr, (words + 64) * sizeof(uint32_t), hipMemcpyDeviceToHost));
+    return SRT_OK;
+}
+
+int srt_read_class_schedule(srt_ctx *c, uint32_t *sched_out, uint32_t *counts_out, size_t n, int *bound) {
+    if (!c || !sched_out || !counts_out) return fail(c, SRT_ERR_INVALID, "srt_read_class_schedule: null argument");
+    const ClassLayout cls(c);
+    if (!c->sched_probe_queue) return fail(c, SRT_ERR_INVALID, "srt_read_class_schedule: the last launch ran no cost probe's queue");
+    if (n != c->tiles_local) return fail(c, SRT_ERR_INVALID, "srt_read_class_schedule: n must be the context's local tiles");
+    if (bound) *bound = 0;
+    if (!c->class_sched_valid || !cls.sched || n > cls.tiles) {
+        memset(sched_out, 0, (kClassHeaderWords + 3 * n) * sizeof(uint32_t));
+        memset(counts_out, 0, ClassLayout::counts_bytes(n));
+        return SRT_OK;
+    }
+    if (const int rc = srt_synchronize(c)) return rc;
+    HIP_TRY(c, hipMemcpy(sched_out, cls.sched, (kClassHeaderWords + 3 * n) * sizeof(uint32_t), hipMemcpyDeviceToHost));
+    HIP_TRY(c, hipMemcpy(counts_out, cls.counts, ClassLayout::counts_bytes(n), hipMemcpyDeviceToHost));
+    if (bound) *bound = c->class_bound ? 1 : 0;
+    return SRT_OK;
+}
+
+int srt_read_rng_state(srt_ctx *c, uint32_t *out, size_t n_words) {
+    if (!c || !out || !c->d_rng || n_words != 6 * (size_t)c->n_lanes) return fail(c, SRT_ERR_INVALID, "srt_read_rng_state: device parameters not initialised / n_words is not 6 * lanes");
+    if (const int rc = srt_synchronize(c)) return rc;
+    HIP_TRY(c, hipMemcpy(out, c->d_rng.ptr, n_words * sizeof(uint32_t), hipMemcpyDeviceToHost));
+    return SRT_OK;
+}
+
+int srt_read_class_passes(srt_ctx *c, uint64_t out[4]) {
+    if (!c || !out) return fail(c, SRT_ERR_INVALID, "srt_read_class_passes: null argument");
+    if (const int rc = srt_synchronize(c)) return rc;
+    unsigned long long h[kCounters];
+    HIP_TRY(c, hipMemcpy(h, c->d_counters.ptr, sizeof(h), hipMemcpyDeviceToHost));
+    out[0] = h[15]; out[1] = h[25]; out[2] = h[26]; out[3] = h[27];
+    return SRT_OK;
+}
+
 int srt_read_tile_schedule(srt_ctx *c, int which, uint32_t *rows_out, size_t rows_cap, srt_tile_schedule_info *info) {
     if (!c || !info || (!rows_out && rows_cap) || (which != 0 && which != 1)) return fail(c, SRT_ERR_INVALID, "srt_read_tile_schedule: bad argument");
     if (which == 0 ? !c->sched_probe_queue : !c->sched_compacted_queue)
diff --git a/cuda-spectral-ray-tracer_amd/csrc/srt_internal.h b/cuda-spectral-ray-tracer_amd/csrc/srt_internal.h
--- a/cuda-spectral-ray-tracer_amd/csrc/srt_internal.h
+++ b/cuda-spectral-ray-tracer_amd/csrc/srt_internal.h
@@ -65,6 +65,31 @@
     unsigned long long *counters;
     uint32_t *wave_debug;
 };
+inline const uint32_t *render_class_schedule(const RenderParams &p) { return p.tile_cost; }
+inline uint32_t *probe_class_counts(const RenderParams &p) { return const_cast<uint32_t *>(p.prio_cost); }
+
+constexpr uint32_t kClassGlass = 0, kClassPlain = 1, kClassSky = 2, kClasses = 3;
+constexpr uint32_t kClassHeaderWords = 16;
+enum ClassHeader : uint32_t { kClsEnabled = 0, kClsLen = 1 , kClsHome = 4 , kClsWaves = 7, kClsStart = 8 , kClsCap = 11 };
+constexpr uint32_t kClassHeadWord = 2;
+constexpr int kQueueHeadSlots = 3;
+__host__ __device__ inline uint32_t class_steal_order(uint32_t home, uint32_t k) {
+    return home == kClassGlass ? k : home == kClassPlain ? (k == 0u ? kClassPlain : k == 1u ? kClassGlass : kClassSky) : 2u - k;
+}
+struct ClassListsParams {
+    const uint32_t *cost;
+    const uint32_t *counts;
+    const uint32_t *rows;
+    const uint32_t *queue_info;
+    uint32_t n;
+    uint32_t n_waves;
+    uint32_t allow;
+    uint32_t glass_min;
+    uint32_t glass_pct;
+    int32_t home_glass;
+    uint32_t *sched;
+};
+hipError_t launch_class_lists(const ClassListsParams &p, hipStream_t st);
 
 struct OrderProfile {
     unsigned long long magic;
diff --git a/cuda-spectral-ray-tracer_amd/csrc/srt_kernel_common.h b/cuda-spectral-ray-tracer_amd/csrc/srt_kernel_common.h
--- a/cuda-spectral-ray-tracer_amd/csrc/srt_kernel_common.h
+++ b/cuda-spectral-ray-tracer_amd/csrc/srt_kernel_common.h
@@ -19,7 +19,9 @@
     uint32_t n_assigned_slots;
     uint32_t prio_cost[2], prio_full;
     uint32_t accum_sums[2], spp_total;
-    uint32_t accum_sum2[2], accum_state[2], min_spp;
+    union { uint32_t accum_sum2[2]; uint32_t class_sched[2]; };
+    union { uint32_t accum_state[2]; struct { uint32_t class_on, class_step; }; };
+    uint32_t min_spp;
     float rel_tol, abs_tol;
     uint32_t accum_film[2];
     uint32_t streams;
diff --git a/cuda-spectral-ray-tracer_amd/csrc/srt_kernels.hip b/cuda-spectral-ray-tracer_amd/csrc/srt_kernels.hip
--- a/cuda-spectral-ray-tracer_amd/csrc/srt_kernels.hip
+++ b/cuda-spectral-ray-tracer_amd/csrc/srt_kernels.hip
@@ -122,6 +122,7 @@
     constexpr bool FILM = (MODE == 5 || MODE == 9);
     constexpr bool STREAMS = (MODE == 6);
     constexpr bool FEATURES = (MODE == 7 || MODE == 8 || MODE == 9);
+    constexpr bool CLASSQ = (MODE == 0 || MODE == 1 || MODE == 3) && ALL_CACHED;
     constexpr bool S2_MEM = ADAPT && !NARROW && !ALL_CACHED && !PAIRED;
     extern __shared__ float4 lds4[];
     lds_uniforms *U = (lds_uniforms *)lds4;
@@ -157,6 +158,12 @@
             const AccumHeader *ah = reinterpret_cast<const AccumHeader *>(P.wave_debug);
             split_ptr(ah->sums, U->accum_sums);
             U->spp_total = ah->spp_total;
+        }
+        if constexpr (CLASSQ) {
+            const uint32_t *cq = P.tile_cost;
+            split_ptr(cq, U->class_sched);
+            U->class_on = (cq && cq[kClsEnabled] != 0u && cq[kClsWaves] == gridDim.x * (blockDim.x >> 6) && P.queue_rows && P.tile_order) ? 1u : 0u;
+            U->class_step = 0u;
         }
         if constexpr (ADAPT) {
             const AccumHeader *ah = reinterpret_cast<const AccumHeader *>(P.wave_debug);
@@ -238,6 +245,9 @@
     uint32_t pixel_rays0 = 0, max_pix_iters = 0, max_pix_rays = 0;
     uint32_t w_shade_passes = 0, l_shade = 0, l_cam = 0, w_reject_iters = 0;
     uint32_t n_hits = 0;
+    uint32_t l_list_slots = 0;
+    uint32_t w_hit_passes = 0, w_glass_passes = 0;
+    uint32_t probe_hits = 0, probe_glass = 0;
 
     for (;;) {
         if (__ballot(have_pixel) == 0ull) parked = false;
@@ -279,6 +289,8 @@
                     const uint32_t mat = __float_as_uint(s0.w);
                     const uint32_t mtype = __float_as_uint(s1.x);
                     const float fuzz = s1.y;
+                    if (PROBE) { probe_hits++; if (mtype == 2u) probe_glass++; }
+                    if (COUNT && lane == (uint32_t)(__ffsll((long long)__ballot(1)) - 1)) w_hit_passes++;
 
                     V3 scatter_direction = mk(0.f, 0.f, 0.f);
                     float eps_sign = 1.0f;
@@ -287,6 +299,7 @@
                     if (mtype == 4u) {
                         did_scatter = false;
                     } else if (mtype == 2u) {
+                        if (COUNT && lane == (uint32_t)(__ffsll((long long)__ballot(1)) - 1)) w_glass_passes++;
                         float ir = sellmeier_index(s1.z, s1.w, s2.x, s2.y, s2.z, s2.w, wl[0]);
                         float refraction_ratio = front_face ? (1.0f / ir) : ir;
                         float cos_theta = fminf(dot(-unit_in, n), 1.0f);
@@ -407,6 +420,12 @@
                     uint32_t *tcost = join_ptr<uint32_t>(U->tile_cost[0], U->tile_cost[1]);
                     atomicAdd(tcost + cur_tile_local, ts.n_iters - pixel_iters0 + 1u);
                     atomicMax(tcost + P.tiles_local + cur_tile_local, ts.n_iters - pixel_iters0 + 1u);
+                    if (P.prio_cost) {
+                        uint32_t *ccount = const_cast<uint32_t *>(P.prio_cost) + 2u * cur_tile_local;
+                        if (probe_hits) atomicAdd(ccount, probe_hits);
+                        if (probe_glass) atomicAdd(ccount + 1u, probe_glass);
+                    }
+                    probe_hits = 0; probe_glass = 0;
                     have_pixel = false;
                 }
                 if (have_pixel && COUNT) { max_pix_iters = max(max_pix_iters, ts.n_iters - pixel_iters0); max_pix_rays = max(max_pix_rays, n_rays - pixel_rays0); }
@@ -470,6 +489,39 @@
                     const bool row_open = SRT_ASSIGN_FIRST_ROW != 0 && ((U->first_row_taken >> wave) & 1u) == 0u;
                     if (COUNT && row_open && m != ~0ull && lane == (uint32_t)leader) atomicAdd(&P.counters[23], 1ull);
                     const bool assigned = row_open && m == ~0ull;
+                    uint32_t pix = 0u;
+                    bool have_slot = false;
+                    if constexpr (CLASSQ) {
+                        if (U->class_on != 0u) {
+                            const uint32_t *cq = join_ptr<const uint32_t>(U->class_sched[0], U->class_sched[1]);
+                            const uint32_t g = assigned_band(wave) * gridDim.x + blockIdx.x, h0 = cq[kClsHome], h1 = cq[kClsHome + 1];
+                            const uint32_t home = g < h0 ? kClassGlass : (g < h0 + h1 ? kClassPlain : kClassSky);
+                            const uint32_t home_i = g - (home == kClassGlass ? 0u : home == kClassPlain ? h0 : h0 + h1);
+                            bool from_head = !assigned;
+                            if (assigned) {
+                                if (lane == 0) atomicOr((unsigned int *)&U->first_row_taken, 1u << wave);
+                                if (home_i < cq[kClsLen + home]) pix = cq[kClassHeaderWords + home * cq[kClsCap] + home_i] * 64u + lane;
+                                else from_head = true;
+                            }
+                            if (from_head) {
+                                const uint32_t step = (U->class_step >> (2u * wave)) & 3u;
+                                if (step == 3u) pix = 0xffffffffu;
+                                else {
+                                    const uint32_t cls = class_steal_order(home, step);
+                                    const uint32_t n_take = (uint32_t)__popcll(m), len64 = cq[kClsLen + cls] * 64u;
+                                    if ((int)lane == leader) base = atomicAdd(join_ptr<uint32_t>(U->pixel_counter[0], U->pixel_counter[1]) + kClassHeadWord + cls, n_take);
+                                    base = (uint32_t)__shfl((int)base, leader, 64) + cq[kClsStart + cls] * 64u;
+                                    if ((int)lane == leader && (base >= len64 || n_take > len64 - base)) atomicAdd((unsigned int *)&U->class_step, 1u << (2u * wave));
+                                    const uint32_t slot = base + (uint32_t)__popcll(m & ((1ull << lane) - 1ull));
+                                    if (slot >= len64) continue;
+                                    pix = cq[kClassHeaderWords + cls * cq[kClsCap] + (slot >> 6)] * 64u + (slot & 63u);
+                                }
+                            }
+                            if (COUNT && pix != 0xffffffffu) l_list_slots++;
+                            have_slot = true;
+                        }
+                    }
+                    if (!have_slot) {
                     if (assigned) {
                         if (lane == 0) atomicOr((unsigned int *)&U->first_row_taken, 1u << wave);
                         base = (assigned_band(wave) * gridDim.x + blockIdx.x) * 64u;
@@ -478,7 +530,8 @@
                         if ((int)lane == leader) base = atomicAdd(join_ptr<uint32_t>(U->pixel_counter[0], U->pixel_counter[1]), (uint32_t)__popcll(m));
                         base = (uint32_t)__shfl((int)base, leader, 64) + (SRT_ASSIGN_FIRST_ROW != 0 ? U->n_assigned_slots : 0u);
                     }
-                    const uint32_t pix = base + (uint32_t)__popcll(m & ((1ull << lane) - 1ull));
+                    pix = base + (uint32_t)__popcll(m & ((1ull << lane) - 1ull));
+                    }
                     if (pix >= U->n_rows * 64u) { dead = true; searching = false; if (COUNT && t_dry == 0) t_dry = __builtin_amdgcn_s_memtime(); }
                     else {
                         const uint32_t *tile_order = join_ptr<const uint32_t>(U->tile_order[0], U->tile_order[1]);
@@ -682,8 +735,12 @@
                 atomicAdd(&P.counters[5], (unsigned long long)ts.w_alive);
             }
             const uint32_t nn = wave_sum(ts.n_nan), nh = wave_sum(n_hits);
+            const uint32_t hp = wave_sum(w_hit_passes), gp = wave_sum(w_glass_passes), ls = wave_sum(l_list_slots);
             if (lane == 0) {
                 atomicAdd(&P.counters[24], (unsigned long long)nh);
+                atomicAdd(&P.counters[25], (unsigned long long)hp);
+                atomicAdd(&P.counters[26], (unsigned long long)gp);
+                atomicAdd(&P.counters[27], (unsigned long long)ls);
                 atomicAdd(&P.counters[6], (unsigned long long)nn);
                 atomicAdd(&P.counters[7], (unsigned long long)ts.w_fringe);
                 atomicAdd(&P.counters[8], (unsigned long long)ts.l_fringe);
@@ -1157,4 +1214,89 @@
     return hipGetLastError();
 }
 
-}
+template <int>
+__global__ __launch_bounds__(1024) void class_lists_kernel(const ClassListsParams P) {
+    __shared__ uint32_t s_scan[kClasses][1024];
+    __shared__ unsigned long long s_w[kClasses];
+    __shared__ uint32_t s_len[kClasses];
+    const uint32_t t = threadIdx.x;
+    const uint32_t n = P.n, n_rows = P.queue_info[0];
+    uint32_t *hdr = P.sched;
+    if (n_rows != n) {
+        if (t < kClassHeaderWords) hdr[t] = t == kClsWaves ? P.n_waves : t == kClsCap ? n : 0u;
+        return;
+    }
+    auto class_of = [&](uint32_t tile) -> uint32_t {
+        const uint32_t hits = P.counts[2u * tile], glass = P.counts[2u * tile + 1u];
+        return hits == 0u ? kClassSky : (glass >= P.glass_min ? kClassGlass : kClassPlain);
+    };
+    if (t < kClasses) s_w[t] = 0ull;
+    __syncthreads();
+    const uint32_t per = (n + 1023u) / 1024u;
+    const uint32_t lo = min(n, t * per), hi = min(n, lo + per);
+    uint32_t mine[kClasses] = {0u, 0u, 0u};
+    unsigned long long w[kClasses] = {0ull, 0ull, 0ull};
+    for (uint32_t q = lo; q < hi; q++) {
+        const uint32_t tile = queue_row_unpack(P.rows[q]).tile_local;
+        const uint32_t c = tile < n ? class_of(tile) : kClassPlain;
+        mine[c]++; w[c] += tile < n ? P.cost[tile] : 0u;
+    }
+    for (uint32_t c = 0; c < kClasses; c++) { s_scan[c][t] = mine[c]; if (w[c]) atomicAdd(&s_w[c], w[c]); }
+    __syncthreads();
+    for (uint32_t off = 1; off < 1024u; off <<= 1) {
+        uint32_t add[kClasses];
+        for (uint32_t c = 0; c < kClasses; c++) add[c] = t >= off ? s_scan[c][t - off] : 0u;
+        __syncthreads();
+        for (uint32_t c = 0; c < kClasses; c++) s_scan[c][t] += add[c];
+        __syncthreads();
+    }
+    if (t < kClasses) s_len[t] = s_scan[t][1023];
+    uint32_t at[kClasses] = {s_scan[0][t] - mine[0], s_scan[1][t] - mine[1], s_scan[2][t] - mine[2]};
+    __syncthreads();
+    for (uint32_t q = lo; q < hi; q++) {
+        const uint32_t tile = queue_row_unpack(P.rows[q]).tile_local;
+        const uint32_t c = tile < n ? class_of(tile) : kClassPlain;
+        hdr[kClassHeaderWords + c * n + at[c]++] = q;
+    }
+    if (t != 0) return;
+    const uint32_t len[kClasses] = {s_len[0], s_len[1], s_len[2]};
+    const uint32_t n_waves = P.n_waves;
+    unsigned long long cw[kClasses] = {s_w[0] * P.glass_pct / 100ull, s_w[1], s_w[2]};
+    while ((cw[0] + cw[1] + cw[2]) >> 40) { cw[0] >>= 1; cw[1] >>= 1; cw[2] >>= 1; }
+    for (uint32_t c = 0; c < kClasses; c++) if (len[c] && cw[c] == 0ull) cw[c] = 1ull;
+    const unsigned long long total = cw[0] + cw[1] + cw[2];
+    uint32_t home[kClasses] = {0u, 0u, 0u};
+    bool ok;
+    if (P.home_glass >= 0) {
+        home[0] = min((uint32_t)P.home_glass, n_waves);
+        const uint32_t rest = n_waves - home[0];
+        const unsigned long long d = cw[1] + cw[2];
+        home[2] = d ? (uint32_t)((unsigned long long)rest * cw[2] / d) : 0u;
+        home[1] = rest - home[2];
+        ok = true;
+    } else {
+        const uint32_t k = (len[0] ? 1u : 0u) + (len[1] ? 1u : 0u) + (len[2] ? 1u : 0u);
+        ok = k >= 2u && n_waves >= k;
+        if (ok) {
+            for (uint32_t c = 0; c < kClasses; c++) home[c] = len[c] ? max(1u, (uint32_t)((unsigned long long)n_waves * cw[c] / total)) : 0u;
+            const uint32_t r = len[1] ? kClassPlain : (cw[0] >= cw[2] ? kClassGlass : kClassSky);
+            const uint32_t a = r == 0u ? 1u : 0u, b = r == 2u ? 1u : 2u;
+            while (home[a] + home[b] > n_waves - 1u) { if (home[a] >= home[b]) home[a]--; else home[b]--; }
+            home[r] = n_waves - home[a] - home[b];
+            if (2u * home[kClassGlass] > n_waves) ok = false;
+        }
+        if (P.allow == 2u) { if (home[0] + home[1] + home[2] != n_waves) { home[0] = 0u; home[1] = n_waves; home[2] = 0u; } ok = true; }
+    }
+    hdr[kClsEnabled] = (P.allow && ok) ? 1u : 0u;
+    for (uint32_t c = 0; c < kClasses; c++) { hdr[kClsLen + c] = len[c]; hdr[kClsHome + c] = home[c]; hdr[kClsStart + c] = min(home[c], len[c]); }
+    hdr[kClsWaves] = n_waves; hdr[kClsCap] = n;
+    for (uint32_t k = kClsCap + 1u; k < kClassHeaderWords; k++) hdr[k] = 0u;
+}
+
+hipError_t launch_class_lists(const ClassListsParams &p, hipStream_t st) {
+    if (p.n == 0) return hipSuccess;
+    hipLaunchKernelGGL(class_lists_kernel<0>, dim3(1), dim3(1024), 0, st, p);
+    return hipGetLastError();
+}
+
+}
diff --git a/cuda-spectral-ray-tracer_amd/renderer.py b/cuda-spectral-ray-tracer_amd/renderer.py
--- a/cuda-spectral-ray-tracer_amd/renderer.py
+++ b/cuda-spectral-ray-tracer_amd/renderer.py
@@ -385,6 +385,38 @@
         rows, info = np.zeros(64 * tl, np.uint32), B.TileScheduleInfo()
         self._ck(B.lib().srt_read_tile_schedule(self._h, int(which), rows.ctypes.data_as(C.POINTER(C.c_uint32)), rows.size, C.byref(info)))
         return rows[:info.n_rows].copy(), {name: getattr(info, name) for name, _ in B.TileScheduleInfo._fields_ if name != "reserved"}
+
+
+    def set_class_queue_test_knobs(self, mode=1, glass_min=16, glass_pct=100, home_glass=-1):
+        self._ck(B.lib().srt_set_class_queue_test_knobs(self._h, int(mode), int(glass_min), int(glass_pct), int(home_glass)))
+
+    def class_lists_kat(self, cost, counts, rows, n_waves, allow=True, glass_min=16, glass_pct=100, home_glass=-1):
+        cost = np.ascontiguousarray(cost, np.uint32); counts = np.ascontiguousarray(counts, np.uint32).reshape(-1); rows = np.ascontiguousarray(rows, np.uint32)
+        n = cost.size
+        u32p = C.POINTER(C.c_uint32)
+        out = np.zeros(B.CLASS_HEADER_WORDS + 3 * n + 64, np.uint32)
+        self._ck(B.lib().srt_class_lists_kat(self._h, cost.ctypes.data_as(u32p), counts.ctypes.data_as(u32p), rows.ctypes.data_as(u32p), rows.size, n,
+                                             int(n_waves), int(allow), int(glass_min), int(glass_pct), int(home_glass), out.ctypes.data_as(u32p)))
+        return out
+
+    def class_schedule(self):
+        _, _, tl, _ = self.tile_buffer()
+        u32p = C.POINTER(C.c_uint32)
+        sched, counts, bound = np.zeros(B.CLASS_HEADER_WORDS + 3 * tl, np.uint32), np.zeros((tl, 2), np.uint32), C.c_int(0)
+        self._ck(B.lib().srt_read_class_schedule(self._h, sched.ctypes.data_as(u32p), counts.ctypes.data_as(u32p), tl, C.byref(bound)))
+        hdr = sched[:B.CLASS_HEADER_WORDS].copy()
+        lists = [sched[B.CLASS_HEADER_WORDS + c * tl:][:hdr[1 + c]].copy() for c in range(3)]
+        return hdr, lists, counts, bool(bound.value)
+
+    def rng_state(self):
+        out = np.zeros((6, self.geom["n_lanes"]), np.uint32)
+        self._ck(B.lib().srt_read_rng_state(self._h, out.ctypes.data_as(C.POINTER(C.c_uint32)), out.size))
+        return out
+
+    def class_passes(self):
+        out = (C.c_uint64 * 4)()
+        self._ck(B.lib().srt_read_class_passes(self._h, out))
+        return dict(passes=out[0], hit_passes=out[1], glass_passes=out[2], list_slots=out[3])
 
 
 class Comm:
diff --git a/include/srt_c_api.h b/include/srt_c_api.h
--- a/include/srt_c_api.h
+++ b/include/srt_c_api.h
@@ -221,6 +221,13 @@
     uint32_t reserved;
 } srt_tile_schedule_info;
 SRT_API int srt_read_tile_schedule(srt_ctx *ctx, int which, uint32_t *rows_out, size_t rows_cap, srt_tile_schedule_info *info);
+#define SRT_CLASS_HEADER_WORDS 16
+SRT_API int srt_set_class_queue_test_knobs(srt_ctx *ctx, int mode, uint32_t glass_min, uint32_t glass_pct, int home_glass);
+SRT_API int srt_class_lists_kat(srt_ctx *ctx, const uint32_t *cost, const uint32_t *counts, const uint32_t *rows, uint32_t n_rows, uint32_t n,
+                                uint32_t n_waves, int allow, uint32_t glass_min, uint32_t glass_pct, int home_glass, uint32_t *sched_out);
+SRT_API int srt_read_class_schedule(srt_ctx *ctx, uint32_t *sched_out, uint32_t *counts_out, size_t n, int *bound);
+SRT_API int srt_read_rng_state(srt_ctx *ctx, uint32_t *out, size_t n_words);
+SRT_API int srt_read_class_passes(srt_ctx *ctx, uint64_t out[4]);
 
 SRT_API int srt_ctx_device(const srt_ctx *ctx);
 SRT_API int srt_ctx_cu_count(const srt_ctx *ctx);
```

Result: faster. 16460 Mray/s (median of 6 runs) (+2.2%).
